# ml-rust/blazr

Measured on AMD Instinct MI355X. Metric: decode tokens/sec, Llama-3-8B AWQ-INT4 seq=1 on MI355X (and HBM-roofline fraction), higher is better.
Workload: dtype i4; 1 GPU; llama3-8b-awq greedy decode, batch 1, seq=1, prompt 16 (seed 26), whole step as one hipGraph; N>1 = independent replicas; resident_weight_bytes=5754585088, context_at_end=242

## Files before the change

blazr_amd/csrc/bz_host.hip:

```cpp
#include "bz_internal.h"
#include "bz_ggml.h"
#include <stdarg.h>
#include <stdio.h>
#include <string.h>
#include <math.h>
#include <algorithm>
#include <chrono>
#include <numeric>
#include <unordered_map>

static thread_local char g_err[1024] = "";
static bool bz_trace_on() { static int t = -1; if (t < 0) t = getenv("BZ_TRACE") ? 1 : 0; return t == 1; }
#define BZ_TRACE(...) do { if (bz_trace_on()) { fprintf(stderr, "[bz] " __VA_ARGS__); fputc('\n', stderr); fflush(stderr); } } while (0)
void bz_set_error(const char* fmt, ...) {
  va_list ap;
  va_start(ap, fmt);
  vsnprintf(g_err, sizeof(g_err), fmt, ap);
  va_end(ap);
}
extern "C" const char* bz_last_error(void) { return g_err; }
extern "C" int bz_abi_version(void) { return BZ_ABI_VERSION; }

size_t bz_dtype_size(int dt) {
  switch (dt) {
// ... 179 lines not shown
extern "C" int bz_tensor_to_host_pipelined(const bz_tensor* t, uint64_t ev, void* host, size_t bytes) {
  BZ_API_BEGIN
  if (!t || !host) BZ_FAIL(BZ_E_INVALID, "bad argument");
  if (bytes > t->nbytes) BZ_FAIL(BZ_E_INVALID, "to_host_pipelined: size");
  bz_device* d = t->dev;
  std::lock_guard<std::mutex> dlock__(d->mu);
  if (ev >= d->events.size()) BZ_FAIL(BZ_E_INVALID, "bad event");
  BZ_HIP(hipStreamWaitEvent(d->copy_stream, d->events[ev], 0));
  BZ_HIP(hipMemcpyAsync(host, t->ptr, bytes, hipMemcpyDeviceToHost, d->copy_stream));
  BZ_HIP(hipStreamSynchronize(d->copy_stream));
  return BZ_OK;
  BZ_API_END
}

struct RawTensor {
  int kind = 0;
  int dtype = BZ_F32;
  std::vector<int64_t> shape;
  int64_t N = 0, K = 0; int gs = 0; int ggml_type = 0;
  void* d0 = nullptr; void* d1 = nullptr; void* d2 = nullptr;
  float* d_bias = nullptr;
  std::vector<int32_t> g_idx;
  size_t bytes = 0;
  bool consumed = false;
};

struct FusedLinear {
  std::vector<LinearDev> parts;
  std::vector<int> n_off;
  int N = 0, K = 0;
  bool fix_out = true;
};

struct LayerDev {
  float* attn_norm = nullptr; float* ffn_norm = nullptr;
  FusedLinear qkv, o, gateup, down;
  void* down_slabs = nullptr;
};

struct MambaLayerDev {
  float* norm = nullptr; float* conv_w = nullptr; float* conv_b = nullptr; float* dt_bias = nullptr; float* A_log = nullptr; float* D = nullptr;
  float* gnorm = nullptr;
  FusedLinear in_proj, out_proj;
};

struct DsLayerDev {
  float* attn_norm = nullptr; float* ffn_norm = nullptr; float* kv_norm = nullptr;
  FusedLinear qkva, o;
  float* q_norm = nullptr; FusedLinear q_b;
  void* kv_b = nullptr; int kv_b_dt = BZ_BF16;
  bool is_moe = false;
  FusedLinear gateup, down;
  void* router = nullptr; int router_dt = BZ_BF16;
  void* e_gu = nullptr; void* e_dn = nullptr; int e_dt = BZ_BF16;
};

struct bz_model {
  std::recursive_mutex mu;
  std::vector<DsLayerDev> dlayers;
  float* mla_ws = nullptr; int mla_nsplit = 1;
  float* mla_scw = nullptr; float* mla_mxw = nullptr;
  double* mla_wsd = nullptr;
  long long* moe_gu_acc = nullptr;
  float* moe_xn = nullptr; float* moe_gu = nullptr; float* moe_out = nullptr; long long* moe_acc = nullptr; int* moe_sel = nullptr; float* moe_w = nullptr; float* moe_lg = nullptr; unsigned* moe_cnt = nullptr;
  int dpf_rows = 0; float* dpf_att = nullptr; void* dpf_xg16 = nullptr; float* dpf_gu = nullptr; void* dpf_a16 = nullptr; float* dpf_ye = nullptr; float* dpf_ysh = nullptr;
  int* dpf_sel = nullptr; float* dpf_w = nullptr; int* dpf_cnt = nullptr; int* dpf_off = nullptr; int* dpf_rowof = nullptr; int* dpf_tokof = nullptr;
  std::vector<MambaLayerDev> mlayers;
  float* ybuf = nullptr; float* vss = nullptr;
  int mpf_rows = 0; float* mpf_h = nullptr; float* mpf_t = nullptr; float* mpf_zx = nullptr; float* mpf_xbc = nullptr; float* mpf_y = nullptr; float* mpf_vss = nullptr;
  void* mpf_x16 = nullptr;
  bz_device* dev = nullptr;
  bz_model_config cfg;
  bool finalized = false;
  std::unordered_map<std::string, RawTensor> raw;
  std::vector<LayerDev> layers;
  void* embed = nullptr; int embed_dt = BZ_F16;
  int embed_ggml = 0;
  float* final_norm = nullptr;
  FusedLinear lm_head;
  std::unordered_map<std::string, LinearDev> named;
  std::vector<void*> owned;
  float* cos_t = nullptr; float* sin_t = nullptr;
  float* rope_cur = nullptr;
  float* att_ws = nullptr;
  float* hbuf[2] = {nullptr, nullptr};
  int pf_rows = 0; float* pf_h = nullptr; float* pf_t = nullptr; float* pf_qkv = nullptr; float* pf_gu = nullptr; void* pf_x16 = nullptr;
  int* row_pos = nullptr; int row_pos_n = 0;
  long long* pf_acc = nullptr;
  struct GqPf { float* wscale = nullptr; void* w3 = nullptr; };
  std::unordered_map<const FusedLinear*, GqPf> gq_pf;
  size_t gq_cache_bytes = 0;
  unsigned* gq_amax = nullptr; void* gq_w3_scratch = nullptr; size_t gq_w3_scratch_bytes = 0;
  void* pf_x3 = nullptr; float* pf_rscale = nullptr;
  void* pf_xq = nullptr; size_t pf_xq_bytes = 0;
  float* pf_ws = nullptr; size_t pf_ws_bytes = 0;
  long long* ring[3] = {nullptr, nullptr, nullptr};
  float* dring[3] = {nullptr, nullptr, nullptr};
  int ring_n = 0;
  float* attn_out = nullptr;
  float* logits = nullptr;
  float* pval = nullptr; int* pidx = nullptr; int nparts = 0;
  float* scratch = nullptr;
  long long* tok_tmp = nullptr;
  int* pos_tmp = nullptr;
  size_t resident = 0, per_token = 0;
};

static int dev_alloc(bz_model* m, void** p, size_t bytes) {
  hipError_t e = hipMalloc(p, std::max<size_t>(bytes, 16));
  if (e != hipSuccess) BZ_FAIL(BZ_E_OOM, "hipMalloc(%zu) failed: %s", bytes, hipGetErrorString(e));
  m->owned.push_back(*p);
  return BZ_OK;
}
static int upload(bz_device* d, void** out, const void* host, size_t bytes) {
  hipError_t e = hipMalloc(out, std::max<size_t>(bytes, 16));
  if (e != hipSuccess) BZ_FAIL(BZ_E_OOM, "hipMalloc(%zu) failed: %s", bytes, hipGetErrorString(e));
  if (bytes) BZ_HIP(hipMemcpy(*out, host, bytes, hipMemcpyHostToDevice));
  (void)d;
  return BZ_OK;
}

extern "C" int bz_model_create(bz_device* dev, const bz_model_config* cfg, bz_model** out) {
  BZ_API_BEGIN
  if (!dev || !cfg || !out) BZ_FAIL(BZ_E_INVALID, "bz_model_create: null argument");
  if (cfg->abi_version != BZ_ABI_VERSION) BZ_FAIL(BZ_E_INVALID, "config abi_version %d != %d", cfg->abi_version, BZ_ABI_VERSION);
  if (cfg->arch != BZ_ARCH_LLAMA && cfg->arch != BZ_ARCH_MAMBA2 && cfg->arch != BZ_ARCH_DEEPSEEK2) BZ_FAIL(BZ_E_UNSUPPORTED, "arch %d is not implemented", cfg->arch);
  if (cfg->arch == BZ_ARCH_DEEPSEEK2) {
    if (cfg->hidden <= 0 || cfg->n_layers <= 0 || cfg->n_heads <= 0 || cfg->vocab <= 0 || cfg->max_seq_len <= 0 || cfg->mla_kv_lora_rank <= 0 ||
        cfg->mla_nope_dim <= 0 || cfg->mla_rope_dim <= 0 || cfg->mla_v_dim <= 0 || cfg->moe_n_experts < 0 || cfg->moe_first_dense < 0)
      BZ_FAIL(BZ_E_INVALID, "config: non-positive deepseek2 dimension");
    if (cfg->mla_q_lora_rank < 0 || cfg->mla_q_lora_rank % 8) BZ_FAIL(BZ_E_INVALID, "config: q_lora_rank %d must be a non-negative multiple of 8", cfg->mla_q_lora_rank);
    if (cfg->hidden % 8 || cfg->mla_kv_lora_rank % 8 || cfg->mla_kv_lora_rank > 1024 || cfg->mla_rope_dim > 64 || (cfg->mla_rope_dim & 1) || cfg->mla_nope_dim % 4 ||
        cfg->mla_v_dim % 4)
      BZ_FAIL(BZ_E_UNSUPPORTED, "config: MLA dims unsupported (rank %% 8, rank <= 1024, rope <= 64 even, nope/v %% 4)");
    if (cfg->moe_n_experts > 0 && (cfg->moe_top_k <= 0 || cfg->moe_top_k > cfg->moe_n_experts || cfg->moe_top_k > 16 || cfg->moe_n_shared < 0 || cfg->moe_n_shared > 8 ||
                                   cfg->moe_inter <= 0 || cfg->moe_inter % 8 || cfg->moe_n_experts > 1024))
      BZ_FAIL(BZ_E_INVALID, "config: bad MoE configuration");
    if ((cfg->moe_first_dense > 0 || cfg->moe_n_experts == 0) && (cfg->inter <= 0 || cfg->inter % 8)) BZ_FAIL(BZ_E_INVALID, "config: dense layers need inter %% 8 == 0");
    if ((size_t)(cfg->mla_kv_lora_rank * 6 + cfg->mla_rope_dim * 2 + cfg->mla_nope_dim + 8 + cfg->max_seq_len) * 4 + 64 > 160 * 1024)
      BZ_FAIL(BZ_E_UNSUPPORTED, "config: max_seq_len %d too long for the single-pass MLA attention kernel", cfg->max_seq_len);
  } else if (cfg->arch == BZ_ARCH_MAMBA2) {
    if (cfg->hidden <= 0 || cfg->n_layers <= 0 || cfg->vocab <= 0 || cfg->ssm_d_inner <= 0 || cfg->ssm_n_heads <= 0 || cfg->ssm_head_dim <= 0 ||
        cfg->ssm_d_state <= 0 || cfg->ssm_n_groups <= 0 || cfg->ssm_conv_kernel < 2)
      BZ_FAIL(BZ_E_INVALID, "config: non-positive mamba2 dimension");
    if (cfg->ssm_n_heads * cfg->ssm_head_dim != cfg->ssm_d_inner || cfg->ssm_n_heads % cfg->ssm_n_groups || cfg->hidden % 8 || cfg->ssm_d_inner % 8)
      BZ_FAIL(BZ_E_INVALID, "config: inconsistent mamba2 dimensions");
  } else {
  if (cfg->hidden <= 0 || cfg->n_layers <= 0 || cfg->n_heads <= 0 || cfg->n_kv_heads <= 0 || cfg->head_dim <= 0 || cfg->inter <= 0 ||
      cfg->vocab <= 0 || cfg->max_seq_len <= 0)
    BZ_FAIL(BZ_E_INVALID, "config: non-positive dimension");
  if (cfg->n_heads % cfg->n_kv_heads) BZ_FAIL(BZ_E_INVALID, "config: n_heads %% n_kv_heads != 0");
  if (cfg->hidden % 8 || cfg->head_dim % 8 || cfg->inter % 8) BZ_FAIL(BZ_E_UNSUPPORTED, "config: hidden/head_dim/inter must be multiples of 8");
  }
  if (cfg->act_dtype != BZ_F32 && cfg->act_dtype != BZ_F16 && cfg->act_dtype != BZ_BF16) BZ_FAIL(BZ_E_INVALID, "config: bad act_dtype");
  bz_model* m = new bz_model();
  m->dev = dev; m->cfg = *cfg;
  if (cfg->arch == BZ_ARCH_DEEPSEEK2) { m->cfg.n_kv_heads = 1; m->cfg.head_dim = cfg->mla_kv_lora_rank + cfg->mla_rope_dim; }
  bz_dev_retain(dev);
  *out = m;
  return BZ_OK;
  BZ_API_END
}

static void raw_free(RawTensor& r) {
  if (r.d0) hipFree(r.d0);
  if (r.d1) hipFree(r.d1);
// ... 423 lines not shown
  const int H = c.hidden, nq = c.n_heads, nkv = c.n_kv_heads, hd = c.head_dim, I = c.inter, V = c.vocab;
  char nm[256];
  m->layers.resize(c.n_layers);
  for (int l = 0; l < c.n_layers; l++) {
    LayerDev& Ld = m->layers[l];
    snprintf(nm, sizeof nm, "model.layers.%d.", l);
    std::string p = nm;
    BZ_TRY(take_vector_f32(m, p + "input_layernorm.weight", H, &Ld.attn_norm));
    BZ_TRY(take_vector_f32(m, p + "post_attention_layernorm.weight", H, &Ld.ffn_norm));
    BZ_TRY(build_fused(m, {p + "self_attn.q_proj", p + "self_attn.k_proj", p + "self_attn.v_proj"}, &Ld.qkv));
    BZ_TRY(build_fused(m, {p + "self_attn.o_proj"}, &Ld.o));
    BZ_TRY(build_fused(m, {p + "mlp.gate_proj", p + "mlp.up_proj"}, &Ld.gateup));
    BZ_TRY(build_fused(m, {p + "mlp.down_proj"}, &Ld.down));
    if (Ld.qkv.N != (nq + 2 * nkv) * hd || Ld.qkv.K != H) BZ_FAIL(BZ_E_INVALID, "layer %d: q/k/v shapes do not match the config", l);
    if (Ld.o.N != H || Ld.o.K != nq * hd) BZ_FAIL(BZ_E_INVALID, "layer %d: o_proj shape does not match the config", l);
    if (Ld.gateup.N != 2 * I || Ld.gateup.K != H) BZ_FAIL(BZ_E_INVALID, "layer %d: gate/up shapes do not match the config", l);
    if (Ld.down.N != H || Ld.down.K != I) BZ_FAIL(BZ_E_INVALID, "layer %d: down_proj shape does not match the config", l);
    if (Ld.gateup.parts.size() == 1 && Ld.down.parts.size() == 1 && Ld.down.parts[0].kind == LK_ROWS) {
      char dummy = 0;
      if (bzk_mlp_dense_fusable(Ld.gateup.parts[0], Ld.down.parts[0], &dummy, H, I, c.act_dtype)) {
        BZ_TRY(dev_alloc(m, &Ld.down_slabs, (size_t)H * I * 2));
        BZ_TRY(bzk_repack_down_slabs(m->dev->stream, Ld.down.parts[0].w, H, I, Ld.down_slabs));
        m->resident += (size_t)H * I * 2;
      }
    }
  }
  BZ_HIP(hipStreamSynchronize(m->dev->stream));
  BZ_TRY(take_vector_f32(m, "model.norm.weight", H, &m->final_norm));
  {
    auto it = m->raw.find("model.embed_tokens.weight");
    if (it == m->raw.end()) BZ_FAIL(BZ_E_NOTFOUND, "finalize: 'model.embed_tokens.weight' was not added");
    RawTensor& r = it->second;
    const bool qemb = r.kind == 3 && (r.ggml_type == BZ_GGML_Q8_0 || r.ggml_type == BZ_GGML_Q4_K || r.ggml_type == BZ_GGML_Q5_K || r.ggml_type == BZ_GGML_Q6_K ||
                                      ggml_is_legacy(r.ggml_type));
    if ((r.kind != 0 && !qemb) || r.N != V || r.K != H)
      BZ_FAIL(BZ_E_INVALID, "finalize: embed_tokens must be dense or GGUF Q4_0/Q4_1/Q5_0/Q5_1/Q8_0/Q4_K/Q5_K/Q6_K [vocab, hidden]");
    const bool tied = c.tie_embeddings || !m->raw.count("lm_head.weight");
    if (qemb && tied) {
      if (V % 64) BZ_FAIL(BZ_E_UNSUPPORTED, "finalize: tied lm_head over a quantised embedding needs a vocabulary that is a multiple of 64 (vocab %d)", V);
      LinearDev L;
      BZ_TRY(build_gq(m, {&r}, &L));
      m->lm_head.parts.push_back(L); m->lm_head.n_off.push_back(0); m->lm_head.N = V; m->lm_head.K = H; m->lm_head.fix_out = true;
      LinearDev Vw = L; Vw.owned = false;
      m->named["lm_head.weight"] = Vw;
    }
    m->embed = r.d0; m->embed_dt = qemb ? BZ_U8 : r.dtype; m->embed_ggml = qemb ? r.ggml_type : 0;
    r.d0 = nullptr; m->owned.push_back(m->embed); r.consumed = true;
    m->resident += r.bytes;
    if (tied && !qemb) {
      LinearDev L; L.kind = LK_ROWS; L.N = V; L.K = H; L.wdt = m->embed_dt; L.w = m->embed; L.owned = false;
      L.bytes = 0; L.algo_bytes = r.bytes;
      m->lm_head.parts.push_back(L); m->lm_head.n_off.push_back(0); m->lm_head.N = V; m->lm_head.K = H; m->lm_head.fix_out = false;
      m->named["lm_head.weight"] = L;
    } else if (!tied) {
      BZ_TRY(build_fused(m, {"lm_head"}, &m->lm_head));
      force_direct(&m->lm_head);
      if (m->lm_head.N != V || m->lm_head.K != H) BZ_FAIL(BZ_E_INVALID, "finalize: lm_head shape does not match the config");
    }
  }
  if (m->lm_head.parts.size() != 1) BZ_FAIL(BZ_E_UNSUPPORTED, "finalize: lm_head must be a single tensor");
  for (auto& kv : m->raw) if (!kv.second.consumed) BZ_FAIL(BZ_E_INVALID, "finalize: tensor '%s' is not used by this architecture", kv.first.c_str());
  m->raw.clear();

  std::vector<float> cs, sn;
  rope_tables_host(c, cs, sn);
  void* p;
  BZ_TRY(dev_alloc(m, &p, cs.size() * 4)); m->cos_t = (float*)p; BZ_HIP(hipMemcpy(p, cs.data(), cs.size() * 4, hipMemcpyHostToDevice));
  BZ_TRY(dev_alloc(m, &p, sn.size() * 4)); m->sin_t = (float*)p; BZ_HIP(hipMemcpy(p, sn.data(), sn.size() * 4, hipMemcpyHostToDevice));
  BZ_TRY(dev_alloc(m, &p, 256 * 4)); m->rope_cur = (float*)p; BZ_HIP(hipMemset(p, 0, 256 * 4));
  BZ_TRY(dev_alloc(m, &p, bzk_attn_split_ws_bytes(c.n_heads))); m->att_ws = (float*)p;

  m->ring_n = std::max(std::max((nq + 2 * nkv) * hd, 2 * I), std::max(H, nq * hd));
  if (m->lm_head.fix_out) m->ring_n = std::max(m->ring_n, V);
  for (int i = 0; i < 3; i++) {
    BZ_TRY(dev_alloc(m, &p, (size_t)m->ring_n * 8)); m->ring[i] = (long long*)p; BZ_HIP(hipMemset(p, 0, (size_t)m->ring_n * 8));
    BZ_TRY(dev_alloc(m, &p, (size_t)m->ring_n * 4)); m->dring[i] = (float*)p; BZ_HIP(hipMemset(p, 0, (size_t)m->ring_n * 4));
  }
  for (int i = 0; i < 2; i++) { BZ_TRY(dev_alloc(m, &p, (size_t)H * 4)); m->hbuf[i] = (float*)p; }
  BZ_TRY(dev_alloc(m, &p, (size_t)nq * hd * 4)); m->attn_out = (float*)p;
  BZ_TRY(dev_alloc(m, &p, (size_t)V * 4)); m->logits = (float*)p;
  m->nparts = m->lm_head.fix_out ? 64 : bzk_gemv_rows_blocks(m->lm_head.parts[0]);
  BZ_TRY(dev_alloc(m, &p, (size_t)m->nparts * 4)); m->pval = (float*)p;
  BZ_TRY(dev_alloc(m, &p, (size_t)m->nparts * 4)); m->pidx = (int*)p;
  BZ_TRY(dev_alloc(m, &p, 4096)); m->scratch = (float*)p;
  BZ_TRY(dev_alloc(m, &p, 64)); m->tok_tmp = (long long*)p;
  BZ_TRY(dev_alloc(m, &p, 64)); m->pos_tmp = (int*)p;

  size_t act_b = bz_dtype_size(c.act_dtype);
  m->per_token = (size_t)(2 * c.n_layers + 1) * H * act_b + (m->embed_ggml ? ggml_blk_row_bytes(m->embed_ggml, H) : (size_t)H * bz_dtype_size(m->embed_dt));
  for (auto& Ld : m->layers)
    for (FusedLinear* F : {&Ld.qkv, &Ld.o, &Ld.gateup, &Ld.down})
      for (auto& L : F->parts) { m->resident += L.bytes; m->per_token += L.algo_bytes; }
  for (auto& L : m->lm_head.parts) { m->resident += L.bytes; m->per_token += L.algo_bytes; }
  BZ_HIP(hipDeviceSynchronize());
  m->finalized = true;
  return BZ_OK;
  BZ_API_END
}

extern "C" int bz_model_get_config(const bz_model* m, bz_model_config* out) {
  BZ_API_BEGIN
  if (!m || !out) BZ_FAIL(BZ_E_INVALID, "null argument");
  *out = m->cfg;
  return BZ_OK;
  BZ_API_END
}
extern "C" int bz_model_weight_bytes(const bz_model* m, size_t* resident, size_t* per_token) {
  BZ_API_BEGIN
  if (!m || !m->finalized) BZ_FAIL(BZ_E_INVALID, "model not finalized");
  if (resident) *resident = m->resident;
  if (per_token) *per_token = m->per_token;
  return BZ_OK;
  BZ_API_END
}
extern "C" int bz_rope_caches(bz_model* m, float* c, float* s) {
  BZ_API_BEGIN
  if (!m || !m->finalized) BZ_FAIL(BZ_E_INVALID, "model not finalized");
  size_t n = (size_t)m->cfg.max_seq_len * (m->cfg.head_dim / 2) * 4;
  if (c) BZ_HIP(hipMemcpy(c, m->cos_t, n, hipMemcpyDeviceToHost));
  if (s) BZ_HIP(hipMemcpy(s, m->sin_t, n, hipMemcpyDeviceToHost));
  return BZ_OK;
  BZ_API_END
}

static int take_dense(bz_model* m, const std::string& name, int64_t N, int64_t K, void** out, int* dt, size_t* bytes) {
  auto it = m->raw.find(name);
  if (it == m->raw.end()) BZ_FAIL(BZ_E_NOTFOUND, "finalize: tensor '%s' was not added", name.c_str());
  RawTensor& r = it->second;
  if (r.kind != 0 || r.N != N || r.K != K) BZ_FAIL(BZ_E_INVALID, "finalize: '%s' must be dense [%lld, %lld]", name.c_str(), (long long)N, (long long)K);
  *out = r.d0; *dt = r.dtype; if (bytes) *bytes = r.bytes;
  r.d0 = nullptr; m->owned.push_back(*out); r.consumed = true;
  m->resident += r.bytes;
  return BZ_OK;
}
static int stack_dense(bz_model* m, const std::string& name, int64_t N, int64_t K, int dt, void* dst, int64_t col0, int64_t ncols) {
  auto it = m->raw.find(name);
  if (it == m->raw.end()) BZ_FAIL(BZ_E_NOTFOUND, "finalize: tensor '%s' was not added", name.c_str());
  RawTensor& r = it->second;
  if (r.kind != 0 || r.N != N || r.K != K || r.dtype != dt) BZ_FAIL(BZ_E_INVALID, "finalize: '%s' must be dense [%lld, %lld] of the experts' dtype", name.c_str(), (long long)N, (long long)K);
  const size_t es = bz_dtype_size(dt);
  BZ_HIP(hipMemcpy2D(dst, (size_t)ncols * es, (const char*)r.d0 + (size_t)col0 * es, (size_t)K * es, (size_t)ncols * es, (size_t)N, hipMemcpyDeviceToDevice));
  return BZ_OK;
}

static int finalize_dsv2(bz_model* m) {
  const bz_model_config& c = m->cfg;
  const int H = c.hidden, NH = c.n_heads, R = c.mla_kv_lora_rank, DN = c.mla_nope_dim, DR = c.mla_rope_dim, DV = c.mla_v_dim, V = c.vocab;
  const int E = c.moe_n_experts, TK = c.moe_top_k, NS = c.moe_n_shared, MI = c.moe_inter;
  const size_t act_b = bz_dtype_size(c.act_dtype);
  char nm[256];
  m->dlayers.resize(c.n_layers);
  size_t per_token = 0;
  int ring_n = std::max(H, NH * DV);
  for (int l = 0; l < c.n_layers; l++) {
    DsLayerDev& L = m->dlayers[l];
    snprintf(nm, sizeof nm, "model.layers.%d.", l);
    std::string p = nm;
    BZ_TRY(take_vector_f32(m, p + "input_layernorm.weight", H, &L.attn_norm));
    BZ_TRY(take_vector_f32(m, p + "post_attention_layernorm.weight", H, &L.ffn_norm));
    BZ_TRY(take_vector_f32(m, p + "self_attn.kv_a_layernorm.weight", R, &L.kv_norm));
    const int QL = c.mla_q_lora_rank;
    if (QL > 0) {
      BZ_TRY(build_fused(m, {p + "self_attn.q_a_proj", p + "self_attn.kv_a_proj_with_mqa"}, &L.qkva));
      BZ_TRY(take_vector_f32(m, p + "self_attn.q_a_layernorm.weight", QL, &L.q_norm));
      BZ_TRY(build_fused(m, {p + "self_attn.q_b_proj"}, &L.q_b));
      if (L.q_b.parts.size() != 1 || L.q_b.parts[0].kind != LK_ROWS || L.q_b.N != NH * (DN + DR) || L.q_b.K != QL) BZ_FAIL(BZ_E_INVALID, "layer %d: q_b_proj must be dense [n_heads (nope + rope), q_lora_rank]", l);
// ... 29 lines not shown
      const size_t gu_sz = (size_t)2 * MI * H * es, dn_sz = (size_t)H * MI * es;
      BZ_TRY(dev_alloc(m, &L.e_gu, (size_t)(E + NS) * gu_sz));
      BZ_TRY(dev_alloc(m, &L.e_dn, (size_t)(E + NS) * dn_sz));
      for (int e = 0; e < E; e++) {
        snprintf(nm, sizeof nm, "%smlp.experts.%d.", p.c_str(), e);
        std::string q = nm;
        BZ_TRY(stack_dense(m, q + "gate_proj.weight", MI, H, L.e_dt, (char*)L.e_gu + (size_t)e * gu_sz, 0, H));
        BZ_TRY(stack_dense(m, q + "up_proj.weight", MI, H, L.e_dt, (char*)L.e_gu + (size_t)e * gu_sz + gu_sz / 2, 0, H));
        BZ_TRY(stack_dense(m, q + "down_proj.weight", H, MI, L.e_dt, (char*)L.e_dn + (size_t)e * dn_sz, 0, MI));
        for (const char* t : {"gate_proj.weight", "up_proj.weight", "down_proj.weight"}) { RawTensor& r = m->raw[q + t]; raw_free(r); r.consumed = true; }
      }
      if (NS > 0) {
        std::string q = p + "mlp.shared_experts.";
        auto itg = m->raw.find(q + "gate_proj.weight"), itu = m->raw.find(q + "up_proj.weight");
        if (itg == m->raw.end() || itu == m->raw.end()) BZ_FAIL(BZ_E_NOTFOUND, "finalize: layer %d shared experts missing", l);
        if (itg->second.kind != 0 || itg->second.N != (int64_t)NS * MI || itg->second.K != H || itg->second.dtype != L.e_dt || itu->second.kind != 0 ||
            itu->second.N != (int64_t)NS * MI || itu->second.K != H || itu->second.dtype != L.e_dt)
          BZ_FAIL(BZ_E_INVALID, "finalize: layer %d shared expert shapes do not match the config", l);
        for (int j = 0; j < NS; j++) {
          const size_t half_rows = (size_t)MI * H * es;
          BZ_HIP(hipMemcpy((char*)L.e_gu + (size_t)(E + j) * gu_sz, (const char*)itg->second.d0 + (size_t)j * half_rows, half_rows, hipMemcpyDeviceToDevice));
          BZ_HIP(hipMemcpy((char*)L.e_gu + (size_t)(E + j) * gu_sz + gu_sz / 2, (const char*)itu->second.d0 + (size_t)j * half_rows, half_rows, hipMemcpyDeviceToDevice));
          BZ_TRY(stack_dense(m, q + "down_proj.weight", H, (int64_t)NS * MI, L.e_dt, (char*)L.e_dn + (size_t)(E + j) * dn_sz, (int64_t)j * MI, MI));
        }
        for (const char* t : {"gate_proj.weight", "up_proj.weight", "down_proj.weight"}) { RawTensor& r = m->raw[q + t]; raw_free(r); r.consumed = true; }
      }
      m->resident += (size_t)(E + NS) * (gu_sz + dn_sz);
      per_token += rb + (size_t)(TK + NS) * (gu_sz + dn_sz);
    }
  }
  BZ_TRY(take_vector_f32(m, "model.norm.weight", H, &m->final_norm));
  {
    auto it = m->raw.find("model.embed_tokens.weight");
    if (it == m->raw.end()) BZ_FAIL(BZ_E_NOTFOUND, "finalize: 'model.embed_tokens.weight' was not added");
    RawTensor& r = it->second;
    if (r.kind != 0 || r.N != V || r.K != H) BZ_FAIL(BZ_E_INVALID, "finalize: embed_tokens must be dense [vocab, hidden]");
    m->embed = r.d0; m->embed_dt = r.dtype; r.d0 = nullptr; m->owned.push_back(m->embed); r.consumed = true;
    m->resident += r.bytes;
    if (c.tie_embeddings || !m->raw.count("lm_head.weight")) {
      LinearDev L; L.kind = LK_ROWS; L.N = V; L.K = H; L.wdt = m->embed_dt; L.w = m->embed; L.owned = false; L.bytes = 0; L.algo_bytes = r.bytes;
      m->lm_head.parts.push_back(L); m->lm_head.n_off.push_back(0); m->lm_head.N = V; m->lm_head.K = H; m->lm_head.fix_out = false;
      m->named["lm_head.weight"] = L;
    } else {
      BZ_TRY(build_fused(m, {"lm_head"}, &m->lm_head));
      force_direct(&m->lm_head);
      if (m->lm_head.N != V || m->lm_head.K != H || m->lm_head.fix_out) BZ_FAIL(BZ_E_INVALID, "finalize: lm_head must be dense [vocab, hidden]");
    }
  }
  for (auto& kv : m->raw) if (!kv.second.consumed) BZ_FAIL(BZ_E_INVALID, "finalize: tensor '%s' is not used by this architecture", kv.first.c_str());
  m->raw.clear();
  bz_model_config rc = c; rc.head_dim = DR;
  std::vector<float> cs, sn;
  rope_tables_host(rc, cs, sn);
  void* p;
  BZ_TRY(dev_alloc(m, &p, cs.size() * 4)); m->cos_t = (float*)p; BZ_HIP(hipMemcpy(p, cs.data(), cs.size() * 4, hipMemcpyHostToDevice));
  BZ_TRY(dev_alloc(m, &p, sn.size() * 4)); m->sin_t = (float*)p; BZ_HIP(hipMemcpy(p, sn.data(), sn.size() * 4, hipMemcpyHostToDevice));
  m->ring_n = std::max(ring_n, NH * (DN + DR) + R + DR + c.mla_q_lora_rank);
  for (int i = 0; i < 3; i++) {
    BZ_TRY(dev_alloc(m, &p, (size_t)m->ring_n * 8)); m->ring[i] = (long long*)p; BZ_HIP(hipMemset(p, 0, (size_t)m->ring_n * 8));
    BZ_TRY(dev_alloc(m, &p, (size_t)m->ring_n * 4)); m->dring[i] = (float*)p; BZ_HIP(hipMemset(p, 0, (size_t)m->ring_n * 4));
  }
  for (int i = 0; i < 2; i++) { BZ_TRY(dev_alloc(m, &p, (size_t)H * 4)); m->hbuf[i] = (float*)p; }
  BZ_TRY(dev_alloc(m, &p, (size_t)NH * DV * 4)); m->attn_out = (float*)p;
  m->mla_nsplit = bzk_mla_nsplit(NH);
  BZ_TRY(dev_alloc(m, &p, (size_t)NH * m->mla_nsplit * (R + 2) * 4)); m->mla_ws = (float*)p;
  BZ_TRY(dev_alloc(m, &p, (size_t)NH * m->mla_nsplit * (R + 1) * 8)); m->mla_wsd = (double*)p;
  BZ_TRY(dev_alloc(m, &p, (size_t)NH * m->mla_nsplit * ((c.max_seq_len + m->mla_nsplit - 1) / m->mla_nsplit + 1) * 4)); m->mla_scw = (float*)p;
  BZ_TRY(dev_alloc(m, &p, (size_t)NH * m->mla_nsplit * 4)); m->mla_mxw = (float*)p;
  BZ_TRY(dev_alloc(m, &p, (size_t)V * 4)); m->logits = (float*)p;
  if (E > 0) {
    BZ_TRY(dev_alloc(m, &p, (size_t)H * 4)); m->moe_xn = (float*)p;
    BZ_TRY(dev_alloc(m, &p, (size_t)(TK + NS) * 2 * MI * 4)); m->moe_gu = (float*)p;
    BZ_TRY(dev_alloc(m, &p, (size_t)(TK + NS) * 2 * MI * 8)); m->moe_gu_acc = (long long*)p; BZ_HIP(hipMemset(p, 0, (size_t)(TK + NS) * 2 * MI * 8));
    BZ_TRY(dev_alloc(m, &p, (size_t)H * 4)); m->moe_out = (float*)p;
    BZ_TRY(dev_alloc(m, &p, (size_t)(TK + 1) * H * 8)); m->moe_acc = (long long*)p; BZ_HIP(hipMemset(p, 0, (size_t)(TK + 1) * H * 8));
    BZ_TRY(dev_alloc(m, &p, (size_t)(TK + NS + 4) * 4)); m->moe_sel = (int*)p; BZ_HIP(hipMemset(p, 0, (size_t)(TK + NS + 4) * 4));
    BZ_TRY(dev_alloc(m, &p, (size_t)(TK + NS + 4) * 4)); m->moe_w = (float*)p; BZ_HIP(hipMemset(p, 0, (size_t)(TK + NS + 4) * 4));
    BZ_TRY(dev_alloc(m, &p, (size_t)(E + 4) * 4)); m->moe_lg = (float*)p;
    BZ_TRY(dev_alloc(m, &p, 64)); m->moe_cnt = (unsigned*)p; BZ_HIP(hipMemset(p, 0, 64));
  }
  m->nparts = bzk_gemv_rows_blocks(m->lm_head.parts[0]);
  BZ_TRY(dev_alloc(m, &p, (size_t)m->nparts * 4)); m->pval = (float*)p;
  BZ_TRY(dev_alloc(m, &p, (size_t)m->nparts * 4)); m->pidx = (int*)p;
  BZ_TRY(dev_alloc(m, &p, 4096)); m->scratch = (float*)p;
  BZ_TRY(dev_alloc(m, &p, 64)); m->tok_tmp = (long long*)p;
  BZ_TRY(dev_alloc(m, &p, 64)); m->pos_tmp = (int*)p;
  for (auto& L : m->lm_head.parts) { m->resident += L.bytes; per_token += L.algo_bytes; }
  m->per_token = per_token + (size_t)H * bz_dtype_size(m->embed_dt) + (size_t)H * act_b;
  BZ_HIP(hipDeviceSynchronize());
  m->finalized = true;
  return BZ_OK;
}

static int finalize_mamba2(bz_model* m) {
  const bz_model_config& c = m->cfg;
  const int D = c.hidden, DI = c.ssm_d_inner, NH = c.ssm_n_heads, NS = c.ssm_d_state, G = c.ssm_n_groups, KC = c.ssm_conv_kernel, V = c.vocab;
  const int conv_dim = DI + 2 * G * NS, d_in = 2 * DI + 2 * G * NS + NH;
  char nm[256];
  m->mlayers.resize(c.n_layers);
  for (int l = 0; l < c.n_layers; l++) {
    MambaLayerDev& L = m->mlayers[l];
    snprintf(nm, sizeof nm, "backbone.layers.%d.", l);
    std::string p = nm;
    BZ_TRY(take_vector_f32(m, p + "norm.weight", D, &L.norm));
    BZ_TRY(take_vector_f32(m, p + "mixer.conv1d.weight", conv_dim * KC, &L.conv_w));
    BZ_TRY(take_vector_f32(m, p + "mixer.conv1d.bias", conv_dim, &L.conv_b));
    BZ_TRY(take_vector_f32(m, p + "mixer.dt_bias", NH, &L.dt_bias, false));
    if (m->raw.count(p + "mixer.A_log")) BZ_TRY(take_vector_f32(m, p + "mixer.A_log", NH, &L.A_log, false));
    else {
      BZ_TRY(take_vector_f32(m, p + "mixer.A", NH, &L.A_log, false));
      std::vector<float> a(NH);
      BZ_HIP(hipMemcpy(a.data(), L.A_log, (size_t)NH * 4, hipMemcpyDeviceToHost));
      for (int i = 0; i < NH; i++) {
        if (!(a[i] < 0.f)) BZ_FAIL(BZ_E_INVALID, "layer %d: mixer.A[%d] = %g is not negative (A = -exp(A_log))", l, i, (double)a[i]);
        a[i] = logf(-a[i]);
      }
      BZ_HIP(hipMemcpy(L.A_log, a.data(), (size_t)NH * 4, hipMemcpyHostToDevice));
    }
    BZ_TRY(take_vector_f32(m, p + "mixer.D", NH, &L.D, false));
    BZ_TRY(take_vector_f32(m, p + "mixer.norm.weight", DI, &L.gnorm));
    BZ_TRY(build_fused(m, {p + "mixer.in_proj"}, &L.in_proj));
    BZ_TRY(build_fused(m, {p + "mixer.out_proj"}, &L.out_proj));
    if (L.in_proj.N != d_in || L.in_proj.K != D || L.out_proj.N != D || L.out_proj.K != DI) BZ_FAIL(BZ_E_INVALID, "layer %d: in_proj/out_proj shapes do not match the config", l);
    if (L.in_proj.parts[0].kind != LK_ROWS || L.out_proj.parts[0].kind != LK_ROWS)
      BZ_FAIL(BZ_E_UNSUPPORTED, "mamba2: quantised projections are not implemented (dense f16/bf16/f32)");
  }
  BZ_TRY(take_vector_f32(m, "backbone.norm_f.weight", D, &m->final_norm));
  {
    auto it = m->raw.find("backbone.embeddings.weight");
    if (it == m->raw.end()) BZ_FAIL(BZ_E_NOTFOUND, "finalize: 'backbone.embeddings.weight' was not added");
    RawTensor& r = it->second;
    if (r.kind != 0 || r.N != V || r.K != D) BZ_FAIL(BZ_E_INVALID, "finalize: embeddings must be dense [vocab, hidden]");
    m->embed = r.d0; m->embed_dt = r.dtype; r.d0 = nullptr; m->owned.push_back(m->embed); r.consumed = true;
    m->resident += r.bytes;
    if (c.tie_embeddings || !m->raw.count("lm_head.weight")) {
      LinearDev L; L.kind = LK_ROWS; L.N = V; L.K = D; L.wdt = m->embed_dt; L.w = m->embed; L.owned = false; L.bytes = 0; L.algo_bytes = r.bytes;
      m->lm_head.parts.push_back(L); m->lm_head.n_off.push_back(0); m->lm_head.N = V; m->lm_head.K = D; m->lm_head.fix_out = false;
      m->named["lm_head.weight"] = L;
    } else {
      BZ_TRY(build_fused(m, {"lm_head"}, &m->lm_head));
      force_direct(&m->lm_head);
      if (m->lm_head.fix_out) BZ_FAIL(BZ_E_UNSUPPORTED, "mamba2: quantised lm_head is not implemented");
    }
  }
  for (auto& kv : m->raw) if (!kv.second.consumed) BZ_FAIL(BZ_E_INVALID, "finalize: tensor '%s' is not used by this architecture", kv.first.c_str());
  m->raw.clear();
  void* p;
  m->ring_n = std::max(std::max(d_in, DI), D);
  for (int i = 0; i < 3; i++) {
    BZ_TRY(dev_alloc(m, &p, (size_t)m->ring_n * 8)); m->ring[i] = (long long*)p; BZ_HIP(hipMemset(p, 0, (size_t)m->ring_n * 8));
    BZ_TRY(dev_alloc(m, &p, (size_t)m->ring_n * 4)); m->dring[i] = (float*)p; BZ_HIP(hipMemset(p, 0, (size_t)m->ring_n * 4));
  }
  for (int i = 0; i < 2; i++) { BZ_TRY(dev_alloc(m, &p, (size_t)D * 4)); m->hbuf[i] = (float*)p; }
  BZ_TRY(dev_alloc(m, &p, (size_t)DI * 4)); m->ybuf = (float*)p;
  BZ_TRY(dev_alloc(m, &p, (size_t)NH * 8)); m->vss = (float*)p;
  BZ_TRY(dev_alloc(m, &p, (size_t)V * 4)); m->logits = (float*)p;
  m->nparts = bzk_gemv_rows_blocks(m->lm_head.parts[0]);
  BZ_TRY(dev_alloc(m, &p, (size_t)m->nparts * 4)); m->pval = (float*)p;
  BZ_TRY(dev_alloc(m, &p, (size_t)m->nparts * 4)); m->pidx = (int*)p;
  BZ_TRY(dev_alloc(m, &p, 64)); m->tok_tmp = (long long*)p;
  BZ_TRY(dev_alloc(m, &p, 64)); m->pos_tmp = (int*)p;
  const size_t act_b = bz_dtype_size(c.act_dtype);
  m->per_token = (size_t)D * bz_dtype_size(m->embed_dt) + (size_t)D * act_b;
  for (auto& L : m->mlayers) {
    for (FusedLinear* F : {&L.in_proj, &L.out_proj}) for (auto& P : F->parts) { m->resident += P.bytes; m->per_token += P.algo_bytes; }
    m->per_token += (size_t)(conv_dim * (KC + 1) + 3 * NH + DI + D) * act_b;
  }
  for (auto& L : m->lm_head.parts) { m->resident += L.bytes; m->per_token += L.algo_bytes; }
  BZ_HIP(hipDeviceSynchronize());
  m->finalized = true;
  return BZ_OK;
}

extern "C" int bz_ssm_state_create(bz_model* m, int batch, int dtype, bz_ssm_state** out) {
  BZ_API_BEGIN
  if (!m || !m->finalized || m->cfg.arch != BZ_ARCH_MAMBA2 || !out) BZ_FAIL(BZ_E_INVALID, "ssm_state_create: needs a finalized mamba2 model");
  if (batch != 1) BZ_FAIL(BZ_E_UNSUPPORTED, "ssm state: batch %d (single-stream decode only)", batch);
  if (dtype != BZ_F32 && dtype != BZ_F16 && dtype != BZ_BF16) BZ_FAIL(BZ_E_INVALID, "ssm state: dtype %d", dtype);
  if (dtype != m->cfg.act_dtype) BZ_FAIL(BZ_E_UNSUPPORTED, "ssm state dtype must equal the model's activation dtype");
  BZ_HIP(hipSetDevice(m->dev->id));
  const bz_model_config& c = m->cfg;
  bz_ssm_state* s = new bz_ssm_state();
  s->dev = m->dev; s->layers = c.n_layers; s->n_heads = c.ssm_n_heads; s->head_dim = c.ssm_head_dim; s->d_state = c.ssm_d_state;
  s->conv_dim = c.ssm_d_inner + 2 * c.ssm_n_groups * c.ssm_d_state; s->kc = c.ssm_conv_kernel; s->dtype = dtype;
  const size_t sb = (size_t)s->layers * s->n_heads * s->head_dim * s->d_state * bz_dtype_size(dtype);
  const size_t cb = (size_t)s->layers * s->conv_dim * (s->kc - 1) * 4;
  if (hipMalloc(&s->ssm, sb) != hipSuccess || hipMalloc((void**)&s->conv, cb) != hipSuccess) { delete s; BZ_FAIL(BZ_E_OOM, "ssm state: hipMalloc failed"); }
  BZ_HIP(hipMemsetAsync(s->ssm, 0, sb, m->dev->stream));
  BZ_HIP(hipMemsetAsync(s->conv, 0, cb, m->dev->stream));
  bz_dev_retain(m->dev);
  *out = s;
  return BZ_OK;
  BZ_API_END
}
extern "C" int bz_ssm_state_free(bz_ssm_state* s) {
  BZ_API_BEGIN
  if (!s) return BZ_OK;
  hipStreamSynchronize(s->dev->stream);
  hipFree(s->ssm); hipFree(s->conv);
  bz_dev_release(s->dev);
  delete s;
  return BZ_OK;
  BZ_API_END
}
extern "C" int bz_ssm_state_reset(bz_ssm_state* s) {
  BZ_API_BEGIN
  if (!s) BZ_FAIL(BZ_E_INVALID, "null state");
  const size_t sb = (size_t)s->layers * s->n_heads * s->head_dim * s->d_state * bz_dtype_size(s->dtype);
  const size_t cb = (size_t)s->layers * s->conv_dim * (s->kc - 1) * 4;
  BZ_HIP(hipMemsetAsync(s->ssm, 0, sb, s->dev->stream));
  BZ_HIP(hipMemsetAsync(s->conv, 0, cb, s->dev->stream));
  return BZ_OK;
  BZ_API_END
}

extern "C" int bz_kv_create(bz_device* dev, int layers, int batch, int n_kv, int init_cap, int max_len, int hd, int dtype, bz_kv** out) {
  BZ_API_BEGIN
  if (!dev || !out) BZ_FAIL(BZ_E_INVALID, "null argument");
  if (batch != 1) BZ_FAIL(BZ_E_UNSUPPORTED, "kv cache: batch %d (single-stream decode only)", batch);
  if (layers <= 0 || n_kv <= 0 || init_cap <= 0 || max_len < init_cap || hd <= 0) BZ_FAIL(BZ_E_INVALID, "kv cache: bad dimensions");
  if (dtype != BZ_F16 && dtype != BZ_BF16 && dtype != BZ_F32) BZ_FAIL(BZ_E_INVALID, "kv cache: dtype %d", dtype);
  BZ_HIP(hipSetDevice(dev->id));
  bz_kv* kv = new bz_kv();
  kv->dev = dev; kv->layers = layers; kv->n_kv = n_kv; kv->cap = init_cap; kv->max_len = max_len; kv->hd = hd; kv->dtype = dtype;
  size_t bytes = (size_t)layers * n_kv * init_cap * hd * bz_dtype_size(dtype);
  if (hipMalloc(&kv->k, bytes) != hipSuccess || hipMalloc(&kv->v, bytes) != hipSuccess) { delete kv; BZ_FAIL(BZ_E_OOM, "kv cache: hipMalloc(%zu) failed", bytes); }
  BZ_HIP(hipMemsetAsync(kv->k, 0, bytes, dev->stream));
  BZ_HIP(hipMemsetAsync(kv->v, 0, bytes, dev->stream));
  bz_dev_retain(dev);
  *out = kv;
  return BZ_OK;
  BZ_API_END
}
extern "C" int bz_kv_free(bz_kv* kv) {
  BZ_API_BEGIN
  if (!kv) return BZ_OK;
  hipStreamSynchronize(kv->dev->stream);
  hipFree(kv->k); hipFree(kv->v);
  bz_dev_release(kv->dev);
  delete kv;
  return BZ_OK;
  BZ_API_END
// ... 16 lines not shown
  const size_t oldp = (size_t)kv->cap * kv->hd * es, newp = (size_t)ncap * kv->hd * es;
  BZ_HIP(hipMemcpy2DAsync(nk, newp, kv->k, oldp, oldp, rows, hipMemcpyDeviceToDevice, st));
  BZ_HIP(hipMemcpy2DAsync(nv, newp, kv->v, oldp, oldp, rows, hipMemcpyDeviceToDevice, st));
  BZ_HIP(hipStreamSynchronize(st));
  hipFree(kv->k); hipFree(kv->v);
  kv->k = nk; kv->v = nv; kv->cap = ncap;
  return BZ_OK;
}

static KvView view_of(const bz_kv* kv) {
  KvView v{};
  v.k = kv->k; v.v = kv->v; v.dtype = kv->dtype; v.hd = kv->hd; v.n_kv = kv->n_kv; v.paged = 0;
  v.layer_stride = (long long)kv->n_kv * kv->cap * kv->hd; v.cap = kv->cap; v.bs = 1; v.block_table = nullptr; v.slot = nullptr;
  return v;
}
static KvView view_of(const bz_paged_kv* kv, const int* block_table, const int* slot) {
  KvView v{};
  v.k = kv->k; v.v = kv->v; v.dtype = kv->dtype; v.hd = kv->hd; v.n_kv = kv->n_kv; v.paged = 1;
  v.layer_stride = (long long)kv->num_blocks * kv->n_kv * kv->block_size * kv->hd; v.cap = 0; v.bs = kv->block_size;
  v.block_table = block_table; v.slot = slot;
  return v;
}

extern "C" int bz_kv_read(const bz_kv* kv, int layer, int kvh, int which, int len, float* host) {
  BZ_API_BEGIN
  if (!kv || !host || layer < 0 || layer >= kv->layers || kvh < 0 || kvh >= kv->n_kv || len < 0 || len > kv->cap) BZ_FAIL(BZ_E_INVALID, "kv_read: bad argument");
  float* d;
  BZ_HIP(hipMalloc(&d, std::max<size_t>((size_t)len * kv->hd * 4, 16)));
  int rc = bzk_kv_read(kv->dev->stream, view_of(kv), layer, kvh, which, len, d);
  if (rc == BZ_OK) { hipMemcpyAsync(host, d, (size_t)len * kv->hd * 4, hipMemcpyDeviceToHost, kv->dev->stream); hipStreamSynchronize(kv->dev->stream); }
  hipFree(d);
  return rc;
  BZ_API_END
}

extern "C" int bz_paged_kv_create(bz_device* dev, int layers, int num_blocks, int block_size, int n_kv, int hd, int dtype, bz_paged_kv** out) {
  BZ_API_BEGIN
  if (!dev || !out) BZ_FAIL(BZ_E_INVALID, "null argument");
  if (layers <= 0 || num_blocks <= 0 || block_size <= 0 || n_kv <= 0 || hd <= 0) BZ_FAIL(BZ_E_INVALID, "paged kv: bad dimensions");
  if (dtype != BZ_F16 && dtype != BZ_BF16 && dtype != BZ_F32) BZ_FAIL(BZ_E_INVALID, "paged kv: dtype %d", dtype);
  BZ_HIP(hipSetDevice(dev->id));
  bz_paged_kv* kv = new bz_paged_kv();
  kv->dev = dev; kv->layers = layers; kv->num_blocks = num_blocks; kv->block_size = block_size; kv->n_kv = n_kv; kv->hd = hd; kv->dtype = dtype;
  size_t bytes = (size_t)layers * num_blocks * n_kv * block_size * hd * bz_dtype_size(dtype);
  if (hipMalloc(&kv->k, bytes) != hipSuccess || hipMalloc(&kv->v, bytes) != hipSuccess) { delete kv; BZ_FAIL(BZ_E_OOM, "paged kv: hipMalloc(%zu) failed", bytes); }
  BZ_HIP(hipMemsetAsync(kv->k, 0, bytes, dev->stream));
  BZ_HIP(hipMemsetAsync(kv->v, 0, bytes, dev->stream));
  bz_dev_retain(dev);
  *out = kv;
  return BZ_OK;
  BZ_API_END
}
extern "C" int bz_paged_kv_free(bz_paged_kv* kv) {
  BZ_API_BEGIN
  if (!kv) return BZ_OK;
  hipStreamSynchronize(kv->dev->stream);
  hipFree(kv->k); hipFree(kv->v);
  bz_dev_release(kv->dev);
  delete kv;
  return BZ_OK;
  BZ_API_END
}
extern "C" int bz_paged_kv_set_seq_len(bz_paged_kv* kv, int n) { if (!kv || n < 0) BZ_FAIL(BZ_E_INVALID, "bad argument"); kv->seq_len = n; return BZ_OK; }
extern "C" int bz_paged_kv_seq_len(const bz_paged_kv* kv) { return kv ? kv->seq_len : -1; }

__global__ void k_set_int(int* p, int v) { p[0] = v; }

static thread_local hipStream_t tl_capture_stream = nullptr;
static hipStream_t step_stream(const bz_model* m) { return tl_capture_stream ? tl_capture_stream : m->dev->stream; }

static int att_split_min() { const char* e = getenv("BZ_SPLIT_MIN"); return e ? atoi(e) : 512; }
static int att_positions_for(int len) { return len > att_split_min() ? len : 0; }

struct StepIO {
  KvView kv;
  const long long* d_tok;
  const int* d_pos;
  const float* hidden_in = nullptr; const float* prev_in = nullptr;
  int layer_start = 0, layer_end = -1;
  bool do_embed = true, do_head = true;
  float* hidden_out = nullptr; float* prev_out = nullptr;
  FinalArgs* final_args = nullptr;
  bz_ssm_state* ssm = nullptr;
  int att_positions = 0;
};

struct RingState { int ri = 0; int dirty[3] = {0, 0, 0}; };

static int run_fused(bz_model* m, const FusedLinear& F, Pro pro, RingState& rs, VSrc* out, const ConvShift* shift = nullptr) {
  hipStream_t st = step_stream(m);
  const int act = m->cfg.act_dtype;
  const int ri = rs.ri, rz = (rs.ri + 1) % 3;
  long long* acc = m->ring[ri];
  float* direct = m->dring[ri];
  static const bool no_mix = getenv("BZ_NO_GQ_MIX") != nullptr;
  if (!no_mix && F.parts.size() == 2 && F.fix_out && F.n_off[1] == F.parts[0].N && bzk_gq_mix_ok(F.parts[0], F.parts[1], pro)) {
    GemvOut o{};
    o.acc = acc; o.zero_buf = rs.dirty[rz] > 0 ? m->ring[rz] : nullptr; o.zero_n = rs.dirty[rz];
    BZ_TRY(bzk_gemv_gq_mix(st, F.parts[0], F.parts[1], pro, o));
    rs.dirty[rz] = 0; rs.dirty[ri] = F.N; rs.ri = rz;
    out->fix = 1; out->p = (const void*)acc;
    return BZ_OK;
  }
  for (size_t i = 0; i < F.parts.size(); i++) {
    const LinearDev& L = F.parts[i];
    Pro p = pro; p.perm = L.perm;
    GemvOut o{};
    o.acc = acc + F.n_off[i]; o.direct = direct + F.n_off[i];
    o.zero_buf = (i == 0 && rs.dirty[rz] > 0) ? m->ring[rz] : nullptr; o.zero_n = rs.dirty[rz];
    if (i == 0 && shift) o.shift = *shift;
    BZ_TRY(bzk_gemv(st, L, p, o, act));
  }
  rs.dirty[rz] = 0;
  rs.dirty[ri] = F.fix_out ? F.N : 0;
  rs.ri = rz;
  out->fix = F.fix_out ? 1 : 0;
  out->p = F.fix_out ? (const void*)acc : (const void*)direct;
  return BZ_OK;
}

static int llama_step(bz_model* m, const StepIO& io) {
  const bz_model_config& c = m->cfg;
  hipStream_t st = step_stream(m);
  const int H = c.hidden, I = c.inter, act = c.act_dtype;
  const int lend = io.layer_end < 0 ? c.n_layers : io.layer_end;
  int cur = 0;
  RingState rs;
  VSrc prev{nullptr, 0};
  if (io.do_embed) {
    BZ_TRY(bzk_embed(st, m->embed, m->embed_dt, m->embed_ggml, io.d_tok, H, act, m->hbuf[cur], io.d_pos, m->cos_t, m->sin_t, c.head_dim / 2, m->rope_cur));
  } else {
    if (io.d_pos && lend > io.layer_start) BZ_TRY(bzk_rope_row(st, io.d_pos, m->cos_t, m->sin_t, c.head_dim / 2, m->rope_cur));
    BZ_HIP(hipMemcpyAsync(m->hbuf[cur], io.hidden_in, (size_t)H * 4, hipMemcpyDeviceToDevice, st));
    if (io.prev_in) { prev.p = io.prev_in; prev.fix = 0; }
  }
  for (int l = io.layer_start; l < lend; l++) {
    const LayerDev& Ld = m->layers[l];
    Pro pn{}; pn.mode = PRO_NORM; pn.src = prev; pn.h_in = m->hbuf[cur]; pn.h_out = m->hbuf[cur ^ 1]; pn.norm_w = Ld.attn_norm;
    pn.eps = c.rms_eps; pn.H = H; pn.act = act;
    VSrc qkv;
    BZ_TRY(run_fused(m, Ld.qkv, pn, rs, &qkv));
    cur ^= 1;

    AttnArgs aa{};
    aa.qkv = qkv; aa.cos_t = m->cos_t; aa.sin_t = m->sin_t; aa.interleaved = c.rope_interleaved; aa.pos = io.d_pos; aa.rope_cur = m->rope_cur;
    aa.nq = c.n_heads; aa.nkv = c.n_kv_heads; aa.hd = c.head_dim; aa.act = act; aa.kv = io.kv; aa.layer = l; aa.out = m->attn_out;
    aa.zero_buf = nullptr; aa.zero_n = 0; aa.q_only = 0;
    VSrc ov;
    static const bool no_fuse = getenv("BZ_NO_ATTN_FUSION") != nullptr;
    const bool fuse_cap = !no_fuse && Ld.o.parts.size() == 1 && Ld.o.fix_out && bzk_attn_oproj_slices(aa, Ld.o.parts[0]) > 0;
    static const bool no_split = getenv("BZ_NO_ATTN_SPLIT") != nullptr;
    const bool split_wanted = !no_split && io.att_positions > 0 && m->att_ws && bzk_attn_split_ok(aa);
    const bool merge_fused = fuse_cap && Ld.o.parts[0].kind == LK_Q4G && bzk_attn_merge_oproj_ok(aa, Ld.o.parts[0]);
    const bool fuse_o = fuse_cap && (io.att_positions == 0 || (split_wanted && merge_fused));
    const bool split = split_wanted && (!fuse_o || merge_fused);
    int nsplit = 0;
    if (split) {
      nsplit = bzk_attn_split_slices(io.att_positions);
      BZ_TRY(bzk_attn_split(st, aa, nsplit, m->att_ws));
    }
    if (fuse_o) {
      const int rz = (rs.ri + 1) % 3;
      aa.zero_buf = rs.dirty[rz] > 0 ? m->ring[rz] : nullptr; aa.zero_n = rs.dirty[rz];
      if (split) BZ_TRY(bzk_attn_merge_oproj(st, aa, m->att_ws, nsplit, Ld.o.parts[0], m->ring[rs.ri]));
      else BZ_TRY(bzk_attn_oproj(st, aa, Ld.o.parts[0], m->ring[rs.ri]));
      ov = VSrc{m->ring[rs.ri], 1};
      rs.dirty[rz] = 0; rs.dirty[rs.ri] = Ld.o.N; rs.ri = rz;
    } else {
      if (split) BZ_TRY(bzk_attn_merge(st, aa, m->att_ws, nsplit));
      else BZ_TRY(bzk_attn_decode(st, aa));
      Pro pp{}; pp.mode = PRO_PLAIN; pp.src = VSrc{m->attn_out, 0}; pp.act = act; pp.H = 0;
      BZ_TRY(run_fused(m, Ld.o, pp, rs, &ov));
    }

    Pro pf{}; pf.mode = PRO_NORM; pf.src = ov; pf.h_in = m->hbuf[cur]; pf.h_out = m->hbuf[cur ^ 1]; pf.norm_w = Ld.ffn_norm;
    pf.eps = c.rms_eps; pf.H = H; pf.act = act;
    VSrc dn;
    static const bool no_mlp_fuse = getenv("BZ_NO_MLP_FUSION") != nullptr;
    if (!no_mlp_fuse && act == BZ_F16 && Ld.gateup.parts.size() == 1 && Ld.down.parts.size() == 1 && bzk_mlp_fusable(Ld.gateup.parts[0], Ld.down.parts[0], H, I)) {
      const int rz = (rs.ri + 1) % 3;
      BZ_TRY(bzk_mlp_q4g(st, Ld.gateup.parts[0], Ld.down.parts[0], H, I, pf, m->ring[rs.ri], rs.dirty[rz] > 0 ? m->ring[rz] : nullptr, rs.dirty[rz]));
      dn = VSrc{m->ring[rs.ri], 1};
      rs.dirty[rz] = 0; rs.dirty[rs.ri] = H; rs.ri = rz;
      cur ^= 1;
    } else if (!no_mlp_fuse && Ld.gateup.parts.size() == 1 && Ld.down.parts.size() == 1 && bzk_mlp_dense_fusable(Ld.gateup.parts[0], Ld.down.parts[0], Ld.down_slabs, H, I, act)) {
      const int rz = (rs.ri + 1) % 3;
      BZ_TRY(bzk_mlp_dense(st, Ld.gateup.parts[0], Ld.down.parts[0], Ld.down_slabs, H, I, pf, m->ring[rs.ri], rs.dirty[rz] > 0 ? m->ring[rz] : nullptr, rs.dirty[rz]));
      dn = VSrc{m->ring[rs.ri], 1};
      rs.dirty[rz] = 0; rs.dirty[rs.ri] = H; rs.ri = rz;
      cur ^= 1;
    } else if (!no_mlp_fuse && Ld.gateup.parts.size() == 1 && Ld.down.parts.size() == 1 && bzk_mlp_gq_fusable(Ld.gateup.parts[0], Ld.down.parts[0], H, I, act)) {
      const int rz = (rs.ri + 1) % 3;
      BZ_TRY(bzk_mlp_gq(st, Ld.gateup.parts[0], Ld.down.parts[0], H, I, pf, m->ring[rs.ri], rs.dirty[rz] > 0 ? m->ring[rz] : nullptr, rs.dirty[rz]));
      dn = VSrc{m->ring[rs.ri], 1};
      rs.dirty[rz] = 0; rs.dirty[rs.ri] = H; rs.ri = rz;
      cur ^= 1;
    } else {
      VSrc gu;
      BZ_TRY(run_fused(m, Ld.gateup, pf, rs, &gu));
      cur ^= 1;
      Pro ps{}; ps.mode = PRO_SILU; ps.src = gu; ps.H = I; ps.act = act;
      BZ_TRY(run_fused(m, Ld.down, ps, rs, &dn));
    }
    prev = dn;
  }
  if (io.hidden_out) {
    BZ_HIP(hipMemcpyAsync(io.hidden_out, m->hbuf[cur], (size_t)H * 4, hipMemcpyDeviceToDevice, st));
    if (io.prev_out && prev.p) {
      if (prev.fix) BZ_TRY(bzk_fix_to_f32(st, (const long long*)prev.p, H, act, io.prev_out));
      else BZ_HIP(hipMemcpyAsync(io.prev_out, prev.p, (size_t)H * 4, hipMemcpyDeviceToDevice, st));
    }
  }
  const int ra = (rs.ri + 2) % 3, rb = (rs.ri + 1) % 3;
  if (io.do_head) {
    Pro ph{}; ph.mode = PRO_NORM; ph.src = prev; ph.h_in = m->hbuf[cur]; ph.h_out = nullptr; ph.norm_w = m->final_norm;
    ph.eps = c.rms_eps; ph.H = H; ph.act = act;
    int rfin = ra;
    if (m->lm_head.fix_out) {
      VSrc lv;
      BZ_TRY(run_fused(m, m->lm_head, ph, rs, &lv));
      BZ_TRY(bzk_fix_to_f32(st, (const long long*)lv.p, c.vocab, act, m->logits));
      BZ_TRY(bzk_argmax_partials(st, m->logits, c.vocab, m->pval, m->pidx, m->nparts));
      rfin = -1;
    } else {
      GemvOut o{};
      o.direct = m->logits; o.amax_val = m->pval; o.amax_idx = m->pidx;
      o.zero_buf = rs.dirty[rb] > 0 ? m->ring[rb] : nullptr; o.zero_n = rs.dirty[rb];
      BZ_TRY(bzk_gemv(st, m->lm_head.parts[0], ph, o, act));
      rs.dirty[rb] = 0;
    }
    if (io.final_args) {
      FinalArgs fa = *io.final_args;
      fa.pval = m->pval; fa.pidx = m->pidx; fa.nparts = m->nparts;
      if (rfin >= 0) { fa.zero_buf = rs.dirty[rfin] > 0 ? m->ring[rfin] : nullptr; fa.zero_n = rs.dirty[rfin]; }
      BZ_TRY(bzk_argmax_final(st, fa));
      if (rfin >= 0) rs.dirty[rfin] = 0;
    }
  }
  for (int i = 0; i < 3; i++) if (rs.dirty[i] > 0) BZ_TRY(bzk_zero64(st, m->ring[i], rs.dirty[i]));
  return BZ_OK;
}


static int mamba_step(bz_model* m, const StepIO& io) {
  const bz_model_config& c = m->cfg;
  hipStream_t st = step_stream(m);
  const int D = c.hidden, DI = c.ssm_d_inner, NH = c.ssm_n_heads, NS = c.ssm_d_state, G = c.ssm_n_groups, KC = c.ssm_conv_kernel, act = c.act_dtype;
  const int conv_dim = DI + 2 * G * NS;
  bz_ssm_state* S = io.ssm;
  int cur = 0;
  RingState rs;
  VSrc prev{nullptr, 0};
  BZ_TRY(bzk_embed(st, m->embed, m->embed_dt, m->embed_ggml, io.d_tok, D, act, m->hbuf[cur]));
  for (int l = 0; l < c.n_layers; l++) {
    const MambaLayerDev& L = m->mlayers[l];
    Pro pn{}; pn.mode = PRO_NORM; pn.src = prev; pn.h_in = m->hbuf[cur]; pn.h_out = m->hbuf[cur ^ 1]; pn.norm_w = L.norm; pn.eps = c.rms_eps; pn.H = D; pn.act = act;
    VSrc zx;
    BZ_TRY(run_fused(m, L.in_proj, pn, rs, &zx));
    cur ^= 1;
    SsmArgs sa{};
    sa.zx = zx; sa.z_off = 0; sa.x_off = DI; sa.dt_off = DI + conv_dim; sa.dt_bias = L.dt_bias; sa.A_log = L.A_log; sa.D = L.D;
    sa.conv_w = L.conv_w; sa.conv_b = L.conv_b; sa.conv_state = S->conv + (size_t)l * conv_dim * (KC - 1); sa.conv_kernel = KC;
    sa.state = (char*)S->ssm + (size_t)l * NH * c.ssm_head_dim * NS * bz_dtype_size(S->dtype); sa.sdt = S->dtype;
    sa.n_heads = NH; sa.head_dim = c.ssm_head_dim; sa.d_state = NS; sa.n_groups = G; sa.d_inner = DI; sa.act = act; sa.y = m->ybuf; sa.gate = 1; sa.vss = m->vss;
    BZ_TRY(bzk_ssm_step(st, sa));
    Pro pg{}; pg.mode = PRO_GATED2; pg.src = VSrc{m->ybuf, 0}; pg.h_in = m->vss; pg.aux2 = NH; pg.norm_w = L.gnorm; pg.eps = c.rms_eps; pg.H = DI; pg.act = act; pg.aux = G;
    VSrc ov;
    ConvShift shf{sa.conv_state, zx, DI, DI, 2 * G * NS, KC};
    BZ_TRY(run_fused(m, L.out_proj, pg, rs, &ov, &shf));
    prev = ov;
  }
  const int ra = (rs.ri + 2) % 3, rb = (rs.ri + 1) % 3;
  if (io.do_head) {
    Pro ph{}; ph.mode = PRO_NORM; ph.src = prev; ph.h_in = m->hbuf[cur]; ph.h_out = nullptr; ph.norm_w = m->final_norm; ph.eps = c.rms_eps; ph.H = D; ph.act = act;
    GemvOut o{};
    o.direct = m->logits; o.amax_val = m->pval; o.amax_idx = m->pidx;
    o.zero_buf = rs.dirty[rb] > 0 ? m->ring[rb] : nullptr; o.zero_n = rs.dirty[rb];
    BZ_TRY(bzk_gemv(st, m->lm_head.parts[0], ph, o, act));
    rs.dirty[rb] = 0;
    if (io.final_args) {
      FinalArgs fa = *io.final_args;
      fa.pval = m->pval; fa.pidx = m->pidx; fa.nparts = m->nparts;
      fa.zero_buf = rs.dirty[ra] > 0 ? m->ring[ra] : nullptr; fa.zero_n = rs.dirty[ra];
      BZ_TRY(bzk_argmax_final(st, fa));
      rs.dirty[ra] = 0;
    }
  }
  for (int i = 0; i < 3; i++) if (rs.dirty[i] > 0) BZ_TRY(bzk_zero64(st, m->ring[i], rs.dirty[i]));
  return BZ_OK;
}

static int dsv2_step(bz_model* m, const StepIO& io) {
  const bz_model_config& c = m->cfg;
  hipStream_t st = step_stream(m);
  const int H = c.hidden, NH = c.n_heads, R = c.mla_kv_lora_rank, DN = c.mla_nope_dim, DR = c.mla_rope_dim, DV = c.mla_v_dim, act = c.act_dtype;
  const int E = c.moe_n_experts, TK = c.moe_top_k, NS = c.moe_n_shared, MI = c.moe_inter;
  int cur = 0;
  RingState rs;
  VSrc prev{nullptr, 0};
  BZ_TRY(bzk_embed(st, m->embed, m->embed_dt, m->embed_ggml, io.d_tok, H, act, m->hbuf[cur]));
  for (int l = 0; l < c.n_layers; l++) {
    const DsLayerDev& L = m->dlayers[l];
    Pro pn{}; pn.mode = PRO_NORM; pn.src = prev; pn.h_in = m->hbuf[cur]; pn.h_out = m->hbuf[cur ^ 1]; pn.norm_w = L.attn_norm; pn.eps = c.rms_eps; pn.H = H; pn.act = act; pn.f32_sums = 0;
    VSrc qkva;
    BZ_TRY(run_fused(m, L.qkva, pn, rs, &qkva));
    cur ^= 1;
    MlaArgs ma{};
    if (c.mla_q_lora_rank > 0) {
      Pro pq{}; pq.mode = PRO_NORM; pq.src = VSrc{nullptr, 0}; pq.h_in = (const float*)qkva.p; pq.h_out = nullptr; pq.norm_w = L.q_norm; pq.eps = c.rms_eps; pq.H = c.mla_q_lora_rank; pq.act = act; pq.f32_sums = 0;
      VSrc qv;
      BZ_TRY(run_fused(m, L.q_b, pq, rs, &qv));
      ma.kva = (const float*)qkva.p + c.mla_q_lora_rank;
      qkva = qv;
    }
    ma.qkv = qkva; ma.kv_norm = L.kv_norm; ma.eps = c.rms_eps; ma.wkvb = L.kv_b; ma.wdt = L.kv_b_dt; ma.cos_t = m->cos_t; ma.sin_t = m->sin_t; ma.pos = io.d_pos;
    ma.n_heads = NH; ma.rank = R; ma.nope = DN; ma.rope = DR; ma.vdim = DV; ma.act = act; ma.kv = io.kv; ma.layer = l; ma.out = m->attn_out;
    ma.scale = mla_softmax_scale(c);
    ma.ws = m->mla_ws; ma.nsplit = m->mla_nsplit;
    static const bool f32_mla = getenv("BZ_DSV2_F32_SUMS") != nullptr;
    if (!f32_mla && (act == BZ_F16 || act == BZ_BF16) && bzk_mla_x_ok(ma, c.max_seq_len)) BZ_TRY(bzk_mla_attn_x(st, ma, c.max_seq_len, m->mla_wsd, m->mla_scw, m->mla_mxw));
    else BZ_TRY(bzk_mla_attn(st, ma, c.max_seq_len));
    Pro pp{}; pp.mode = PRO_PLAIN; pp.src = VSrc{m->attn_out, 0}; pp.act = act; pp.H = 0; pp.f32_sums = 0;
    VSrc ov;
    BZ_TRY(run_fused(m, L.o, pp, rs, &ov));
    Pro pf{}; pf.mode = PRO_NORM; pf.src = ov; pf.h_in = m->hbuf[cur]; pf.h_out = m->hbuf[cur ^ 1]; pf.norm_w = L.ffn_norm; pf.eps = c.rms_eps; pf.H = H; pf.act = act; pf.f32_sums = 0;
    if (!L.is_moe) {
      VSrc gu, dn;
      BZ_TRY(run_fused(m, L.gateup, pf, rs, &gu));
      cur ^= 1;
      Pro ps{}; ps.mode = PRO_SILU; ps.src = gu; ps.H = c.inter; ps.act = act; ps.f32_sums = 0;
      BZ_TRY(run_fused(m, L.down, ps, rs, &dn));
      prev = dn;
    } else {
      const int slots = TK + NS;
      const size_t es = bz_dtype_size(L.e_dt);
      static const bool no_fr = getenv("BZ_NO_MOE_ROUTE_FUSION") != nullptr;
      if (!no_fr && bzk_moe_rows2_ok(L.e_dt, H) && bzk_moe_rows2_ok(L.e_dt, MI) && bzk_moe_rows2_ok(L.router_dt, H) && E <= 1024 && slots <= 128) {
        LinearDev RL; RL.kind = LK_ROWS; RL.N = E; RL.K = H; RL.wdt = L.router_dt; RL.w = L.router; RL.sk = 2; RL.owned = false; RL.algo_bytes = (size_t)E * H * bz_dtype_size(L.router_dt);
        FusedLinear RF; RF.parts.push_back(RL); RF.n_off.push_back(0); RF.N = E; RF.K = H; RF.fix_out = true;
        VSrc lg;
        Pro pr = pf; pr.f32_sums = 0;
        BZ_TRY(run_fused(m, RF, pr, rs, &lg));
        cur ^= 1;
        Pro pg = pf; pg.h_out = nullptr;
        MoeGemvArgs g1{};
        g1.w = L.e_gu; g1.expert_stride = (long long)2 * MI * H; g1.sel = nullptr; g1.N = 2 * MI; g1.K = H; g1.src_stride = 0;
        g1.acc = m->moe_gu_acc; g1.acc_stride = 2 * MI; g1.acc_slots = slots;
        g1.route = RouteArgs{(const long long*)lg.p, E, TK, NS, c.moe_routed_scale, c.moe_norm_topk, m->moe_sel, m->moe_w};
        BZ_TRY(bzk_moe_gemv(st, g1, L.e_dt, slots, pg, act, true, (double)slots * 2 * MI * H * es));
        MoeGemvArgs g2{};
        g2.w = L.e_dn; g2.expert_stride = (long long)H * MI; g2.sel = m->moe_sel; g2.N = H; g2.K = MI; g2.src_stride = 2 * MI;
        g2.acc = m->moe_acc; g2.acc_stride = H; g2.acc_slots = TK + 1;
        Pro p2{}; p2.mode = PRO_SILU; p2.src = VSrc{m->moe_gu_acc, 1}; p2.H = MI; p2.act = act;
        BZ_TRY(bzk_moe_gemv(st, g2, L.e_dt, slots, p2, act, true, (double)slots * H * MI * es));
        BZ_TRY(bzk_moe_combine(st, m->moe_acc, m->moe_w, TK, NS > 0, H, act, m->moe_out, m->moe_gu_acc, slots * 2 * MI));
        prev = VSrc{m->moe_out, 0};
        continue;
      }
      BZ_TRY(bzk_moe_router(st, pf, L.router, L.router_dt, E, TK, NS, c.moe_routed_scale, c.moe_norm_topk, m->moe_xn, m->moe_sel, m->moe_w, m->moe_lg, m->moe_cnt));
      cur ^= 1;
      const bool r2 = bzk_moe_rows2_ok(L.e_dt, H) && bzk_moe_rows2_ok(L.e_dt, MI);
      MoeGemvArgs g1{};
      g1.w = L.e_gu; g1.expert_stride = (long long)2 * MI * H; g1.sel = m->moe_sel; g1.N = 2 * MI; g1.K = H; g1.src_stride = 0;
      g1.out = m->moe_gu; g1.out_stride = 2 * MI;
      if (r2) { g1.acc = m->moe_gu_acc; g1.acc_stride = 2 * MI; g1.acc_slots = slots; }
      Pro p1{}; p1.mode = PRO_PLAIN; p1.src = VSrc{m->moe_xn, 0}; p1.act = act;
      BZ_TRY(bzk_moe_gemv(st, g1, L.e_dt, slots, p1, act, r2, (double)slots * 2 * MI * H * es));
      MoeGemvArgs g2{};
      g2.w = L.e_dn; g2.expert_stride = (long long)H * MI; g2.sel = m->moe_sel; g2.N = H; g2.K = MI; g2.src_stride = 2 * MI;
      g2.acc = m->moe_acc; g2.acc_stride = H; g2.acc_slots = TK + 1;
      Pro p2{}; p2.mode = PRO_SILU; p2.src = r2 ? VSrc{m->moe_gu_acc, 1} : VSrc{m->moe_gu, 0}; p2.H = MI; p2.act = act;
      BZ_TRY(bzk_moe_gemv(st, g2, L.e_dt, slots, p2, act, true, (double)slots * H * MI * es));
      BZ_TRY(bzk_moe_combine(st, m->moe_acc, m->moe_w, TK, NS > 0, H, act, m->moe_out, r2 ? m->moe_gu_acc : nullptr, slots * 2 * MI));
      prev = VSrc{m->moe_out, 0};
    }
  }
  const int ra = (rs.ri + 2) % 3, rb = (rs.ri + 1) % 3;
  if (io.do_head) {
    Pro ph{}; ph.mode = PRO_NORM; ph.src = prev; ph.h_in = m->hbuf[cur]; ph.h_out = nullptr; ph.norm_w = m->final_norm; ph.eps = c.rms_eps; ph.H = H; ph.act = act;
    GemvOut o{};
    o.direct = m->logits; o.amax_val = m->pval; o.amax_idx = m->pidx;
    o.zero_buf = rs.dirty[rb] > 0 ? m->ring[rb] : nullptr; o.zero_n = rs.dirty[rb];
    BZ_TRY(bzk_gemv(st, m->lm_head.parts[0], ph, o, act));
    rs.dirty[rb] = 0;
    if (io.final_args) {
      FinalArgs fa = *io.final_args;
      fa.pval = m->pval; fa.pidx = m->pidx; fa.nparts = m->nparts;
      fa.zero_buf = rs.dirty[ra] > 0 ? m->ring[ra] : nullptr; fa.zero_n = rs.dirty[ra];
      BZ_TRY(bzk_argmax_final(st, fa));
      rs.dirty[ra] = 0;
    }
  }
  for (int i = 0; i < 3; i++) if (rs.dirty[i] > 0) BZ_TRY(bzk_zero64(st, m->ring[i], rs.dirty[i]));
  return BZ_OK;
}

static int model_step(bz_model* m, const StepIO& io) {
  if (m->cfg.arch == BZ_ARCH_MAMBA2) return mamba_step(m, io);
  if (m->cfg.arch == BZ_ARCH_DEEPSEEK2) return dsv2_step(m, io);
  return llama_step(m, io);
}

static int check_fwd(bz_model* m, const bz_tensor* tokens, int S) {
  if (!m || !m->finalized) BZ_FAIL(BZ_E_INVALID, "forward: model not finalized");
  if (!tokens || tokens->dtype != BZ_I64 || tokens->nbytes < (size_t)S * 8 || S <= 0) BZ_FAIL(BZ_E_INVALID, "forward: tokens must be an I64 tensor with >= S elements");
  BZ_HIP(hipSetDevice(m->dev->id));
  return BZ_OK;
}

static int emit_logits(bz_model* m, bz_tensor* logits_out, int row) {
  const size_t vb = (size_t)m->cfg.vocab * 4;
  if (!logits_out || logits_out->dtype != BZ_F32 || logits_out->nbytes < (size_t)(row + 1) * vb) BZ_FAIL(BZ_E_INVALID, "forward: logits_out too small");
  BZ_HIP(hipMemcpyAsync((char*)logits_out->ptr + (size_t)row * vb, m->logits, vb, hipMemcpyDeviceToDevice, m->dev->stream));
  return BZ_OK;
}


static int find_linear(bz_model* m, const char* name, LinearDev* out);
static int prefill_min_rows() {
  static const int v = getenv("BZ_NO_MFMA_PREFILL") ? (1 << 30) : (getenv("BZ_PREFILL_MIN") ? atoi(getenv("BZ_PREFILL_MIN")) : 8);
  return v;
}
static int prefill_exact(const bz_model* m, int n, bool decode_batch);
static bool prefill_eligible(const bz_model* m, int S, int total_len, bool decode_batch = false) {
  const bz_model_config& c = m->cfg;
  static const bool no_gq = getenv("BZ_NO_GGUF_PREFILL") != nullptr;
  if (c.arch != BZ_ARCH_LLAMA || S < prefill_min_rows() || (c.act_dtype != BZ_F16 && c.act_dtype != BZ_BF16 && (c.act_dtype != BZ_F32 || no_gq))) return false;
  if (c.hidden % 64 || (c.n_heads * c.head_dim) % 64 || c.inter % 64 || c.head_dim % 8 || 256 % (c.head_dim / 8)) return false;
  const int rep = c.n_heads / c.n_kv_heads;
  if (rep != 1 && rep != 2 && rep != 4 && rep != 8) return false;
  const bool attn_exact = !decode_batch && (prefill_exact(m, S, false) != 0 || c.act_dtype == BZ_F32);
  const bool attn_mfma = !decode_batch && c.act_dtype != BZ_F32 && !attn_exact && bzk_pf_attn_mfma_ok(c.head_dim, rep);
  if (!attn_mfma && (!decode_batch || !bzk_pf_attn_mfma_ok(c.head_dim, rep)) &&
      bzk_pf_attn_smem(c.n_heads, c.n_kv_heads, c.head_dim, total_len, attn_exact) > 160 * 1024) return false;
  if (c.act_dtype == BZ_F32) {
    for (const LayerDev& L : m->layers)
      for (const FusedLinear* F : {&L.qkv, &L.o, &L.gateup, &L.down}) {
        if (F->parts.empty()) return false;
        unsigned long long ntot = 0;
        for (const LinearDev& P : F->parts) { if (!bzk_gq_split_ok(P) || P.bias || P.K != F->parts[0].K) return false; ntot += (unsigned long long)P.N; }
        if (ntot * 3ull * (unsigned long long)F->parts[0].K >= (1ull << 32) || (unsigned long long)std::min(S, 2048) * 3ull * (unsigned long long)F->parts[0].K >= (1ull << 32)) return false;
      }
    return true;
  }
  bool any_dense = false;
  for (const LayerDev& L : m->layers)
    for (const FusedLinear* F : {&L.qkv, &L.o, &L.gateup, &L.down}) {
      if (F->parts.size() != 1) return false;
      const LinearDev& P = F->parts[0];
      const bool dense_ok = P.kind == LK_ROWS && P.wdt == c.act_dtype, q4_ok = bzk_gemm_q4g_rows_ok(P);
      if (!dense_ok && !q4_ok) return false;
      any_dense = any_dense || dense_ok;
    }
  if (any_dense && !decode_batch) {
    static const int env = getenv("BZ_EXACT_PREFILL") ? atoi(getenv("BZ_EXACT_PREFILL")) : -1;
    static const int max_rows = getenv("BZ_EXACT_PREFILL_MAX") ? atoi(getenv("BZ_EXACT_PREFILL_MAX")) : 16;
    if (env != 0 && (env > 0 || S <= max_rows)) return false;
  }
  return m->lm_head.parts.size() == 1 && m->lm_head.parts[0].kind == LK_ROWS && !m->lm_head.fix_out;
}
static int ensure_pf_ws(bz_model* m) {
  if (m->pf_ws) return BZ_OK;
  void* p;
  m->pf_ws_bytes = (size_t)48 << 20;
  BZ_TRY(dev_alloc(m, &p, m->pf_ws_bytes));
  m->pf_ws = (float*)p;
  return BZ_OK;
}
static int prefill_ws(bz_model* m, int rows) {
  if (m->pf_rows >= rows) return BZ_OK;
  const bz_model_config& c = m->cfg;
  const size_t qn = (size_t)(c.n_heads + 2 * c.n_kv_heads) * c.head_dim, xw = std::max<size_t>(std::max<size_t>(c.hidden, c.inter), (size_t)c.n_heads * c.head_dim);
  BZ_HIP(hipStreamSynchronize(m->dev->stream));
  void* p;
// ... 809 lines not shown
  const int wave = (blockIdx.x * 512 + threadIdx.x) >> 6, lane = threadIdx.x & 63;
  const bz_u32x4_t* p = src + (size_t)wave * per_wave_vec + lane;
  bz_u32x4_t acc = {0, 0, 0, 0};
  for (size_t i = 0; i < per_wave_vec; i += 64 * 8) {
    bz_u32x4_t v[8];
#pragma unroll
    for (int d = 0; d < 8; d++) v[d] = __builtin_nontemporal_load(p + i + 64 * d);
#pragma unroll
    for (int d = 0; d < 8; d++) acc ^= v[d];
  }
  if ((acc.x ^ acc.y ^ acc.z ^ acc.w) == 0x12345678u) sink[0] = 1;
}
extern "C" int bz_probe_hbm_read(bz_device* dev, size_t bytes, int iters, double* gbs) {
  BZ_API_BEGIN
  if (!dev || !gbs || iters <= 0 || bytes < (64u << 20)) BZ_FAIL(BZ_E_INVALID, "probe_hbm_read: bad argument (>= 64 MiB)");
  BZ_HIP(hipSetDevice(dev->id));
  hipStream_t st = dev->stream;
  const int NBUF = 4, waves = 256 * 8;
  const size_t per_wave_vec = bytes / 16 / waves / 512 * 512;
  const size_t used = per_wave_vec * 16 * waves;
  void* bufs[NBUF] = {nullptr, nullptr, nullptr, nullptr}; unsigned* sink = nullptr;
  int rc = BZ_OK;
  for (int b = 0; b < NBUF; b++) if (hipMalloc(&bufs[b], used) != hipSuccess) { rc = BZ_E_OOM; bufs[b] = nullptr; break; } else hipMemsetAsync(bufs[b], b + 1, used, st);
  if (rc == BZ_OK && hipMalloc((void**)&sink, 64) != hipSuccess) rc = BZ_E_OOM;
  double best = 0.0;
  if (rc == BZ_OK) {
    hipEvent_t e0, e1; hipEventCreate(&e0); hipEventCreate(&e1);
    for (int i = 0; i < iters + 2; i++) {
      hipEventRecord(e0, st);
      hipLaunchKernelGGL(k_probe_read, dim3(256), dim3(512), 0, st, (const bz_u32x4_t*)bufs[i % NBUF], per_wave_vec, sink);
      hipEventRecord(e1, st);
      hipEventSynchronize(e1);
      float ms = 0.f; hipEventElapsedTime(&ms, e0, e1);
      if (i >= 2 && ms > 0.f) best = std::max(best, (double)used / 1e9 / (ms * 1e-3));
    }
    hipEventDestroy(e0); hipEventDestroy(e1);
  }
  for (int b = 0; b < NBUF; b++) if (bufs[b]) hipFree(bufs[b]);
  if (sink) hipFree(sink);
  if (rc != BZ_OK) BZ_FAIL(rc, "probe_hbm_read: out of device memory");
  *gbs = best;
  return BZ_OK;
  BZ_API_END
}

extern "C" int bz_logits_to_token(bz_device* dev, const bz_tensor* logits, int64_t rows, int64_t vocab, const bz_tensor* ids, const bz_tensor* cnts,
                                  int n, float rp, float fp, float pp, float temperature, int top_k, float top_p, float min_p, uint64_t seed,
                                  bz_tensor* token_out) {
  BZ_API_BEGIN
  if (!dev || !logits || !token_out || rows <= 0 || vocab <= 0) BZ_FAIL(BZ_E_INVALID, "logits_to_token: bad argument");
  if (logits->dtype != BZ_F32 || logits->nbytes < (size_t)rows * vocab * 4) BZ_FAIL(BZ_E_INVALID, "logits_to_token: logits must be F32 [rows,vocab]");
  if (token_out->dtype != BZ_I64 || token_out->nbytes < 8) BZ_FAIL(BZ_E_INVALID, "logits_to_token: token_out must be I64[1]");
  if (n > 0 && (!ids || !cnts || ids->dtype != BZ_I64 || cnts->dtype != BZ_I32 || ids->nbytes < (size_t)n * 8 || cnts->nbytes < (size_t)n * 4))
    BZ_FAIL(BZ_E_INVALID, "logits_to_token: ids I64[n] / cnts I32[n] required");
  std::lock_guard<std::mutex> dlock__(dev->mu);
  BZ_HIP(hipSetDevice(dev->id));
  float* scratch = dev->scratch;
  if (temperature < 0.0f) BZ_FAIL(BZ_E_INVALID, "logits_to_token: negative temperature");
  if (temperature != 0.0f)
    return bzk_sample(dev->stream, &dev->samp_ws, (const float*)logits->ptr + (size_t)(rows - 1) * vocab, vocab, n ? (const long long*)ids->ptr : nullptr,
                      n ? (const int*)cnts->ptr : nullptr, n, rp, fp, pp, temperature, top_k, top_p, min_p, seed, (long long*)token_out->ptr);
  int rc = bzk_logits_to_token(dev->stream, (const float*)logits->ptr + (size_t)(rows - 1) * vocab, vocab, n ? (const long long*)ids->ptr : nullptr,
                               n ? (const int*)cnts->ptr : nullptr, n, rp, fp, pp, temperature, top_k, top_p, min_p, seed, scratch,
                               (long long*)token_out->ptr);
  return rc;
  BZ_API_END
}
extern "C" int bz_argmax_to_buf(bz_device* dev, const bz_tensor* logits, int64_t rows, int64_t vocab, bz_tensor* token_out) {
  BZ_API_BEGIN
  return bz_logits_to_token(dev, logits, rows, vocab, nullptr, nullptr, 0, 1.0f, 0.f, 0.f, 0.f, 0, 1.f, 0.f, 0, token_out);
  BZ_API_END
}

struct bz_decode_graph {
  bz_model* m = nullptr;
  bz_device* dev = nullptr;
  hipGraph_t graph = nullptr; hipGraphExec_t exec = nullptr;
  hipGraph_t graph_long = nullptr; hipGraphExec_t exec_long = nullptr;
  KvView view{}; int capacity = 0;
  int seed_pos = 0;
  long long* tok_buf = nullptr;
  int* pos = nullptr;
  int* step = nullptr;
  long long* tok_log = nullptr;
  int* block_table = nullptr; int max_blocks = 0;
  bz_kv* kv = nullptr; bz_paged_kv* pkv = nullptr; bz_ssm_state* ssm = nullptr;
  std::vector<hipEvent_t> evs;
  long long replays = 0;
  static const int LOGCAP = 4096;
};

static int graph_capture_variant(bz_decode_graph* g, int att_positions, hipGraph_t* graph_out, hipGraphExec_t* exec_out) {
  bz_model* m = g->m;
  FinalArgs fa{};
  fa.tok_out = g->tok_buf; fa.tok_log = g->tok_log; fa.step = g->step; fa.logcap = bz_decode_graph::LOGCAP; fa.pos = g->pos;
  StepIO io{};
  io.kv = g->view; io.d_tok = g->tok_buf; io.d_pos = g->pos; io.final_args = &fa; io.ssm = g->ssm; io.att_positions = att_positions;
  BZ_TRACE("graph: begin capture");
  hipStream_t cap = nullptr;
  BZ_HIP(hipStreamCreateWithFlags(&cap, hipStreamNonBlocking));
  hipError_t eb = hipStreamBeginCapture(cap, hipStreamCaptureModeThreadLocal);
  if (eb != hipSuccess) { hipStreamDestroy(cap); BZ_FAIL(BZ_E_HIP, "hipStreamBeginCapture failed: %s", hipGetErrorString(eb)); }
  tl_capture_stream = cap;
  int rc = model_step(m, io);
  tl_capture_stream = nullptr;
  hipGraph_t graph = nullptr;
  hipError_t e = hipStreamEndCapture(cap, &graph);
  hipStreamDestroy(cap);
  BZ_TRACE("graph: end capture rc=%d hip=%d", rc, (int)e);
  if (rc != BZ_OK) { if (graph) hipGraphDestroy(graph); return rc; }
  if (e != hipSuccess) BZ_FAIL(BZ_E_HIP, "hipStreamEndCapture failed: %s", hipGetErrorString(e));
  *graph_out = graph;
  BZ_HIP(hipGraphInstantiate(exec_out, graph, nullptr, nullptr, 0));
  BZ_TRACE("graph: instantiated");
  return BZ_OK;
}

static int graph_capture_common(bz_decode_graph* g, const KvView& view) {
  bz_model* m = g->m;
  hipStream_t st = m->dev->stream;
  BZ_HIP(hipMalloc(&g->tok_buf, 64));
  BZ_HIP(hipMalloc(&g->pos, 64));
  BZ_HIP(hipMalloc(&g->step, 64));
  BZ_HIP(hipMemset(g->tok_buf, 0, 64)); BZ_HIP(hipMemset(g->pos, 0, 64)); BZ_HIP(hipMemset(g->step, 0, 64));
  BZ_HIP(hipHostMalloc(&g->tok_log, sizeof(long long) * bz_decode_graph::LOGCAP, hipHostMallocDefault));
  memset(g->tok_log, 0xff, sizeof(long long) * bz_decode_graph::LOGCAP);
  BZ_HIP(hipDeviceSynchronize());
  g->view = view;
  BZ_TRY(graph_capture_variant(g, 0, &g->graph, &g->exec));
  for (int i = 0; i < 8; i++) { hipEvent_t ev; BZ_HIP(hipEventCreateWithFlags(&ev, hipEventDisableTiming)); g->evs.push_back(ev); }
  return BZ_OK;
}

extern "C" int bz_decode_graph_capture(bz_model* m, bz_kv* kv, bz_decode_graph** out) {
  BZ_API_BEGIN
  if (!m || !m->finalized || !kv || !out) BZ_FAIL(BZ_E_INVALID, "graph capture: bad argument");
  std::lock_guard<std::recursive_mutex> lock__(m->mu);
  if (m->cfg.arch == BZ_ARCH_MAMBA2) BZ_FAIL(BZ_E_INVALID, "graph capture: model has no KV cache (use bz_decode_graph_capture_ssm)");
  if (kv->layers != m->cfg.n_layers || kv->n_kv != m->cfg.n_kv_heads || kv->hd != m->cfg.head_dim) BZ_FAIL(BZ_E_INVALID, "graph capture: cache does not match the model");
  BZ_HIP(hipSetDevice(m->dev->id));
  BZ_TRY(kv_grow(kv, kv->max_len));
  bz_decode_graph* g = new bz_decode_graph();
  bz_dev_retain(m->dev); g->dev = m->dev;
  g->m = m; g->kv = kv; g->capacity = kv->max_len;
  int rc = graph_capture_common(g, view_of(kv));
  if (rc != BZ_OK) { bz_decode_graph_free(g); return rc; }
  *out = g;
  return BZ_OK;
  BZ_API_END
}
extern "C" int bz_decode_graph_capture_paged(bz_model* m, bz_paged_kv* kv, int max_blocks, bz_decode_graph** out) {
  BZ_API_BEGIN
  if (!m || !m->finalized || !kv || !out || max_blocks <= 0) BZ_FAIL(BZ_E_INVALID, "graph capture: bad argument");
  std::lock_guard<std::recursive_mutex> lock__(m->mu);
  if (m->cfg.arch == BZ_ARCH_MAMBA2) BZ_FAIL(BZ_E_INVALID, "graph capture: model has no KV cache (use bz_decode_graph_capture_ssm)");
  if (kv->layers != m->cfg.n_layers || kv->n_kv != m->cfg.n_kv_heads || kv->hd != m->cfg.head_dim) BZ_FAIL(BZ_E_INVALID, "graph capture: cache does not match the model");
  BZ_HIP(hipSetDevice(m->dev->id));
  bz_decode_graph* g = new bz_decode_graph();
  bz_dev_retain(m->dev); g->dev = m->dev;
  g->m = m; g->pkv = kv; g->max_blocks = max_blocks; g->capacity = std::min(max_blocks * kv->block_size, m->cfg.max_seq_len);
  BZ_HIP(hipMalloc(&g->block_table, (size_t)max_blocks * 4));
  BZ_HIP(hipMemset(g->block_table, 0, (size_t)max_blocks * 4));
  int rc = graph_capture_common(g, view_of(kv, g->block_table, nullptr));
  if (rc != BZ_OK) { bz_decode_graph_free(g); return rc; }
  *out = g;
  return BZ_OK;
  BZ_API_END
}
extern "C" int bz_decode_graph_capture_ssm(bz_model* m, bz_ssm_state* st, bz_decode_graph** out) {
  BZ_API_BEGIN
  if (!m || !m->finalized || !out) BZ_FAIL(BZ_E_INVALID, "graph capture: bad argument");
  std::lock_guard<std::recursive_mutex> lock__(m->mu);
  BZ_TRY(check_ssm(m, st));
  BZ_HIP(hipSetDevice(m->dev->id));
  bz_decode_graph* g = new bz_decode_graph();
  bz_dev_retain(m->dev); g->dev = m->dev;
  g->m = m; g->ssm = st;
  int rc = graph_capture_common(g, KvView{});
  if (rc != BZ_OK) { bz_decode_graph_free(g); return rc; }
  *out = g;
  return BZ_OK;
  BZ_API_END
}
struct bz_batch_graph {
  bz_model* m = nullptr; bz_device* dev = nullptr; bz_paged_kv* kv = nullptr;
  hipGraph_t graph = nullptr; hipGraphExec_t exec = nullptr;
  int N = 0, max_blocks = 0, capacity = 0;
  long long* tok = nullptr; long long* next = nullptr; int* pos = nullptr; int* slot = nullptr; int* table = nullptr; int* step = nullptr;
  bz_tensor* logits = nullptr;
  long long* log = nullptr;
  std::vector<int> host_pos;
  long long replays = 0;
  static const int LOGCAP = 1024;
};
extern "C" int bz_decode_batch_graph_free(bz_batch_graph* g) {
  BZ_API_BEGIN
  if (!g) return BZ_OK;
  if (g->dev) hipSetDevice(g->dev->id);
  hipDeviceSynchronize();
  if (g->exec) hipGraphExecDestroy(g->exec);
  if (g->graph) hipGraphDestroy(g->graph);
  for (void* p : {(void*)g->tok, (void*)g->next, (void*)g->pos, (void*)g->slot, (void*)g->table, (void*)g->step}) if (p) hipFree(p);
  if (g->log) hipHostFree(g->log);
  if (g->logits) bz_tensor_free(g->logits);
  if (g->dev) bz_dev_release(g->dev);
  delete g;
  return BZ_OK;
  BZ_API_END
}
extern "C" int bz_decode_batch_graph_capture(bz_model* m, bz_paged_kv* kv, int N, int max_blocks, bz_batch_graph** out) {
  BZ_API_BEGIN
  if (!m || !m->finalized || !kv || !out || N < 2 || N > 512 || max_blocks <= 0) BZ_FAIL(BZ_E_INVALID, "batch graph capture: bad argument (2 <= N <= 512)");
// ... 46 lines not shown
  BZ_API_END
}
extern "C" int bz_decode_batch_graph_seed(bz_batch_graph* g, const int64_t* tokens, const int32_t* seq_lens, const int32_t* block_table) {
  BZ_API_BEGIN
  if (!g || !tokens || !seq_lens || !block_table) BZ_FAIL(BZ_E_INVALID, "batch graph seed: null argument");
  std::lock_guard<std::recursive_mutex> lock__(g->m->mu);
  std::vector<int> p0(g->N);
  for (int i = 0; i < g->N; i++) {
    if (seq_lens[i] <= 0 || seq_lens[i] > g->capacity) BZ_FAIL(BZ_E_INVALID, "batch graph seed: sequence %d has length %d (capacity %d)", i, seq_lens[i], g->capacity);
    p0[i] = seq_lens[i] - 2;
    g->host_pos[i] = seq_lens[i] - 2;
  }
  hipStream_t st = g->m->dev->stream;
  int z = 0;
  BZ_HIP(hipMemcpyAsync(g->next, tokens, (size_t)g->N * 8, hipMemcpyHostToDevice, st));
  BZ_HIP(hipMemcpyAsync(g->pos, p0.data(), (size_t)g->N * 4, hipMemcpyHostToDevice, st));
  BZ_HIP(hipMemcpyAsync(g->table, block_table, (size_t)g->N * g->max_blocks * 4, hipMemcpyHostToDevice, st));
  BZ_HIP(hipMemcpyAsync(g->step, &z, 4, hipMemcpyHostToDevice, st));
  BZ_HIP(hipStreamSynchronize(st));
  g->replays = 0;
  return BZ_OK;
  BZ_API_END
}
extern "C" int bz_decode_batch_graph_set_block_table(bz_batch_graph* g, const int32_t* block_table) {
  BZ_API_BEGIN
  if (!g || !block_table) BZ_FAIL(BZ_E_INVALID, "batch graph set_block_table: null argument");
  hipStream_t st = g->m->dev->stream;
  BZ_HIP(hipMemcpyAsync(g->table, block_table, (size_t)g->N * g->max_blocks * 4, hipMemcpyHostToDevice, st));
  BZ_HIP(hipStreamSynchronize(st));
  return BZ_OK;
  BZ_API_END
}
extern "C" int bz_decode_batch_graph_replay(bz_batch_graph* g) {
  BZ_API_BEGIN
  if (!g || !g->exec) BZ_FAIL(BZ_E_INVALID, "null batch graph");
  std::lock_guard<std::recursive_mutex> lock__(g->m->mu);
  int maxlen = 0;
  for (int i = 0; i < g->N; i++) {
    if (g->host_pos[i] + 1 >= g->capacity) BZ_FAIL(BZ_E_INVALID, "batch graph replay: sequence %d would reach position %d, beyond the capacity %d the step was captured over", i, g->host_pos[i] + 1, g->capacity);
    maxlen = std::max(maxlen, g->host_pos[i] + 2);
  }
  BZ_HIP(hipGraphLaunch(g->exec, g->m->dev->stream));
  for (int i = 0; i < g->N; i++) g->host_pos[i]++;
  if (g->kv->seq_len < maxlen) g->kv->seq_len = maxlen;
  g->replays++;
  return BZ_OK;
  BZ_API_END
}
extern "C" int bz_decode_batch_graph_read_tokens(bz_batch_graph* g, int64_t step, int64_t* tokens_out) {
  BZ_API_BEGIN
  if (!g || !tokens_out || step < 0 || step >= g->replays || step < g->replays - bz_batch_graph::LOGCAP) BZ_FAIL(BZ_E_INVALID, "batch graph read_tokens: step out of range");
  BZ_HIP(hipStreamSynchronize(g->m->dev->stream));
  const long long* row = g->log + (size_t)(step % bz_batch_graph::LOGCAP) * g->N;
  for (int i = 0; i < g->N; i++) tokens_out[i] = row[i];
  return BZ_OK;
  BZ_API_END
}
extern "C" int bz_decode_batch_graph_logits(bz_batch_graph* g, bz_tensor** logits_out) {
  BZ_API_BEGIN
  if (!g || !logits_out) BZ_FAIL(BZ_E_INVALID, "batch graph logits: null argument");
  *logits_out = g->logits;
  return BZ_OK;
  BZ_API_END
}

extern "C" int bz_decode_graph_set_block_table(bz_decode_graph* g, const int32_t* bt, int n) {
  BZ_API_BEGIN
  if (!g || !g->block_table || !bt || n < 0 || n > g->max_blocks) BZ_FAIL(BZ_E_INVALID, "set_block_table: bad argument");
  BZ_HIP(hipMemcpyAsync(g->block_table, bt, (size_t)n * 4, hipMemcpyHostToDevice, g->m->dev->stream));
  BZ_HIP(hipStreamSynchronize(g->m->dev->stream));
  return BZ_OK;
  BZ_API_END
}
extern "C" int bz_decode_graph_seed(bz_decode_graph* g, int64_t token, int position) {
  BZ_API_BEGIN
  if (!g) BZ_FAIL(BZ_E_INVALID, "null graph");
  const int limit = g->ssm ? INT32_MAX : std::min(g->capacity, g->m->cfg.max_seq_len);
  if (position < 0 || position >= limit) BZ_FAIL(BZ_E_INVALID, "graph seed: position %d out of range (cache capacity %d, max_seq_len %d)", position, g->capacity, g->m->cfg.max_seq_len);
  hipStream_t st = g->m->dev->stream;
  long long t = token; int p = position, z = 0;
  BZ_HIP(hipMemcpyAsync(g->tok_buf, &t, 8, hipMemcpyHostToDevice, st));
  BZ_HIP(hipMemcpyAsync(g->pos, &p, 4, hipMemcpyHostToDevice, st));
  BZ_HIP(hipMemcpyAsync(g->step, &z, 4, hipMemcpyHostToDevice, st));
  BZ_HIP(hipStreamSynchronize(st));
  g->replays = 0; g->seed_pos = position;
  return BZ_OK;
  BZ_API_END
}
extern "C" int bz_decode_graph_replay(bz_decode_graph* g) {
  BZ_API_BEGIN
  if (!g || !g->exec) BZ_FAIL(BZ_E_INVALID, "null graph");
  std::lock_guard<std::recursive_mutex> lock__(g->m->mu);
  hipStream_t st = g->m->dev->stream;
  hipGraphExec_t exec = g->exec;
  if (!g->ssm && g->seed_pos + g->replays >= (long long)std::min(g->capacity, g->m->cfg.max_seq_len))
    BZ_FAIL(BZ_E_INVALID, "graph replay: position %lld is beyond the cache capacity %d / max_seq_len %d the step was captured over", g->seed_pos + g->replays, g->capacity,
            g->m->cfg.max_seq_len);
  if (!g->ssm && g->capacity > 0 && att_positions_for((int)(g->seed_pos + g->replays + 1)) > 0) {
    if (!g->exec_long) {
      BZ_HIP(hipSetDevice(g->m->dev->id));
      BZ_TRY(graph_capture_variant(g, g->capacity, &g->graph_long, &g->exec_long));
    }
    exec = g->exec_long;
  }
  BZ_HIP(hipGraphLaunch(exec, st));
  BZ_HIP(hipEventRecord(g->evs[g->replays % g->evs.size()], st));
  g->replays++;
  if (g->kv) g->kv->seq_len++;
  if (g->pkv) g->pkv->seq_len++;
  return BZ_OK;
  BZ_API_END
}
extern "C" int bz_decode_graph_read_token(bz_decode_graph* g, int64_t step, int64_t* out) {
  BZ_API_BEGIN
  if (!g || !out || step < 0 || step >= g->replays) BZ_FAIL(BZ_E_INVALID, "read_token: step %lld of %lld", (long long)step, g ? g->replays : 0);
  if (g->replays - step > (long long)g->evs.size()) BZ_HIP(hipStreamSynchronize(g->m->dev->stream));
  else BZ_HIP(hipEventSynchronize(g->evs[step % g->evs.size()]));
  if (g->replays - step > bz_decode_graph::LOGCAP) BZ_FAIL(BZ_E_INVALID, "read_token: step %lld fell out of the token log", (long long)step);
  *out = ((volatile long long*)g->tok_log)[step % bz_decode_graph::LOGCAP];
  return BZ_OK;
  BZ_API_END
}
extern "C" int bz_decode_graph_read_logits(bz_decode_graph* g, float* host, size_t n) {
  BZ_API_BEGIN
  if (!g || !host || n > (size_t)g->m->cfg.vocab) BZ_FAIL(BZ_E_INVALID, "read_logits: bad argument");
  BZ_HIP(hipMemcpyAsync(host, g->m->logits, n * 4, hipMemcpyDeviceToHost, g->m->dev->stream));
  BZ_HIP(hipStreamSynchronize(g->m->dev->stream));
  return BZ_OK;
  BZ_API_END
}
extern "C" int bz_decode_graph_free(bz_decode_graph* g) {
  BZ_API_BEGIN
  if (!g) return BZ_OK;
  hipStreamSynchronize(g->dev->stream);
  for (auto ev : g->evs) hipEventDestroy(ev);
  if (g->exec) hipGraphExecDestroy(g->exec);
  if (g->graph) hipGraphDestroy(g->graph);
  if (g->exec_long) hipGraphExecDestroy(g->exec_long);
  if (g->graph_long) hipGraphDestroy(g->graph_long);
  if (g->tok_buf) hipFree(g->tok_buf);
  if (g->pos) hipFree(g->pos);
  if (g->step) hipFree(g->step);
  if (g->block_table) hipFree(g->block_table);
  if (g->tok_log) hipHostFree(g->tok_log);
  bz_dev_release(g->dev);
  delete g;
  return BZ_OK;
  BZ_API_END
}

static int penalty_window(const std::vector<uint32_t>& hist, int last_n, std::vector<int64_t>& ids, std::vector<int32_t>& cnts) {
  size_t b = 0;
  if (last_n > 0 && (size_t)last_n < hist.size()) b = hist.size() - last_n;
  ids.clear(); cnts.clear();
  for (size_t i = b; i < hist.size(); i++) {
    size_t j = 0;
    for (; j < ids.size(); j++) if (ids[j] == (int64_t)hist[i]) { cnts[j]++; break; }
    if (j == ids.size()) { ids.push_back(hist[i]); cnts.push_back(1); }
  }
  return (int)ids.size();
}

extern "C" int bz_generate(bz_model* m, const int64_t* prompt, int n_prompt, const bz_gen_config* gc, int64_t* out_tokens, bz_gen_stats* stats) { return bz_generate_grammar(m, prompt, n_prompt, gc, nullptr, nullptr, nullptr, 0, out_tokens, stats); }

extern "C" int bz_generate_grammar(bz_model* m, const int64_t* prompt, int n_prompt, const bz_gen_config* gc, bz_grammar* g, const uint8_t* vocab_bytes,
                                   const int64_t* offsets, int64_t V, int64_t* out_tokens, bz_gen_stats* stats) {
  BZ_API_BEGIN
  if (!m || !m->finalized || !prompt || !gc || !out_tokens) BZ_FAIL(BZ_E_INVALID, "generate: bad argument");
  if (g && (!offsets || V != m->cfg.vocab)) BZ_FAIL(BZ_E_INVALID, "generate: a grammar needs the bytes of all %d tokens of the model's vocabulary (got V = %lld)", m->cfg.vocab, (long long)V);
  if (n_prompt <= 0) { if (stats) memset(stats, 0, sizeof(*stats)); return BZ_OK; }
  const bz_model_config& c = m->cfg;
  bz_device* dev = m->dev;
  BZ_HIP(hipSetDevice(dev->id));
  for (int i = 0; i < n_prompt; i++) if (prompt[i] < 0 || prompt[i] >= c.vocab) BZ_FAIL(BZ_E_INVALID, "generate: prompt token %lld out of vocab", (long long)prompt[i]);
  int max_tokens = std::min(gc->max_tokens, std::max(0, c.max_seq_len - n_prompt));
  const bool greedy = gc->temperature == 0.0f;
  if (gc->use_graph && !greedy) BZ_FAIL(BZ_E_INVALID, "generate: graph mode is greedy-only (cli/run.rs:144-157)");
  if (gc->use_graph && (gc->dry_multiplier > 0.f || gc->typical_p > 0.f || gc->n_logit_bias > 0 || gc->mirostat_mode >= 2))
    BZ_FAIL(BZ_E_INVALID, "generate: graph mode has no host-side sampler options");
  if (gc->n_logit_bias < 0 || (gc->n_logit_bias > 0 && (!gc->logit_bias_ids || !gc->logit_bias_vals))) BZ_FAIL(BZ_E_INVALID, "generate: bad logit_bias arrays");
  const int kv_dt = c.act_dtype;
  int rc = BZ_OK;
  bz_tensor *t_prompt = nullptr, *t_logits = nullptr, *t_tok = nullptr, *t_ids = nullptr, *t_cnts = nullptr, *t_slot = nullptr, *t_bt = nullptr;
  bz_kv* kv = nullptr; bz_paged_kv* pkv = nullptr; bz_decode_graph* graph = nullptr; bz_ssm_state* ssm = nullptr; bz_mirostat* mstate = nullptr;
  bz_device_grammar* dg = nullptr;
  const bool use_graph = gc->use_graph && !g;
  const bool mamba = c.arch == BZ_ARCH_MAMBA2;
  auto mamba_arch = [](const bz_model_config& cc) { return cc.arch == BZ_ARCH_MAMBA2; };
  std::vector<uint32_t> history(prompt, prompt + n_prompt);
  std::vector<int32_t> bt;
  int n_out = 0, finish = 0;
  auto T0 = std::chrono::steady_clock::now();
  auto T1 = T0;
  std::vector<std::chrono::steady_clock::time_point> tok_t;
  tok_t.reserve((size_t)std::max(max_tokens, 0));
  const char* backend = mamba_arch(c) ? "mamba2" : (gc->paged ? "paged" : "contiguous");
  BZ_TRACE("phase=\"prefill_start\" backend=\"%s\" prompt_tokens=%d", backend, n_prompt);
  int64_t sh1[1] = {1}, shp[1] = {n_prompt}, shv[2] = {1, c.vocab}, sh64[1] = {4096};
#define GEN_TRY(x) do { rc = (x); if (rc != BZ_OK) goto done; } while (0)
  GEN_TRY(bz_tensor_from_host(dev, BZ_I64, shp, 1, prompt, &t_prompt));
  GEN_TRY(bz_tensor_zeros(dev, BZ_F32, shv, 2, &t_logits));
  GEN_TRY(bz_tensor_zeros(dev, BZ_I64, sh1, 1, &t_tok));
  GEN_TRY(bz_tensor_zeros(dev, BZ_I64, sh64, 1, &t_ids));
  GEN_TRY(bz_tensor_zeros(dev, BZ_I32, sh64, 1, &t_cnts));
  if (g) GEN_TRY(bz_grammar_to_device(dev, g, vocab_bytes, offsets, V, &dg));
  if (mamba) {
    GEN_TRY(bz_ssm_state_create(m, 1, c.act_dtype, &ssm));
    GEN_TRY(bz_forward_ssm(m, t_prompt, n_prompt, ssm, t_logits, 0));
  } else if (gc->paged) {
    const int bs = gc->block_size > 0 ? gc->block_size : 16;
    const int total = n_prompt + max_tokens;
    const int nblocks = (total + bs - 1) / bs + 4;
    GEN_TRY(bz_paged_kv_create(dev, c.n_layers, nblocks, bs, c.n_kv_heads, c.head_dim, kv_dt, &pkv));
    bt.resize(nblocks);
    for (int i = 0; i < nblocks; i++) bt[i] = i;
    int64_t shb[1] = {nblocks}, shs[1] = {n_prompt};
    GEN_TRY(bz_tensor_from_host(dev, BZ_I32, shb, 1, bt.data(), &t_bt));
    std::vector<int32_t> slots(n_prompt);
    for (int i = 0; i < n_prompt; i++) slots[i] = bt[i / bs] * bs + i % bs;
    GEN_TRY(bz_tensor_from_host(dev, BZ_I32, shs, 1, slots.data(), &t_slot));
    GEN_TRY(bz_forward_paged(m, t_prompt, n_prompt, pkv, t_slot, t_bt, nblocks, n_prompt, 0, t_logits, 0));
  } else {
    const int cap = std::min(n_prompt + max_tokens, c.max_seq_len);
    GEN_TRY(bz_kv_create(dev, c.n_layers, 1, c.n_kv_heads, std::max(cap, 1), c.max_seq_len, c.head_dim, kv_dt, &kv));
    GEN_TRY(bz_forward_kv(m, t_prompt, n_prompt, kv, 0, t_logits, 0));
// ... 431 lines not shown
```

blazr_amd/csrc/bz_internal.h:

```cpp
#pragma once
#include <hip/hip_runtime.h>
#include <hip/hip_ext.h>
#include <hip/hip_fp16.h>
#include <stdint.h>
#include <string>
#include <vector>
#include <unordered_map>
#include <memory>
#include <mutex>
#include <new>
#include <stdexcept>
#include "../../include/blazr_hip.h"

void bz_set_error(const char* fmt, ...);
#define BZ_FAIL(code, ...) do { bz_set_error(__VA_ARGS__); return (code); } while (0)
#define BZ_HIP(expr) do { hipError_t e__ = (expr); if (e__ != hipSuccess) { \
  bz_set_error("%s failed: %s (%s:%d)", #expr, hipGetErrorString(e__), __FILE__, __LINE__); return BZ_E_HIP; } } while (0)
#define BZ_TRY(expr) do { int rc__ = (expr); if (rc__ != BZ_OK) return rc__; } while (0)
#define BZ_API_BEGIN try {
#define BZ_API_END } catch (const std::bad_alloc&) { bz_set_error("out of host memory (std::bad_alloc)"); return BZ_E_OOM; } \
  catch (const std::length_error& e__) { bz_set_error("size out of range (%s)", e__.what()); return BZ_E_OOM; }             \
  catch (const std::exception& e__) { bz_set_error("internal error: %s", e__.what()); return BZ_E_INVALID; }               \
  catch (...) { bz_set_error("internal error: unknown C++ exception"); return BZ_E_INVALID; }

// ... 50 lines not shown
  int refs = 1;
};
void bz_dev_retain(bz_device* d);
void bz_dev_release(bz_device* d);

struct bz_tensor {
  bz_device* dev = nullptr;
  void* ptr = nullptr;
  int dtype = BZ_F32;
  std::vector<int64_t> shape;
  size_t nbytes = 0;
  bool owned = true;
};

struct bz_kv {
  bz_device* dev = nullptr;
  int layers = 0, batch = 1, n_kv = 0, cap = 0, max_len = 0, hd = 0, dtype = BZ_F16;
  int seq_len = 0;
  void* k = nullptr; void* v = nullptr;
};

struct bz_ssm_state {
  bz_device* dev = nullptr;
  int layers = 0, n_heads = 0, head_dim = 0, d_state = 0, conv_dim = 0, kc = 0, dtype = BZ_BF16;
  void* ssm = nullptr;
  float* conv = nullptr;
};

struct bz_paged_kv {
  bz_device* dev = nullptr;
  int layers = 0, num_blocks = 0, block_size = 16, n_kv = 0, hd = 0, dtype = BZ_F16;
  int seq_len = 0;
  void* k = nullptr; void* v = nullptr;
};

struct KvView {
  void* k; void* v;
  int dtype, hd, n_kv;
  int paged;
  long long layer_stride;
  int cap;
  int bs;
  const int* block_table;
  const int* slot;
};

size_t bz_dtype_size(int dtype);

struct BzTimingRec { const char* label; double bytes; hipEvent_t e0, e1; };
struct BzTimingSink { std::vector<BzTimingRec> recs; };
void bzk_set_timing_sink(BzTimingSink* s);
BzTimingSink* bzk_timing_sink();
#define BZ_LAUNCH(label, bytes, kernel, grid, block, smem, stream, ...)                                              \
  do {                                                                                                               \
    BzTimingSink* sink__ = bzk_timing_sink();                                                                        \
    if (sink__) {                                                                                                    \
      hipEvent_t e0__, e1__;                                                                                         \
      BZ_HIP(hipEventCreate(&e0__));                                                                                 \
      BZ_HIP(hipEventCreate(&e1__));                                                                                 \
      hipExtLaunchKernelGGL(kernel, grid, block, smem, stream, e0__, e1__, 0, __VA_ARGS__);                          \
      sink__->recs.push_back(BzTimingRec{label, (double)(bytes), e0__, e1__});                                       \
    } else {                                                                                                         \
      hipLaunchKernelGGL(kernel, grid, block, smem, stream, __VA_ARGS__);                                            \
    }                                                                                                                \
  } while (0)

struct ConvShift { float* cs; VSrc src; int x_off, ch0, n, kc; };

struct MoeSlots { const int* sel; long long expert_stride; int n; long long src_stride; long long acc_stride; int acc_slots; };

struct RouteArgs { const long long* lg; int E, top_k, n_shared; float routed_scale; int norm_topk; int* sel_out; float* w_out; };

struct GqMix { const uint4* Wq6; const uint2* Wh6; const uint4* Hd6; const __half* Dd6; int nt4; };
bool bzk_gq_mix_ok(const LinearDev& A, const LinearDev& B, const Pro& pro);
int bzk_gemv_gq_mix(hipStream_t s, const LinearDev& A, const LinearDev& B, const Pro& pro, const struct GemvOut& out);

struct GemvOut {
  long long* acc;
  float* direct;
  long long* zero_buf;
  int zero_n;
  float* amax_val; int* amax_idx;
  ConvShift shift;
};

int bzk_gemv(hipStream_t s, const LinearDev& L, const Pro& pro, const GemvOut& out, int act);
int bzk_gemv_rows_blocks(const LinearDev& L);
bool bzk_gemm_q4g_rows_ok(const LinearDev& L);
bool bzk_gemm_q4g_mfma_ok(const LinearDev& L, int xdt, int rows);
int bzk_gemm_q4g_mfma(hipStream_t s, const LinearDev& L, const void* x16, int S, int act, float* y, float* ws = nullptr, size_t ws_bytes = 0);
int bzk_gemm_q4g_rows(hipStream_t s, const LinearDev& L, int xdt, const void* x16, int rows, int act, long long* acc, float* y);
int bzk_rows_choose_sk(int N, int K);
bool bzk_mlp_gq_fusable(const LinearDev& gu, const LinearDev& dn, int H, int I, int act);
int bzk_mlp_gq(hipStream_t s, const LinearDev& gu, const LinearDev& dn, int H, int I, const Pro& pro, long long* acc, long long* zero_buf, int zero_n);
int bzk_repack_down_slabs(hipStream_t s, const void* w, int H, int I, void* out);
bool bzk_mlp_dense_fusable(const LinearDev& gu, const LinearDev& dn, const void* down_slabs, int H, int I, int act);
int bzk_mlp_dense(hipStream_t s, const LinearDev& gu, const LinearDev& dn, const void* down_slabs, int H, int I, const Pro& pro, long long* acc, long long* zero_buf, int zero_n);
bool bzk_mlp_fusable(const LinearDev& gu, const LinearDev& dn, int H, int I);
int bzk_mlp_q4g(hipStream_t s, const LinearDev& gu, const LinearDev& dn, int H, int I, const Pro& pro, long long* acc, long long* zero_buf, int zero_n);
int bzk_repack_awq(hipStream_t s, const uint32_t* d_qweight, const float* d_scales, const float* d_zeros, int N, int K, int gs,
                   void* w_out, void* s_out, void* z_out);
int bzk_repack_gptq(hipStream_t s, const uint32_t* d_qweight, const float* d_scales, const uint32_t* d_qzeros, const int* d_perm,
                    const int* d_gidx, int N, int K, int gs, void* w_out, void* s_out, void* z_out);
int bzk_dequant_q4g(hipStream_t s, const LinearDev& L, float* out );
int bzk_dequant_rows(hipStream_t s, const LinearDev& L, float* out);
int bzk_repack_gq(hipStream_t s, int kind, const void* raw, int N, int K, void* wq, void* wh, void* hd, void* dd);
int bzk_dequant_gq(hipStream_t s, const LinearDev& L, float* out);
bool bzk_gq_split_ok(const LinearDev& L);
int bzk_gq_absmax(hipStream_t s, const LinearDev& L, unsigned* amax);
int bzk_gq_wscale(hipStream_t s, const unsigned* amax, float* wscale);
int bzk_gq_split3(hipStream_t s, const LinearDev& L, const float* wscale, void* out, int row0);
bool bzk_gemm_q4g_i8_ok(const LinearDev& L, int xdt);
size_t bzk_pf_quant_i8_bytes(int S, int K, size_t* par_off);
int bzk_pf_quant_i8(hipStream_t s, const void* x16, int S, int K, void* xq);
int bzk_gemm_q4g_i8(hipStream_t s, const LinearDev& L, const void* xq, int S, int act, float* y);
int bzk_pf_split3(hipStream_t s, const float* x, int S, int K, void* xs, float* rscale, const float* wscale);
int bzk_argmax_partials(hipStream_t s, const float* v, long long n, float* pval, int* pidx, int nb);
int bzk_embed(hipStream_t s, const void* table, int tdt, int gg, const long long* tok, int H, int act, float* h_out, const int* pos = nullptr,
              const float* cos_t = nullptr, const float* sin_t = nullptr, int half = 0, float* rope_cur = nullptr);
int bzk_rope_row(hipStream_t s, const int* pos, const float* cos_t, const float* sin_t, int half, float* rope_cur);
int bzk_fix_to_f32(hipStream_t s, const long long* acc, int n, int act, float* out);
int bzk_zero64(hipStream_t s, long long* p, int n);

struct AttnArgs {
  VSrc qkv;
  const float* cos_t; const float* sin_t;
  const float* rope_cur;
  int interleaved;
  const int* pos;
  int nq, nkv, hd, act;
  KvView kv; int layer;
  float* out;
  long long* zero_buf; int zero_n;
  int q_only;
};
int bzk_attn_decode(hipStream_t s, const AttnArgs& a);
int bzk_attn_oproj_slices(const AttnArgs& a, const LinearDev& L);
int bzk_attn_oproj(hipStream_t s, const AttnArgs& a, const LinearDev& L, long long* acc);
int bzk_attn_split_slices(int positions);
int bzk_attn_split_ok(const AttnArgs& a);
size_t bzk_attn_split_ws_bytes(int nq);
int bzk_attn_split(hipStream_t s, const AttnArgs& a, int nsplit, float* ws);
int bzk_attn_merge(hipStream_t s, const AttnArgs& a, const float* ws, int nsplit);
int bzk_attn_merge_oproj_ok(const AttnArgs& a, const LinearDev& L);
int bzk_attn_merge_oproj(hipStream_t s, const AttnArgs& a, const float* ws, int nsplit, const LinearDev& L, long long* acc);
int bzk_kv_insert(hipStream_t s, const KvView& kv, int layer, const float* k, const float* v, const int* pos, int nkv, int hd);
int bzk_kv_read(hipStream_t s, const KvView& kv, int layer, int kvh, int which, int len, float* out);


struct FinalArgs {
  const float* pval; const int* pidx; int nparts;
  long long* tok_out;
  long long* tok_log; int* step;
  int logcap;
  int* pos;
  long long* zero_buf; int zero_n;
};
int bzk_argmax_final(hipStream_t s, const FinalArgs& a);
int bzk_logits_to_token(hipStream_t s, const float* logits, long long V, const long long* ids, const int* cnts, int n, float rp,
                        float fp, float pp, float temperature, int top_k, float top_p, float min_p, unsigned long long seed,
                        float* scratch , long long* tok_out);
int bzk_rms_norm(hipStream_t s, const float* x, const float* prev, const float* w, int rows, int n, float eps, int act, float* y,
                 float* h_out);
int bzk_rope(hipStream_t s, float* x, int S, int nh, int hd, int position, const float* cos_t, const float* sin_t, int interleaved,
             int act);
int bzk_silu_mul(hipStream_t s, const float* g, const float* u, long long n, int act, float* y);

struct MlaArgs {
  VSrc qkv;
  const float* kv_norm; float eps;
  const void* wkvb; int wdt;
  const float* cos_t; const float* sin_t; const int* pos;
  int n_heads, rank, nope, rope, vdim, act;
  KvView kv; int layer;
  float* out;
  float scale;
  int batch; int pos0; long long q_stride; long long out_stride;
  const float* kva;
  float* ws; int nsplit;
};
int bzk_mla_nsplit(int n_heads);
bool bzk_mla_x_ok(const MlaArgs& a, int max_len);
int bzk_mla_attn_x(hipStream_t s, const MlaArgs& a, int max_len, double* wsd, float* scw, float* mxw);
int bzk_mla_append_rows(hipStream_t s, const float* kva, long long stride, int S, const float* kv_norm, float eps, int rank, int rope, const float* cos_t, const float* sin_t,
                        int pos0, int act, const KvView& kv, int layer);
int bzk_moe_route_rows(hipStream_t s, int dt, const void* x16, int S, int H, const void* wr, int wdt, int E, int top_k, float routed_scale, int norm_topk, int* sel, float* wsel);
int bzk_moe_plan_rows(hipStream_t s, const int* sel, int S, int top_k, int E, int* counts, int* offsets, int* row_of, int* tok_of);
int bzk_moe_gather_rows(hipStream_t s, const void* x16, const int* tok_of, int rows, int H, void* xg16);
int bzk_moe_combine_rows(hipStream_t s, const float* ye, const int* row_of, const float* wsel, const float* ysh, int S, int top_k, int H, int act, float* out);
struct MoeGemvArgs {
  const void* w; long long expert_stride;
  const int* sel;
  int N, K;
  long long src_stride;
  float* out; long long out_stride;
  long long* acc; long long acc_stride; int acc_slots;
  RouteArgs route;
};
int bzk_moe_gemv(hipStream_t s, const MoeGemvArgs& g, int wdt, int n_slots, const Pro& pro, int act, bool split, double bytes);
int bzk_mla_attn(hipStream_t s, const MlaArgs& a, int max_len);
int bzk_moe_router(hipStream_t s, const Pro& pro, const void* wr, int wdt, int E, int top_k, int n_shared, float routed_scale, int norm_topk,
                   float* xn_out, int* sel, float* wsel, float* lg_glob, unsigned* counter);
int bzk_moe_combine(hipStream_t s, long long* acc, const float* wsel, int top_k, int has_shared, int H, int act, float* out, long long* zero_buf = nullptr, int zero_n = 0);
bool bzk_moe_rows2_ok(int wdt, int K);

int bzk_gemm_nt(hipStream_t s, int dt, const void* x16, const void* w, const float* bias, int S, int N, int K, int act, float* y, float* ws = nullptr, size_t ws_bytes = 0,
                const float* rscale = nullptr);
int bzk_gemm_nt_grouped(hipStream_t s, int dt, const void* x16, const void* w, long long w_stride, int G, const int* g_off, const int* g_cnt, int max_rows, long long total_rows,
                        int N, int K, int act, float* y);
int bzk_pf_cvt16(hipStream_t s, int dt, const float* x, size_t n, void* y);
int bzk_pf_embed(hipStream_t s, const void* table, int tdt, int gg, const long long* tok, int S, int H, int act, float* out);
int bzk_pf_norm(hipStream_t s, int dt, float* hbuf, const float* prev, const float* w, int S, int H, float eps, int act, void* x16);
int bzk_pf_rope_kv(hipStream_t s, float* qkv, int S, int nq, int nkv, int hd, const float* cos_t, const float* sin_t, int interleaved, int pos0, int act,
                   const KvView& kv, int layer, const int* slots, const int* row_pos = nullptr);
int bzk_pf_attn(hipStream_t s, int dt, const float* qkv, int S, int nq, int nkv, int hd, int pos0, int act, const KvView& kv, int layer, void* out16,
                const int* row_pos = nullptr, int table_stride = 0, int max_len = 0, bool exact = false);
struct BzSsmScan {
  const float* xbc; int conv_dim; const float* zx; int ld; int dt_off; const float* dt_bias; const float* A_log; const float* D; void* state;
  int n_heads, head_dim, d_state, n_groups, d_inner, act, S; float* y; float* vss;
};
bool bzk_ssm_scan_ok(int head_dim, int d_state, int n_groups, int kc);
int bzk_ssm_scan_pieces(int head_dim);
int bzk_pf_conv(hipStream_t s, const float* zx, int ld, int x_off, int conv_dim, int kc, const float* w, const float* b, float* conv_state, int S, int act, float* out);
int bzk_ssm_scan(hipStream_t s, const BzSsmScan& b, int state_dtype);
int bzk_pf_gnorm(hipStream_t s, int dt, const float* v, const float* vss, const float* w, int S, int DI, int G, int NH, float eps, int act, void* x16);
int bzk_pf_silu(hipStream_t s, int dt, const float* gu, int S, int I, int act, void* a16);
size_t bzk_pf_attn_smem(int nq, int nkv, int hd, int len, bool exact = false);
bool bzk_pf_attn_mfma_ok(int hd, int rep);

int bzk_sample(hipStream_t s, void** ws, const float* logits, long long V, const long long* ids, const int* cnts, int n, float rp, float fp, float pp,
               float temperature, int top_k, float top_p, float min_p, unsigned long long seed, long long* tok_out);
int bzk_sample_free(void* ws);

struct SsmArgs {
  VSrc zx;
  int z_off, x_off, dt_off;
  const float* conv_w; const float* conv_b; float* conv_state; int conv_kernel;
  const float* dt_bias; const float* A_log; const float* D;
  void* state; int sdt;
  int n_heads, head_dim, d_state, n_groups, d_inner, act;
  float* y;
// ... 122 lines not shown
```

blazr_amd/csrc/bz_kernels.hip:

```cpp
#include "bz_internal.h"
#include "bz_dev.h"
#include "bz_ggml.h"
#include <math.h>

#include <hip/hip_ext.h>

static thread_local BzTimingSink* g_sink = nullptr;
void bzk_set_timing_sink(BzTimingSink* s) { g_sink = s; }
BzTimingSink* bzk_timing_sink() { return g_sink; }

__device__ __forceinline__ float block_sum256(float v, float* red) {
  v = wave_sum(v);
  if ((threadIdx.x & 63) == 0) red[threadIdx.x >> 6] = v;
  __syncthreads();
  float t = (red[0] + red[1]) + (red[2] + red[3]);
  __syncthreads();
  return t;
}

template <int NTH>
__device__ __forceinline__ void zero_duty(long long* zb, int zn) {
  if (zb)
    for (int i = blockIdx.x * NTH + threadIdx.x; i < zn; i += gridDim.x * NTH) zb[i] = 0;
}
// ... 1500 lines not shown
      if (WDT == BZ_F16) {
        w[2 * i] = __half2float(__ushort_as_half((unsigned short)(u[i] & 0xffffu)));
        w[2 * i + 1] = __half2float(__ushort_as_half((unsigned short)(u[i] >> 16)));
      } else {
        w[2 * i] = __uint_as_float(u[i] << 16);
        w[2 * i + 1] = __uint_as_float(u[i] & 0xffff0000u);
      }
    }
  }
}

template <int WDT> struct RowPiece { uint4 a; };
template <> struct RowPiece<BZ_F32> { uint4 a, b; };
template <int WDT>
__device__ __forceinline__ RowPiece<WDT> piece_load(const void* W, size_t elem_off) {
  RowPiece<WDT> p;
  if constexpr (WDT == BZ_F32) { p.a = ldnt((const uint4*)((const float*)W + elem_off)); p.b = ldnt((const uint4*)((const float*)W + elem_off + 4)); }
  else p.a = ldnt((const uint4*)((const unsigned short*)W + elem_off));
  return p;
}
template <int WDT>
__device__ __forceinline__ float piece_dot(const RowPiece<WDT>& p, const float4& xa, const float4& xb) {
  float w[8];
  if constexpr (WDT == BZ_F32) {
    w[0] = __uint_as_float(p.a.x); w[1] = __uint_as_float(p.a.y); w[2] = __uint_as_float(p.a.z); w[3] = __uint_as_float(p.a.w);
    w[4] = __uint_as_float(p.b.x); w[5] = __uint_as_float(p.b.y); w[6] = __uint_as_float(p.b.z); w[7] = __uint_as_float(p.b.w);
  } else {
    const unsigned u[4] = {p.a.x, p.a.y, p.a.z, p.a.w};
#pragma unroll
    for (int i = 0; i < 4; i++) {
      if constexpr (WDT == BZ_F16) {
        w[2 * i] = __half2float(__ushort_as_half((unsigned short)(u[i] & 0xffffu)));
        w[2 * i + 1] = __half2float(__ushort_as_half((unsigned short)(u[i] >> 16)));
      } else {
        w[2 * i] = __uint_as_float(u[i] << 16);
        w[2 * i + 1] = __uint_as_float(u[i] & 0xffff0000u);
      }
    }
  }
  return w[0] * xa.x + w[1] * xa.y + w[2] * xa.z + w[3] * xa.w + w[4] * xb.x + w[5] * xb.y + w[6] * xb.z + w[7] * xb.w;
}
template <int WDT>
__device__ __forceinline__ double piece_dot_d(const RowPiece<WDT>& p, const double (&x)[8], double acc) {
  float w[8];
  if constexpr (WDT == BZ_F32) {
    w[0] = __uint_as_float(p.a.x); w[1] = __uint_as_float(p.a.y); w[2] = __uint_as_float(p.a.z); w[3] = __uint_as_float(p.a.w);
    w[4] = __uint_as_float(p.b.x); w[5] = __uint_as_float(p.b.y); w[6] = __uint_as_float(p.b.z); w[7] = __uint_as_float(p.b.w);
  } else {
    const unsigned u[4] = {p.a.x, p.a.y, p.a.z, p.a.w};
#pragma unroll
    for (int i = 0; i < 4; i++) {
      if constexpr (WDT == BZ_F16) {
        w[2 * i] = __half2float(__ushort_as_half((unsigned short)(u[i] & 0xffffu)));
        w[2 * i + 1] = __half2float(__ushort_as_half((unsigned short)(u[i] >> 16)));
      } else {
        w[2 * i] = __uint_as_float(u[i] << 16);
        w[2 * i + 1] = __uint_as_float(u[i] & 0xffff0000u);
      }
    }
  }
#pragma unroll
  for (int e = 0; e < 8; e++) acc = fma((double)w[e], x[e], acc);
  return acc;
}
template <int WDT>
__device__ __forceinline__ double piece_dot_x(const RowPiece<WDT>& p, const float4& xa, const float4& xb, double acc) {
  static_assert(WDT == BZ_F16 || WDT == BZ_BF16, "exact f32 products need 16-bit operands");
  const unsigned u[4] = {p.a.x, p.a.y, p.a.z, p.a.w};
  const float x[8] = {xa.x, xa.y, xa.z, xa.w, xb.x, xb.y, xb.z, xb.w};
#pragma unroll
  for (int i = 0; i < 4; i++) {
    float w0, w1;
    if constexpr (WDT == BZ_F16) { w0 = __half2float(__ushort_as_half((unsigned short)(u[i] & 0xffffu))); w1 = __half2float(__ushort_as_half((unsigned short)(u[i] >> 16))); }
    else { w0 = __uint_as_float(u[i] << 16); w1 = __uint_as_float(u[i] & 0xffff0000u); }
    acc += (double)__fmul_rn(w0, x[2 * i]);
    acc += (double)__fmul_rn(w1, x[2 * i + 1]);
  }
  return acc;
}
__device__ __forceinline__ void x8_to_d(const float4& xa, const float4& xb, double (&x)[8]) {
  x[0] = (double)xa.x; x[1] = (double)xa.y; x[2] = (double)xa.z; x[3] = (double)xa.w; x[4] = (double)xb.x; x[5] = (double)xb.y; x[6] = (double)xb.z; x[7] = (double)xb.w;
}

template <int WDT, bool SPLIT>
__device__ __forceinline__ void rows_body(const void* __restrict__ W, const float* __restrict__ bias, int N, int K, int rows_per_wg, const Pro& pro,
                                          float* out, int act, float* pval, int* pidx, long long* zero_buf, int zero_n, int SK, long long* accbuf,
                                          const int bid) {
  extern __shared__ __attribute__((aligned(16))) char smem[];
  const int KP = (K + 511) & ~511;
  float* xs = (float*)smem;
  float* red = xs + KP;
  const int wave = __builtin_amdgcn_readfirstlane(threadIdx.x >> 6), lane = threadIdx.x & 63;
  const int rpw = rows_per_wg >> 2;
  const int rb = SPLIT ? bid / SK : bid, ks = SPLIT ? bid % SK : 0;
  const int rbeg = rb * rows_per_wg + wave * rpw;
  const int rend = min(rbeg + rpw, N);
  const int KCall = KP >> 9, KCs = SPLIT ? (KCall + SK - 1) / SK : KCall;
  const int kc0 = ks * KCs;
  const int KC = max(min(KCs, KCall - kc0), 1);
  const int kb = kc0 * 512;
  const int ngroups = rend > rbeg ? (rend - rbeg + 3) >> 2 : 0;
  const int nsteps = ngroups * KC;
  struct Stage { RowPiece<WDT> p[4]; };
  int ir = min(rbeg, N - 1), ikc = 0, ist = 0;
  auto issue = [&](Stage& S) {
    const int k = kb + ikc * 512 + lane * 8;
    const int ko = k < K ? k : 0;
#pragma unroll
    for (int rr = 0; rr < 4; rr++) S.p[rr] = piece_load<WDT>(W, (size_t)min(ir + rr, N - 1) * K + ko);
    if (ist + 1 < nsteps) { ist++; if (++ikc == KC) { ikc = 0; ir += 4; } }
  };
  Stage s0, s1, s2;
  issue(s0);
  issue(s1);
  __builtin_amdgcn_sched_barrier(0);
  zero_duty<256>(zero_buf, zero_n);
  const float4* xs4;
  if (!SPLIT || pro.mode == PRO_GATED) {
    for (int i = K + threadIdx.x; i < KP; i += 256) xs[xs_pos<true>(i)] = 0.f;
    build_x_simple<true>(pro, 0, K, xs, red, bid == 0);
    xs4 = (const float4*)(xs + kb);
  } else {
    const int KR = max(min(K - kb, KC * 512), 0);
    for (int i = KR + threadIdx.x; i < KC * 512; i += 256) xs[xs_pos<true>(i)] = 0.f;
    build_x_simple<true>(pro, kb, KR, xs, red, bid == 0);
    xs4 = (const float4*)xs;
  }
  float bestv = -INFINITY; int besti = 0x7fffffff;
  double acc[4] = {0.0, 0.0, 0.0, 0.0};
  int cr = rbeg, ckc = 0, cst = 0;
  auto consume = [&](const Stage& S) {
    if (cst >= nsteps) return;
    cst++;
    const float4 xa = xs4[ckc * 128 + lane], xb = xs4[ckc * 128 + 64 + lane];
    if constexpr (WDT == BZ_F32) {
      double xd[8];
      x8_to_d(xa, xb, xd);
#pragma unroll
      for (int rr = 0; rr < 4; rr++) acc[rr] = piece_dot_d<WDT>(S.p[rr], xd, acc[rr]);
    } else {
#pragma unroll
      for (int rr = 0; rr < 4; rr++) acc[rr] = piece_dot_x<WDT>(S.p[rr], xa, xb, acc[rr]);
    }
    if (++ckc == KC) {
      ckc = 0;
#pragma unroll
      for (int rr = 0; rr < 4; rr++) {
        const double vd = wave_sum_d(acc[rr]);
        acc[rr] = 0.0;
        if (cr + rr < rend) {
          if (SPLIT) {
            if (lane == 0) atomicAdd((unsigned long long*)(accbuf + cr + rr), (unsigned long long)d2fix(vd + ((bias && ks == 0) ? (double)bias[cr + rr] : 0.0), pro.act));
          } else {
            float v = (float)vd;
            if (bias) v += bias[cr + rr];
            v = round_act(v, act);
            if (lane == 0) out[cr + rr] = v;
            if (v > bestv) { bestv = v; besti = cr + rr; }
          }
        }
      }
      cr += 4;
    }
  };
  for (int st = 0; st < nsteps; st += 3) {
    issue(s2); consume(s0);
    issue(s0); consume(s1);
    issue(s1); consume(s2);
  }
  if (!SPLIT && pval) {
    float* bv = red + 4; int* bi = (int*)(red + 8);
    if (lane == 0) { bv[wave] = bestv; bi[wave] = besti; }
    __syncthreads();
    if (threadIdx.x == 0) {
      float v = bv[0]; int ix = bi[0];
      for (int w2 = 1; w2 < 4; w2++) if (bv[w2] > v) { v = bv[w2]; ix = bi[w2]; }
      pval[bid] = v; pidx[bid] = ix;
    }
  }
}

template <int WDT, bool SPLIT>
__global__ __launch_bounds__(256) void k_gemv_rows(const void* __restrict__ W, const float* __restrict__ bias, int N, int K,
                                                   int rows_per_wg, Pro pro, float* out, int act, float* pval, int* pidx,
                                                   long long* zero_buf, int zero_n, int SK, long long* accbuf) {
  rows_body<WDT, SPLIT>(W, bias, N, K, rows_per_wg, pro, out, act, pval, pidx, zero_buf, zero_n, SK, accbuf, blockIdx.x);
}

__device__ __forceinline__ float wave_sum4(float v0, float v1, float v2, float v3) {
  bz_u2_t r = __builtin_amdgcn_permlane32_swap(__float_as_uint(v0), __float_as_uint(v1), false, false);
  const float s01 = __uint_as_float(r.x) + __uint_as_float(r.y);
  r = __builtin_amdgcn_permlane32_swap(__float_as_uint(v2), __float_as_uint(v3), false, false);
  const float s23 = __uint_as_float(r.x) + __uint_as_float(r.y);
  r = __builtin_amdgcn_permlane16_swap(__float_as_uint(s01), __float_as_uint(s23), false, false);
  return grp_reduce<16, OpAdd>(__uint_as_float(r.x) + __uint_as_float(r.y));
}
__device__ __forceinline__ void swap32_d(double a, double b, double& ra, double& rb) {
  const long long ba = __double_as_longlong(a), bb = __double_as_longlong(b);
  const bz_u2_t lo = __builtin_amdgcn_permlane32_swap((unsigned)ba, (unsigned)bb, false, false), hi = __builtin_amdgcn_permlane32_swap((unsigned)(ba >> 32), (unsigned)(bb >> 32), false, false);
  ra = __longlong_as_double(((long long)hi.x << 32) | lo.x); rb = __longlong_as_double(((long long)hi.y << 32) | lo.y);
}
__device__ __forceinline__ void swap16_d(double a, double b, double& ra, double& rb) {
  const long long ba = __double_as_longlong(a), bb = __double_as_longlong(b);
  const bz_u2_t lo = __builtin_amdgcn_permlane16_swap((unsigned)ba, (unsigned)bb, false, false), hi = __builtin_amdgcn_permlane16_swap((unsigned)(ba >> 32), (unsigned)(bb >> 32), false, false);
  ra = __longlong_as_double(((long long)hi.x << 32) | lo.x); rb = __longlong_as_double(((long long)hi.y << 32) | lo.y);
}
__device__ __forceinline__ double wave_sum4_d(double v0, double v1, double v2, double v3) {
  double a, b;
  swap32_d(v0, v1, a, b); const double s01 = a + b;
  swap32_d(v2, v3, a, b); const double s23 = a + b;
  swap16_d(s01, s23, a, b);
  return grp_sum_d<16>(a + b);
}

__device__ __forceinline__ void conv_shift_one(const ConvShift& c, int i, int act) {
  const int ch = c.ch0 + i;
  float* cs = c.cs + (size_t)ch * (c.kc - 1);
  const float xr = vsrc_get(c.src, c.x_off + ch, act);
  for (int j = 0; j + 1 < c.kc - 1; j++) cs[j] = cs[j + 1];
  cs[c.kc - 2] = xr;
}
__global__ void k_conv_shift(ConvShift c, int act) {
  const int i = blockIdx.x * blockDim.x + threadIdx.x;
  if (i < c.n) conv_shift_one(c, i, act);
}

__device__ void moe_softmax_topk(const float* lg, int E, int top_k, int n_shared, float routed_scale, int norm_topk, int* sel, float* wsel, int lane);
template <int WDT, int MODE, bool FIX, int ROUTE = 0, bool EX = false>
__global__ __launch_bounds__(ROUTE ? 832 : 768) void k_gemv_rows2(const void* __restrict__ W, const float* __restrict__ bias, int N, int K, Pro pro,
                                                    long long* __restrict__ acc, long long* zero_buf, int zero_n, ConvShift shift, MoeSlots slots, RouteArgs route) {
  constexpr int NR = ROUTE ? 2 : 1;
  __shared__ __attribute__((aligned(16))) float xs[NR * 1024];
  __shared__ double dred[4];
  __shared__ float grs[4][8];
  __shared__ unsigned cnt[4];
  __shared__ float lgs[ROUTE ? 1024 : 1];
  __shared__ int ssel[ROUTE ? 128 : 1];
  __shared__ float swgt[ROUTE ? 128 : 1];
  const int tid = threadIdx.x, lane = tid & 63;
  const int wave = __builtin_amdgcn_readfirstlane(tid >> 6);
  const int NRG = (N + 3) >> 2, KCall = (K + 511) >> 9;
  int u0[NR], u1[NR], ub[NR], kcA[NR], slA[NR], kcB[NR], slB[NR], sbase[NR];
  bool hasB[NR];
#pragma unroll
  for (int r = 0; r < NR; r++) {
    sbase[r] = ROUTE ? (r == 0 ? route.top_k : 0) : 0;
    const int nsl = ROUTE ? (r == 0 ? route.n_shared : route.top_k) : slots.n;
    const int nseg = KCall * nsl;
    const long long U = (long long)NRG * nseg;
    u0[r] = (int)(U * blockIdx.x / gridDim.x); u1[r] = (int)(U * (blockIdx.x + 1) / gridDim.x);
    const int segA = u0[r] / NRG, segB = min(segA + 1, max(nseg - 1, 0));
    hasB[r] = segA + 1 < nseg;
    const int nd = max(nsl, 1);
    kcA[r] = segA / nd; slA[r] = segA - kcA[r] * nd; kcB[r] = segB / nd; slB[r] = segB - kcB[r] * nd;
    ub[r] = (segA + 1) * NRG;
  }
  const int act = pro.act;
  if (tid == 0) { cnt[0] = 0; cnt[1] = 0; cnt[2] = 0; cnt[3] = 0; }
  if (ROUTE && wave == 12) {
    __builtin_amdgcn_s_setprio(3);
    for (int j = lane; j < route.E; j += 64) lgs[j] = fix2f(route.lg[j], pro.act);
    __syncthreads();
    __builtin_amdgcn_s_waitcnt(0xc07f);
    moe_softmax_topk(lgs, route.E, route.top_k, route.n_shared, route.routed_scale, route.norm_topk, ssel, swgt, lane);
    __builtin_amdgcn_s_waitcnt(0xc07f);
    if (lane == 0) atomicAdd(&cnt[2], 1u);
    if (blockIdx.x == 0)
      for (int j = lane; j < route.top_k + route.n_shared; j += 64) { route.sel_out[j] = ssel[j]; route.w_out[j] = swgt[j]; }
    return;
// ... 565 lines not shown
    const unsigned hb = (wh[(((size_t)nt * (K >> 8) + (k >> 8)) * 64 + lane) * 8 + (kc & 7)] >> (8 * (r & 3) + (r >> 2))) & 1u;
    const float d = __half2float(__ushort_as_half((unsigned short)(hw[0] & 0xffffu))), dmin = __half2float(__ushort_as_half((unsigned short)(hw[0] >> 16)));
    int sc, mn;
    q4k_scale_min(hw, (k & 255) >> 5, sc, mn);
    return __fsub_rn(__fmul_rn(__fmul_rn(d, (float)sc), (float)(lo | (hb << 4))), __fmul_rn(dmin, (float)mn));
  }
  const int F = r >> 2;
  const unsigned hword = wh[(((size_t)nt * (K >> 5) + kc) * 64 + lane) * 2 + (F >> 2)];
  const unsigned hi2 = (hword >> (8 * (r & 3) + 2 * (F & 3))) & 3u;
  const int q = (int)(lo | (hi2 << 4)) - 32;
  const int si = (k & 255) >> 4;
  const int sc = (int)(signed char)((hw[si >> 2] >> (8 * (si & 3))) & 255u);
  return __half2float(dd[((size_t)nt * (K >> 8) + (k >> 8)) * 64 + lane]) * (float)sc * (float)q;
}
__global__ void k_dequant_gq(int fmt, const uint32_t* wq, const uint32_t* wh, const uint32_t* hd, const __half* dd, int N, int K, float* out) {
  const size_t total = (size_t)N * K;
  for (size_t idx = (size_t)blockIdx.x * blockDim.x + threadIdx.x; idx < total; idx += (size_t)gridDim.x * blockDim.x)
    out[idx] = gq_elem(fmt, wq, wh, hd, dd, K, (int)(idx / (size_t)K), (int)(idx % (size_t)K));
}
static int gq_fmt(const LinearDev& L) { return gq_fmt_of(L.kind); }
int bzk_dequant_gq(hipStream_t s, const LinearDev& L, float* out) {
  hipLaunchKernelGGL(k_dequant_gq, dim3(2048), dim3(256), 0, s, gq_fmt(L), (const uint32_t*)L.w, (const uint32_t*)L.zeros, (const uint32_t*)L.hdr,
                     (const __half*)L.scales, L.N, L.K, out);
  BZ_HIP(hipGetLastError());
  return BZ_OK;
}

__global__ void k_gq_absmax(int fmt, const uint32_t* wq, const uint32_t* wh, const uint32_t* hd, const __half* dd, int N, int K, unsigned* amax) {
  const size_t total = (size_t)N * K;
  float am = 0.f;
  for (size_t idx = (size_t)blockIdx.x * blockDim.x + threadIdx.x; idx < total; idx += (size_t)gridDim.x * blockDim.x)
    am = fmaxf(am, fabsf(gq_elem(fmt, wq, wh, hd, dd, K, (int)(idx / (size_t)K), (int)(idx % (size_t)K))));
  am = wave_max(am);
  if ((threadIdx.x & 63) == 0) atomicMax(amax, __float_as_uint(am));
}
__global__ void k_gq_wscale(const unsigned* amax, float* wscale) {
  const unsigned eb = (*amax >> 23) & 255u;
  *wscale = (eb == 0u || eb == 255u || eb > 240u || eb < 20u) ? 1.0f : __uint_as_float((127u + 13u + 127u - eb) << 23);
}
__global__ __launch_bounds__(256) void k_gq_split3(int fmt, const uint32_t* wq, const uint32_t* wh, const uint32_t* hd, const __half* dd, int N, int K, const float* wscale,
                                                   unsigned short* out, int row0) {
  const size_t total = (size_t)N * (K >> 3);
  const float sc = *wscale;
  for (size_t idx = (size_t)blockIdx.x * blockDim.x + threadIdx.x; idx < total; idx += (size_t)gridDim.x * blockDim.x) {
    const int n = (int)(idx / (size_t)(K >> 3)), k0 = (int)(idx % (size_t)(K >> 3)) * 8;
    unsigned short a[8], b[8], c[8];
#pragma unroll
    for (int e = 0; e < 8; e++) {
      const float vs = gq_elem(fmt, wq, wh, hd, dd, K, n, k0 + e) * sc;
      const __half h = f16_cvt(vs);
      const float hf = __half2float(h), l = vs - hf;
      a[e] = __half_as_ushort(h); b[e] = __half_as_ushort(f16_cvt(hf * (1.0f / 2048.0f))); c[e] = __half_as_ushort(f16_cvt(l * 2048.0f));
    }
    unsigned short* o = out + (size_t)(row0 + n) * 3 * K + k0;
    *(uint4*)o = make_uint4(a[0] | ((unsigned)a[1] << 16), a[2] | ((unsigned)a[3] << 16), a[4] | ((unsigned)a[5] << 16), a[6] | ((unsigned)a[7] << 16));
    *(uint4*)(o + K) = make_uint4(b[0] | ((unsigned)b[1] << 16), b[2] | ((unsigned)b[3] << 16), b[4] | ((unsigned)b[5] << 16), b[6] | ((unsigned)b[7] << 16));
    *(uint4*)(o + 2 * K) = make_uint4(c[0] | ((unsigned)c[1] << 16), c[2] | ((unsigned)c[3] << 16), c[4] | ((unsigned)c[5] << 16), c[6] | ((unsigned)c[7] << 16));
  }
}
bool bzk_gq_split_ok(const LinearDev& L) {
  return (L.kind == LK_Q80 || L.kind == LK_Q4K || L.kind == LK_Q5K || L.kind == LK_Q6K || L.kind == LK_Q40 || L.kind == LK_Q41 || L.kind == LK_Q50 ||
          L.kind == LK_Q51) && L.K % 64 == 0 && L.N % 64 == 0;
}
int bzk_gq_absmax(hipStream_t s, const LinearDev& L, unsigned* amax) {
  hipLaunchKernelGGL(k_gq_absmax, dim3(2048), dim3(256), 0, s, gq_fmt(L), (const uint32_t*)L.w, (const uint32_t*)L.zeros, (const uint32_t*)L.hdr, (const __half*)L.scales, L.N, L.K, amax);
  BZ_HIP(hipGetLastError());
  return BZ_OK;
}
int bzk_gq_wscale(hipStream_t s, const unsigned* amax, float* wscale) {
  hipLaunchKernelGGL(k_gq_wscale, dim3(1), dim3(1), 0, s, amax, wscale);
  BZ_HIP(hipGetLastError());
  return BZ_OK;
}
int bzk_gq_split3(hipStream_t s, const LinearDev& L, const float* wscale, void* out, int row0) {
  hipLaunchKernelGGL(k_gq_split3, dim3(4096), dim3(256), 0, s, gq_fmt(L), (const uint32_t*)L.w, (const uint32_t*)L.zeros, (const uint32_t*)L.hdr, (const __half*)L.scales, L.N, L.K, wscale,
                     (unsigned short*)out, row0);
  BZ_HIP(hipGetLastError());
  return BZ_OK;
}

int bzk_argmax_partials(hipStream_t s, const float* v, long long n, float* pval, int* pidx, int nb);

int bzk_gemv(hipStream_t s, const LinearDev& L, const Pro& pro, const GemvOut& out, int act) {
  if (L.kind == LK_Q4G && act == BZ_F16 && bzk_gemv_slim_ok(L, pro)) {
    if (!out.acc) BZ_FAIL(BZ_E_INVALID, "int4 gemv needs a fixed-point accumulator");
    const int nks = L.K / 256, ntg = (L.N / 64 + 7) / 8;
#define LAUNCH_SLIM(FIX, NJ) BZ_LAUNCH("gemv_q4g<norm>", L.algo_bytes, (k_gemv_q4g_slim<FIX, NJ, BZ_F16>), dim3(nks * ntg), dim3(768), 0, s, (const uint4*)L.w, \
    (const __half*)L.scales, (const unsigned char*)L.zeros, L.bias, L.N, L.K, pro, out.acc, out.zero_buf, out.zero_n)
#define LAUNCH_SLIM_NJ(FIX) do { if (L.K == 2048) LAUNCH_SLIM(FIX, 1); else if (L.K == 4096) LAUNCH_SLIM(FIX, 2); else LAUNCH_SLIM(FIX, 4); } while (0)
    if (pro.src.fix) LAUNCH_SLIM_NJ(1); else LAUNCH_SLIM_NJ(0);
#undef LAUNCH_SLIM_NJ
#undef LAUNCH_SLIM
    BZ_HIP(hipGetLastError());
    return BZ_OK;
  }
  if (L.kind == LK_Q4G) {
    if (!out.acc) BZ_FAIL(BZ_E_INVALID, "q4g gemv needs a fixed-point accumulator");
    const int G = L.K / 128, GW = L.gw;
    const int nst = (L.N + 255) / 256;
    const int grid = nst * (G / GW);
    const size_t smem = q4g_smem(GW);
    const int maxj = pro.mode == PRO_NORM ? (pro.H + 1023) / 1024 : 1;
    if (GW > 16) BZ_FAIL(BZ_E_INVALID, "q4g gemv: %d groups per workgroup (max 16)", GW);
#define LAUNCH_Q4G(MODE, FIX, MJ, NPF) BZ_LAUNCH(MODE == PRO_NORM ? "gemv_q4g<norm>" : (MODE == PRO_SILU ? "gemv_q4g<silu>" : "gemv_q4g<plain>"), \
    L.algo_bytes, (k_gemv_q4g<MODE, FIX, MJ, NPF>), dim3(grid), dim3(256), smem, s, (const uint4*)L.w,                      \
    (const __half*)L.scales, (const unsigned char*)L.zeros, L.bias, L.N, L.K, GW, nst, pro, out.acc, out.zero_buf, out.zero_n)
#define LAUNCH_Q4G_N(MODE, FIX, MJ) do { if (GW == 1) LAUNCH_Q4G(MODE, FIX, MJ, 1); else if (L.npf >= 4 && GW >= 4) LAUNCH_Q4G(MODE, FIX, MJ, 4); \
                                          else LAUNCH_Q4G(MODE, FIX, MJ, 2); } while (0)
#define LAUNCH_Q4G_F(MODE, MJ) do { if (pro.src.fix) LAUNCH_Q4G_N(MODE, 1, MJ); else LAUNCH_Q4G_N(MODE, 0, MJ); } while (0)
    if (pro.mode == PRO_PLAIN) LAUNCH_Q4G_F(PRO_PLAIN, 1);
    else if (pro.mode == PRO_SILU) LAUNCH_Q4G_F(PRO_SILU, 1);
    else if (maxj <= 1) LAUNCH_Q4G_F(PRO_NORM, 1);
    else if (maxj <= 2) LAUNCH_Q4G_F(PRO_NORM, 2);
    else if (maxj <= 4) LAUNCH_Q4G_F(PRO_NORM, 4);
    else if (maxj <= 8) LAUNCH_Q4G_F(PRO_NORM, 8);
    else BZ_FAIL(BZ_E_UNSUPPORTED, "hidden size %d too large for the fused norm prologue", pro.H);
#undef LAUNCH_Q4G_N
#undef LAUNCH_Q4G_F
#undef LAUNCH_Q4G
    BZ_HIP(hipGetLastError());
    return BZ_OK;
  }
  if (L.kind == LK_ROWS && bzk_rows2_ok(L, pro, out)) {
    const long long U = (long long)((L.N + 3) / 4) * ((L.K + 511) / 512);
    const int KC = (L.K + 511) / 512;
    const int nb = (int)std::max<long long>(std::min<long long>(256, U), KC);
    const char* lbl = pro.mode == PRO_NORM ? "gemv_rows2<norm>" : pro.mode == PRO_GATED2 ? "gemv_rows2<gated>" : pro.mode == PRO_SILU ? "gemv_rows2<silu>" : "gemv_rows2";
#define LAUNCH_R2(DT, MODE, FIX) do { if (pro.f32_sums) LAUNCH_R2X(DT, MODE, FIX, false); else LAUNCH_R2X(DT, MODE, FIX, true); } while (0)
#define LAUNCH_R2X(DT, MODE, FIX, EX_) BZ_LAUNCH(lbl, L.algo_bytes, (k_gemv_rows2<DT, MODE, FIX, 0, EX_>), dim3(nb), dim3(768), 0, s, (const void*)L.w, L.bias, L.N, L.K, pro, \
    out.acc, out.zero_buf, out.zero_n, out.shift, MoeSlots{nullptr, 0, 1, 0, 0, 1}, RouteArgs{})
#define LAUNCH_R2_F(DT, MODE) do { if (pro.src.fix) LAUNCH_R2(DT, MODE, true); else LAUNCH_R2(DT, MODE, false); } while (0)
#define LAUNCH_R2_M(DT) do { if (pro.mode == PRO_NORM) LAUNCH_R2_F(DT, PRO_NORM); else if (pro.mode == PRO_SILU) LAUNCH_R2_F(DT, PRO_SILU); \
    else if (pro.mode == PRO_GATED2) LAUNCH_R2(DT, PRO_GATED2, false); else LAUNCH_R2_F(DT, PRO_PLAIN); } while (0)
    if (L.wdt == BZ_F16) LAUNCH_R2_M(BZ_F16); else LAUNCH_R2_M(BZ_BF16);
#undef LAUNCH_R2_M
#undef LAUNCH_R2_F
#undef LAUNCH_R2
#undef LAUNCH_R2X
    BZ_HIP(hipGetLastError());
    return BZ_OK;
  }
  if (L.kind == LK_ROWS) {
    const int SK = L.sk > 1 ? L.sk : 1;
    if (out.shift.cs) { hipLaunchKernelGGL(k_conv_shift, dim3((out.shift.n + 255) / 256), dim3(256), 0, s, out.shift, act); BZ_HIP(hipGetLastError()); }
    if (SK == 1 && !out.direct) BZ_FAIL(BZ_E_INVALID, "rows gemv needs a direct output");
    if (SK > 1 && (!out.acc || out.amax_val)) BZ_FAIL(BZ_E_INVALID, "split-K rows gemv needs a fixed-point accumulator");
    const int rpw = SK > 1 ? 16 : rows_per_wg_for(L.N);
    const int grid = ((L.N + rpw - 1) / rpw) * SK;
    const int KP = (L.K + 511) & ~511;
    const size_t smem = (size_t)KP * 4 + 64;
    if (smem > 160 * 1024) BZ_FAIL(BZ_E_UNSUPPORTED, "K=%d too large for the rows GEMV", L.K);
    const char* lbl = out.amax_val ? "gemv_rows<lm_head+argmax>" : pro.mode == PRO_NORM ? "gemv_rows<norm>" : (pro.mode == PRO_GATED || pro.mode == PRO_GATED2) ? "gemv_rows<gated>"
                      : pro.mode == PRO_SILU ? "gemv_rows<silu>" : "gemv_rows";
#define LAUNCH_ROWS1(DT, SP) BZ_LAUNCH(lbl, L.algo_bytes, (k_gemv_rows<DT, SP>), dim3(grid), \
    dim3(256), smem, s, (const void*)L.w, L.bias, L.N, L.K, rpw, pro, out.direct, act, out.amax_val, out.amax_idx, out.zero_buf, out.zero_n, SK, out.acc)
#define LAUNCH_ROWS(DT) do { if (SK > 1) LAUNCH_ROWS1(DT, true); else LAUNCH_ROWS1(DT, false); } while (0)
    if (L.wdt == BZ_F16) LAUNCH_ROWS(BZ_F16); else if (L.wdt == BZ_BF16) LAUNCH_ROWS(BZ_BF16); else LAUNCH_ROWS(BZ_F32);
#undef LAUNCH_ROWS
#undef LAUNCH_ROWS1
    BZ_HIP(hipGetLastError());
    return BZ_OK;
  }
  if (bzk_gq_slim_ok(L, pro)) {
    if (!out.acc) BZ_FAIL(BZ_E_INVALID, "block-quant gemv needs a fixed-point accumulator");
    const int nsb = L.K / 256, ntg = (L.N / 64 + 7) / 8;
    const char* label = L.kind == LK_Q4K ? "gemv_q4_K<slim>" : L.kind == LK_Q5K ? "gemv_q5_K<slim>" : L.kind == LK_Q6K ? "gemv_q6_K<slim>"
                      : L.kind == LK_Q40 ? "gemv_q4_0<slim>" : L.kind == LK_Q41 ? "gemv_q4_1<slim>" : L.kind == LK_Q50 ? "gemv_q5_0<slim>" : "gemv_q5_1<slim>";
#define LAUNCH_GQS(FMT, MODE, FIX, NJ) BZ_LAUNCH(label, L.algo_bytes, (k_gemv_gq_slim<FMT, MODE, FIX, NJ>), dim3(nsb * ntg), dim3(512), 0, s, (const uint4*)L.w, \
    (const uint2*)L.zeros, (const uint4*)L.hdr, (const __half*)L.scales, L.bias, L.N, L.K, pro, out.acc, out.zero_buf, out.zero_n, GqMix{})
#define LAUNCH_GQS_NJ(FMT, FIX) do { if (pro.mode == PRO_SILU) LAUNCH_GQS(FMT, PRO_SILU, FIX, 1); else if (L.K == 2048) LAUNCH_GQS(FMT, PRO_NORM, FIX, 1); \
    else if (L.K == 4096) LAUNCH_GQS(FMT, PRO_NORM, FIX, 2); else LAUNCH_GQS(FMT, PRO_NORM, FIX, 4); } while (0)
#define LAUNCH_GQS_F(FMT) do { if (pro.src.fix) LAUNCH_GQS_NJ(FMT, 1); else LAUNCH_GQS_NJ(FMT, 0); } while (0)
    if (L.kind == LK_Q4K) LAUNCH_GQS_F(GQ_Q4K); else if (L.kind == LK_Q5K) LAUNCH_GQS_F(GQ_Q5K); else if (L.kind == LK_Q6K) LAUNCH_GQS_F(GQ_Q6K);
    else if (L.kind == LK_Q40) LAUNCH_GQS_F(GQ_Q40); else if (L.kind == LK_Q41) LAUNCH_GQS_F(GQ_Q41); else if (L.kind == LK_Q50) LAUNCH_GQS_F(GQ_Q50);
    else LAUNCH_GQS_F(GQ_Q51);
#undef LAUNCH_GQS_F
#undef LAUNCH_GQS_NJ
#undef LAUNCH_GQS
    BZ_HIP(hipGetLastError());
    return BZ_OK;
  }
  if (L.kind == LK_Q80 || L.kind == LK_Q4K || L.kind == LK_Q5K || L.kind == LK_Q6K || L.kind == LK_Q40 || L.kind == LK_Q41 || L.kind == LK_Q50 || L.kind == LK_Q51) {
    if (!out.acc) BZ_FAIL(BZ_E_INVALID, "block-quant gemv needs a fixed-point accumulator");
    const int SB = L.K / 256, SBW = L.gw;
    if (SBW <= 0 || SB % SBW || SBW > 8) BZ_FAIL(BZ_E_INVALID, "block-quant gemv: bad k-slice %d of %d superblocks", SBW, SB);
    const int nst = (L.N + 255) / 256;
    const int grid = nst * (SB / SBW);
    const size_t smem = gq_smem(SBW);
    const int maxj = pro.mode == PRO_NORM ? (pro.H + 1023) / 1024 : 1;
    const char* label = L.kind == LK_Q80 ? "gemv_q8_0" : L.kind == LK_Q4K ? "gemv_q4_K" : L.kind == LK_Q5K ? "gemv_q5_K" : L.kind == LK_Q6K ? "gemv_q6_K"
                      : L.kind == LK_Q40 ? "gemv_q4_0" : L.kind == LK_Q41 ? "gemv_q4_1" : L.kind == LK_Q50 ? "gemv_q5_0" : "gemv_q5_1";
#define LAUNCH_GQ(FMT, MODE, FIX, MJ) BZ_LAUNCH(label, L.algo_bytes, (k_gemv_gq<FMT, MODE, FIX, MJ>), dim3(grid), dim3(256), smem, s, (const uint4*)L.w, \
    (const uint2*)L.zeros, (const uint4*)L.hdr, (const __half*)L.scales, L.bias, L.N, L.K, SBW, nst, pro, out.acc, out.zero_buf, out.zero_n)
#define LAUNCH_GQ_F(FMT, MODE, MJ) do { if (pro.src.fix) LAUNCH_GQ(FMT, MODE, 1, MJ); else LAUNCH_GQ(FMT, MODE, 0, MJ); } while (0)
#define LAUNCH_GQ_M(FMT) do { if (pro.mode == PRO_PLAIN) LAUNCH_GQ_F(FMT, PRO_PLAIN, 1); else if (pro.mode == PRO_SILU) LAUNCH_GQ_F(FMT, PRO_SILU, 1); \
    else if (maxj <= 1) LAUNCH_GQ_F(FMT, PRO_NORM, 1); else if (maxj <= 2) LAUNCH_GQ_F(FMT, PRO_NORM, 2); else if (maxj <= 4) LAUNCH_GQ_F(FMT, PRO_NORM, 4); \
    else if (maxj <= 8) LAUNCH_GQ_F(FMT, PRO_NORM, 8); else BZ_FAIL(BZ_E_UNSUPPORTED, "hidden size %d too large for the fused norm prologue", pro.H); } while (0)
    if (L.kind == LK_Q80) LAUNCH_GQ_M(GQ_Q80); else if (L.kind == LK_Q4K) LAUNCH_GQ_M(GQ_Q4K); else if (L.kind == LK_Q5K) LAUNCH_GQ_M(GQ_Q5K);
    else if (L.kind == LK_Q6K) LAUNCH_GQ_M(GQ_Q6K); else if (L.kind == LK_Q40) LAUNCH_GQ_M(GQ_Q40); else if (L.kind == LK_Q41) LAUNCH_GQ_M(GQ_Q41);
    else if (L.kind == LK_Q50) LAUNCH_GQ_M(GQ_Q50); else LAUNCH_GQ_M(GQ_Q51);
#undef LAUNCH_GQ_M
#undef LAUNCH_GQ_F
#undef LAUNCH_GQ
    BZ_HIP(hipGetLastError());
    return BZ_OK;
  }
  BZ_FAIL(BZ_E_UNSUPPORTED, "gemv: linear kind %d not implemented", L.kind);
}

__device__ __forceinline__ unsigned awq_nib(const uint32_t* qw, int N, int k, int n) {
  const unsigned sh = ((n & 1) << 4) | ((n & 7) >> 1 << 2);
  return (qw[(size_t)k * (N >> 3) + (n >> 3)] >> sh) & 15u;
}

__global__ void k_repack_awq(const uint32_t* qw, const float* sc, const float* zf, int N, int K, int gs, uint32_t* wout, __half* sout,
                             unsigned char* zout) {
  const size_t total = (size_t)N * (K >> 3);
  const int G = K / gs;
  for (size_t idx = (size_t)blockIdx.x * blockDim.x + threadIdx.x; idx < total; idx += (size_t)gridDim.x * blockDim.x) {
    const int j = idx & 3;
    const int lane = (idx >> 2) & 63;
    const size_t t = idx >> 8;
    const int kc = (int)(t % (size_t)(K >> 5));
    const int nt = (int)(t / (size_t)(K >> 5));
    const int n = nt * 64 + lane;
    unsigned word = 0;
#pragma unroll
    for (int bb = 0; bb < 4; bb++) {
      const int k1 = kc * 32 + j * 8 + bb;
      const unsigned q1 = awq_nib(qw, N, k1, n), q2 = awq_nib(qw, N, k1 + 4, n);
      word |= ((q1 ^ 8u) | ((q2 ^ 8u) << 4)) << (8 * bb);
    }
    wout[idx] = word;
  }
// ... 1167 lines not shown
#define LAUNCH_SP_P(DT) do { if (a.kv.paged) LAUNCH_SP_R(DT, 1); else LAUNCH_SP_R(DT, 0); } while (0)
  if (a.kv.dtype == BZ_F16) LAUNCH_SP_P(BZ_F16); else LAUNCH_SP_P(BZ_BF16);
#undef LAUNCH_SP_P
#undef LAUNCH_SP_R
#undef LAUNCH_SP
  BZ_HIP(hipGetLastError());
  return BZ_OK;
}
int bzk_attn_merge(hipStream_t s, const AttnArgs& a, const float* ws, int nsplit) {
  BZ_LAUNCH("attn_merge", 0.0, k_attn_merge, dim3(a.nq), dim3(512), 0, s, a, ws, nsplit);
  BZ_HIP(hipGetLastError());
  return BZ_OK;
}
int bzk_attn_merge_oproj_ok(const AttnArgs& a, const LinearDev& L) { int nw; return attn_oproj_plan(a, L, nw) > 0 && nw == 8; }
int bzk_attn_merge_oproj(hipStream_t s, const AttnArgs& a, const float* ws, int nsplit, const LinearDev& L, long long* acc) {
  int NW;
  const int CS = attn_oproj_plan(a, L, NW);
  if (CS <= 0 || NW != 8) BZ_FAIL(BZ_E_INVALID, "attn merge + o_proj fusion does not apply to this shape");
  const int TPW = (L.N / 64) / (CS * 8);
#define LAUNCH_MO(T) BZ_LAUNCH("attn_merge+o_proj", L.algo_bytes, (k_attn_merge_oproj<T>), dim3(a.nq * CS), dim3(512), 0, s, a, ws, nsplit, \
    (const uint4*)L.w, (const __half*)L.scales, (const unsigned char*)L.zeros, L.bias, CS, acc)
  if (TPW == 1) LAUNCH_MO(1); else LAUNCH_MO(2);
#undef LAUNCH_MO
  BZ_HIP(hipGetLastError());
  return BZ_OK;
}

int bzk_attn_decode(hipStream_t s, const AttnArgs& a) {
  const size_t smem = (size_t)(3 * a.hd + 8 + 256 * (a.hd + 4)) * 4;
#define LAUNCH_ATT(HD, DT) BZ_LAUNCH("attn_decode", 0.0, (k_attn_decode<HD, DT>), dim3(a.nq), dim3(256), smem, s, a)
#define LAUNCH_ATT_DT(HD) do { if (a.kv.dtype == BZ_F16) LAUNCH_ATT(HD, BZ_F16); else if (a.kv.dtype == BZ_BF16) LAUNCH_ATT(HD, BZ_BF16); \
                               else LAUNCH_ATT(HD, BZ_F32); } while (0)
  static const bool no_a64 = getenv("BZ_NO_ATTN2_HD64") != nullptr;
  if ((a.hd == 128 || (a.hd == 64 && a.rope_cur != nullptr && !no_a64)) && a.kv.dtype != BZ_F32) {
#define LAUNCH_A2(DT, PG, HDV) BZ_LAUNCH("attn_decode", 0.0, (k_attn2<DT, 0, 1, 8, PG, HDV>), dim3(a.nq), dim3(512), attn2_smem(8), s, a, (const uint4*)nullptr, \
    (const __half*)nullptr, (const unsigned char*)nullptr, (const float*)nullptr, 1, (long long*)nullptr)
#define LAUNCH_A2_P(DT, HDV) do { if (a.kv.paged) LAUNCH_A2(DT, 1, HDV); else LAUNCH_A2(DT, 0, HDV); } while (0)
#define LAUNCH_A2_H(DT) do { if (a.hd == 128) LAUNCH_A2_P(DT, 128); else LAUNCH_A2_P(DT, 64); } while (0)
    if (a.kv.dtype == BZ_F16) LAUNCH_A2_H(BZ_F16); else LAUNCH_A2_H(BZ_BF16);
#undef LAUNCH_A2_H
#undef LAUNCH_A2_P
#undef LAUNCH_A2
  }
  else if (a.hd == 128 && a.kv.dtype == BZ_F32 && a.rope_cur != nullptr && getenv("BZ_NO_ATTN_F32") == nullptr) {
    if (a.kv.paged) BZ_LAUNCH("attn_decode", 0.0, (k_attn2f<1, 0>), dim3(a.nq), dim3(512), 0, s, a, (const uint4*)nullptr, (const uint4*)nullptr, (const float*)nullptr, 1, (long long*)nullptr);
    else BZ_LAUNCH("attn_decode", 0.0, (k_attn2f<0, 0>), dim3(a.nq), dim3(512), 0, s, a, (const uint4*)nullptr, (const uint4*)nullptr, (const float*)nullptr, 1, (long long*)nullptr);
  }
  else if (a.hd == 64) LAUNCH_ATT_DT(64);
  else if (a.hd == 128) LAUNCH_ATT_DT(128);
  else BZ_FAIL(BZ_E_UNSUPPORTED, "head_dim %d unsupported (64 and 128 are built)", a.hd);
#undef LAUNCH_ATT_DT
#undef LAUNCH_ATT
  BZ_HIP(hipGetLastError());
  return BZ_OK;
}

__global__ void k_kv_insert(KvView kv, int layer, const float* k, const float* v, const int* pos, int nkv, int hd) {
  const int p = pos[0];
  for (int i = blockIdx.x * blockDim.x + threadIdx.x; i < nkv * hd; i += gridDim.x * blockDim.x) {
    const int h = i / hd, d = i % hd;
    const size_t off = kv.paged ? kv_slot_off(kv, layer, h, kv.slot ? kv.slot[0] : (kv.block_table[p / kv.bs] * kv.bs + p % kv.bs))
                                : kv_row_off(kv, layer, h, p);
    kv_st(kv.k, off + d, kv.dtype, k[i]);
    kv_st(kv.v, off + d, kv.dtype, v[i]);
  }
}
int bzk_kv_insert(hipStream_t s, const KvView& kv, int layer, const float* k, const float* v, const int* pos, int nkv, int hd) {
  hipLaunchKernelGGL(k_kv_insert, dim3((nkv * hd + 255) / 256), dim3(256), 0, s, kv, layer, k, v, pos, nkv, hd);
  BZ_HIP(hipGetLastError());
  return BZ_OK;
}
__global__ void k_kv_read(KvView kv, int layer, int kvh, int which, int len, float* out) {
  for (int i = blockIdx.x * blockDim.x + threadIdx.x; i < len * kv.hd; i += gridDim.x * blockDim.x) {
    const int p = i / kv.hd, d = i % kv.hd;
    out[i] = kv_ld(which ? kv.v : kv.k, kv_row_off(kv, layer, kvh, p) + d, kv.dtype);
  }
}
int bzk_kv_read(hipStream_t s, const KvView& kv, int layer, int kvh, int which, int len, float* out) {
  hipLaunchKernelGGL(k_kv_read, dim3((len * kv.hd + 255) / 256), dim3(256), 0, s, kv, layer, kvh, which, len, out);
  BZ_HIP(hipGetLastError());
  return BZ_OK;
}

__device__ __forceinline__ bool better(float v, int i, float bv, int bi) { return v > bv || (v == bv && i < bi); }

__global__ __launch_bounds__(256) void k_argmax_final(FinalArgs a) {
  __shared__ float sv[256];
  __shared__ int si[256];
  float bv = -INFINITY; int bi = 0x7fffffff;
  for (int i = threadIdx.x; i < a.nparts; i += 256) {
    const float v = a.pval[i]; const int ix = a.pidx[i];
    if (better(v, ix, bv, bi)) { bv = v; bi = ix; }
  }
  sv[threadIdx.x] = bv; si[threadIdx.x] = bi;
  __syncthreads();
  for (int s = 128; s > 0; s >>= 1) {
    if (threadIdx.x < s && better(sv[threadIdx.x + s], si[threadIdx.x + s], sv[threadIdx.x], si[threadIdx.x])) {
      sv[threadIdx.x] = sv[threadIdx.x + s]; si[threadIdx.x] = si[threadIdx.x + s];
    }
    __syncthreads();
  }
  if (threadIdx.x == 0) {
    const long long tok = si[0];
    a.tok_out[0] = tok;
    if (a.tok_log) { const int st = a.step[0]; a.tok_log[st % a.logcap] = tok; a.step[0] = st + 1; }
    if (a.pos) a.pos[0] = a.pos[0] + 1;
  }
  if (a.zero_buf) for (int i = threadIdx.x; i < a.zero_n; i += 256) a.zero_buf[i] = 0;
}
__global__ void k_batch_advance(long long* tok, const long long* next, int* pos, int* slot, const int* table, int stride, int bs, int N) {
  const int i = blockIdx.x * blockDim.x + threadIdx.x;
  if (i >= N) return;
  tok[i] = next[i];
  const int p = pos[i] + 1;
  pos[i] = p;
  slot[i] = table[(size_t)i * stride + p / bs] * bs + p % bs;
}
__global__ __launch_bounds__(256) void k_batch_argmax(const float* __restrict__ logits, int V, long long* next, long long* log, int* step, int logcap, int N) {
  __shared__ float sv[4]; __shared__ int si[4];
  const int row = blockIdx.x, tid = threadIdx.x, wave = tid >> 6, lane = tid & 63;
  const float* lg = logits + (size_t)row * V;
  float bv = -INFINITY; int bi = 0x7fffffff;
  for (int i = tid; i < V; i += 256) { const float v = lg[i]; if (v > bv) { bv = v; bi = i; } }
  for (int off = 32; off >= 1; off >>= 1) {
    const float ov = __shfl_xor(bv, off); const int oi = __shfl_xor(bi, off);
    if (ov > bv || (ov == bv && oi < bi)) { bv = ov; bi = oi; }
  }
  if (lane == 0) { sv[wave] = bv; si[wave] = bi; }
  __syncthreads();
  if (tid == 0) {
    for (int w = 1; w < 4; w++) if (sv[w] > bv || (sv[w] == bv && si[w] < bi)) { bv = sv[w]; bi = si[w]; }
    next[row] = bi;
    const int st = *step;
    log[(size_t)(st % logcap) * N + row] = bi;
  }
}
__global__ void k_batch_step_inc(int* step) { *step = *step + 1; }
int bzk_batch_advance(hipStream_t s, long long* tok, const long long* next, int* pos, int* slot, const int* table, int stride, int bs, int N) {
  hipLaunchKernelGGL(k_batch_advance, dim3((N + 63) / 64), dim3(64), 0, s, tok, next, pos, slot, table, stride, bs, N);
  BZ_HIP(hipGetLastError());
  return BZ_OK;
}
int bzk_batch_argmax(hipStream_t s, const float* logits, int V, long long* next, long long* log, int* step, int logcap, int N) {
  hipLaunchKernelGGL(k_batch_argmax, dim3(N), dim3(256), 0, s, logits, V, next, log, step, logcap, N);
  hipLaunchKernelGGL(k_batch_step_inc, dim3(1), dim3(1), 0, s, step);
  BZ_HIP(hipGetLastError());
  return BZ_OK;
}

int bzk_argmax_final(hipStream_t s, const FinalArgs& a) {
  BZ_LAUNCH("argmax_final", 0.0, k_argmax_final, dim3(1), dim3(256), 0, s, a);
  BZ_HIP(hipGetLastError());
  return BZ_OK;
}

__global__ __launch_bounds__(256) void k_penalised_argmax(const float* logits, long long V, const long long* ids, const int* cnts, int n,
                                                          float rp, float fp, float pp, float* pval, int* pidx) {
  __shared__ float sv[256];
  __shared__ int si[256];
  float bv = -INFINITY; int bi = 0x7fffffff;
  for (long long i = (long long)blockIdx.x * 256 + threadIdx.x; i < V; i += (long long)gridDim.x * 256) {
    float x = logits[i];
    for (int j = 0; j < n; j++) {
      if (ids[j] == i) {
        if (rp != 1.0f) x = (x > 0.f) ? x / rp : x * rp;
        x -= fp * (float)cnts[j] + pp;
      }
    }
// ... 1403 lines not shown
```

Baseline: 673.6 tokens/s.

## Fuse final argmax and next-token embed/RoPE staging into lm_head GEMV tail

The lm_head rows GEMV gains a last-block-done ticket. The final workgroup reduces the argmax partials, writes the token and position, and stages the next step's embedding row and RoPE cos/sin row into graph-owned buffers. This removes the separate argmax_final launch and the embed kernel at the start of each decode step inside the hipGraph. The cost is an atomic ticket plus serialized tail work in one block, and added complexity in memory ordering between blocks.

Result: no change. 673.4 tokens/s, median of 2 (-0.0%).

```diff
diff --git a/blazr_amd/csrc/bz_host.hip b/blazr_amd/csrc/bz_host.hip
--- a/blazr_amd/csrc/bz_host.hip
+++ b/blazr_amd/csrc/bz_host.hip
@@ -285,6 +285,7 @@
   std::vector<void*> owned;
   float* cos_t = nullptr; float* sin_t = nullptr;
   float* rope_cur = nullptr;
+  unsigned* tail_ticket = nullptr;
   float* att_ws = nullptr;
   float* hbuf[2] = {nullptr, nullptr};
   int pf_rows = 0; float* pf_h = nullptr; float* pf_t = nullptr; float* pf_qkv = nullptr; float* pf_gu = nullptr; void* pf_x16 = nullptr;
@@ -874,6 +875,7 @@
   m->nparts = m->lm_head.fix_out ? 64 : bzk_gemv_rows_blocks(m->lm_head.parts[0]);
   BZ_TRY(dev_alloc(m, &p, (size_t)m->nparts * 4)); m->pval = (float*)p;
   BZ_TRY(dev_alloc(m, &p, (size_t)m->nparts * 4)); m->pidx = (int*)p;
+  BZ_TRY(dev_alloc(m, &p, 64)); m->tail_ticket = (unsigned*)p; BZ_HIP(hipMemset(p, 0, 64));
   BZ_TRY(dev_alloc(m, &p, 4096)); m->scratch = (float*)p;
   BZ_TRY(dev_alloc(m, &p, 64)); m->tok_tmp = (long long*)p;
   BZ_TRY(dev_alloc(m, &p, 64)); m->pos_tmp = (int*)p;
@@ -1069,6 +1071,7 @@
   m->nparts = bzk_gemv_rows_blocks(m->lm_head.parts[0]);
   BZ_TRY(dev_alloc(m, &p, (size_t)m->nparts * 4)); m->pval = (float*)p;
   BZ_TRY(dev_alloc(m, &p, (size_t)m->nparts * 4)); m->pidx = (int*)p;
+  BZ_TRY(dev_alloc(m, &p, 64)); m->tail_ticket = (unsigned*)p; BZ_HIP(hipMemset(p, 0, 64));
   BZ_TRY(dev_alloc(m, &p, 4096)); m->scratch = (float*)p;
   BZ_TRY(dev_alloc(m, &p, 64)); m->tok_tmp = (long long*)p;
   BZ_TRY(dev_alloc(m, &p, 64)); m->pos_tmp = (int*)p;
@@ -1145,6 +1148,7 @@
   m->nparts = bzk_gemv_rows_blocks(m->lm_head.parts[0]);
   BZ_TRY(dev_alloc(m, &p, (size_t)m->nparts * 4)); m->pval = (float*)p;
   BZ_TRY(dev_alloc(m, &p, (size_t)m->nparts * 4)); m->pidx = (int*)p;
+  BZ_TRY(dev_alloc(m, &p, 64)); m->tail_ticket = (unsigned*)p; BZ_HIP(hipMemset(p, 0, 64));
   BZ_TRY(dev_alloc(m, &p, 64)); m->tok_tmp = (long long*)p;
   BZ_TRY(dev_alloc(m, &p, 64)); m->pos_tmp = (int*)p;
   const size_t act_b = bz_dtype_size(c.act_dtype);
@@ -1327,6 +1331,7 @@
   float* hidden_out = nullptr; float* prev_out = nullptr;
   FinalArgs* final_args = nullptr;
   bz_ssm_state* ssm = nullptr;
+  float* h_row = nullptr; float* rope_row = nullptr;
   int att_positions = 0;
 };
 
@@ -1364,6 +1369,42 @@
   return BZ_OK;
 }
 
+static bool step_tail_ok(const bz_model* m) {
+  return !m->lm_head.fix_out && m->lm_head.parts.size() == 1 && m->lm_head.parts[0].kind == LK_ROWS && m->lm_head.parts[0].sk <= 1 && m->tail_ticket != nullptr;
+}
+
+static int head_dense(bz_model* m, const StepIO& io, const Pro& ph, RingState& rs) {
+  const bz_model_config& c = m->cfg;
+  hipStream_t st = step_stream(m);
+  const int ra = (rs.ri + 2) % 3, rb = (rs.ri + 1) % 3;
+  GemvOut o{};
+  o.direct = m->logits; o.amax_val = m->pval; o.amax_idx = m->pidx;
+  o.zero_buf = rs.dirty[rb] > 0 ? m->ring[rb] : nullptr; o.zero_n = rs.dirty[rb];
+  StepTail tl{};
+  const bool fused = io.final_args && step_tail_ok(m);
+  if (fused) {
+    tl.fin = *io.final_args;
+    tl.fin.pval = m->pval; tl.fin.pidx = m->pidx; tl.fin.nparts = m->nparts;
+    tl.fin.zero_buf = rs.dirty[ra] > 0 ? m->ring[ra] : nullptr; tl.fin.zero_n = rs.dirty[ra];
+    tl.ticket = m->tail_ticket;
+    if (io.h_row) {
+      tl.table = m->embed; tl.tdt = m->embed_dt; tl.gg = m->embed_ggml; tl.H = c.hidden; tl.act = c.act_dtype; tl.vocab = c.vocab; tl.h_out = io.h_row;
+    }
+    if (io.rope_row) { tl.cos_t = m->cos_t; tl.sin_t = m->sin_t; tl.half = c.head_dim / 2; tl.rope_rows = c.max_seq_len; tl.rope_out = io.rope_row; }
+    o.tail = &tl;
+  }
+  BZ_TRY(bzk_gemv(st, m->lm_head.parts[0], ph, o, c.act_dtype));
+  rs.dirty[rb] = 0;
+  if (io.final_args && !fused) {
+    FinalArgs fa = *io.final_args;
+    fa.pval = m->pval; fa.pidx = m->pidx; fa.nparts = m->nparts;
+    fa.zero_buf = rs.dirty[ra] > 0 ? m->ring[ra] : nullptr; fa.zero_n = rs.dirty[ra];
+    BZ_TRY(bzk_argmax_final(st, fa));
+  }
+  if (io.final_args) rs.dirty[ra] = 0;
+  return BZ_OK;
+}
+
 static int llama_step(bz_model* m, const StepIO& io) {
   const bz_model_config& c = m->cfg;
   hipStream_t st = step_stream(m);
@@ -1372,7 +1413,9 @@
   int cur = 0;
   RingState rs;
   VSrc prev{nullptr, 0};
-  if (io.do_embed) {
+  float* rope_cur = io.rope_row ? io.rope_row : m->rope_cur;
+  if (io.h_row) {
+  } else if (io.do_embed) {
     BZ_TRY(bzk_embed(st, m->embed, m->embed_dt, m->embed_ggml, io.d_tok, H, act, m->hbuf[cur], io.d_pos, m->cos_t, m->sin_t, c.head_dim / 2, m->rope_cur));
   } else {
     if (io.d_pos && lend > io.layer_start) BZ_TRY(bzk_rope_row(st, io.d_pos, m->cos_t, m->sin_t, c.head_dim / 2, m->rope_cur));
@@ -1381,14 +1424,14 @@
   }
   for (int l = io.layer_start; l < lend; l++) {
     const LayerDev& Ld = m->layers[l];
-    Pro pn{}; pn.mode = PRO_NORM; pn.src = prev; pn.h_in = m->hbuf[cur]; pn.h_out = m->hbuf[cur ^ 1]; pn.norm_w = Ld.attn_norm;
+    Pro pn{}; pn.mode = PRO_NORM; pn.src = prev; pn.h_in = (io.h_row && l == io.layer_start) ? io.h_row : m->hbuf[cur]; pn.h_out = m->hbuf[cur ^ 1]; pn.norm_w = Ld.attn_norm;
     pn.eps = c.rms_eps; pn.H = H; pn.act = act;
     VSrc qkv;
     BZ_TRY(run_fused(m, Ld.qkv, pn, rs, &qkv));
     cur ^= 1;
 
     AttnArgs aa{};
-    aa.qkv = qkv; aa.cos_t = m->cos_t; aa.sin_t = m->sin_t; aa.interleaved = c.rope_interleaved; aa.pos = io.d_pos; aa.rope_cur = m->rope_cur;
+    aa.qkv = qkv; aa.cos_t = m->cos_t; aa.sin_t = m->sin_t; aa.interleaved = c.rope_interleaved; aa.pos = io.d_pos; aa.rope_cur = rope_cur;
     aa.nq = c.n_heads; aa.nkv = c.n_kv_heads; aa.hd = c.head_dim; aa.act = act; aa.kv = io.kv; aa.layer = l; aa.out = m->attn_out;
     aa.zero_buf = nullptr; aa.zero_n = 0; aa.q_only = 0;
     VSrc ov;
@@ -1456,30 +1499,21 @@
       else BZ_HIP(hipMemcpyAsync(io.prev_out, prev.p, (size_t)H * 4, hipMemcpyDeviceToDevice, st));
     }
   }
-  const int ra = (rs.ri + 2) % 3, rb = (rs.ri + 1) % 3;
   if (io.do_head) {
     Pro ph{}; ph.mode = PRO_NORM; ph.src = prev; ph.h_in = m->hbuf[cur]; ph.h_out = nullptr; ph.norm_w = m->final_norm;
     ph.eps = c.rms_eps; ph.H = H; ph.act = act;
-    int rfin = ra;
     if (m->lm_head.fix_out) {
       VSrc lv;
       BZ_TRY(run_fused(m, m->lm_head, ph, rs, &lv));
       BZ_TRY(bzk_fix_to_f32(st, (const long long*)lv.p, c.vocab, act, m->logits));
       BZ_TRY(bzk_argmax_partials(st, m->logits, c.vocab, m->pval, m->pidx, m->nparts));
-      rfin = -1;
+      if (io.final_args) {
+        FinalArgs fa = *io.final_args;
+        fa.pval = m->pval; fa.pidx = m->pidx; fa.nparts = m->nparts;
+        BZ_TRY(bzk_argmax_final(st, fa));
+      }
     } else {
-      GemvOut o{};
-      o.direct = m->logits; o.amax_val = m->pval; o.amax_idx = m->pidx;
-      o.zero_buf = rs.dirty[rb] > 0 ? m->ring[rb] : nullptr; o.zero_n = rs.dirty[rb];
-      BZ_TRY(bzk_gemv(st, m->lm_head.parts[0], ph, o, act));
-      rs.dirty[rb] = 0;
-    }
-    if (io.final_args) {
-      FinalArgs fa = *io.final_args;
-      fa.pval = m->pval; fa.pidx = m->pidx; fa.nparts = m->nparts;
-      if (rfin >= 0) { fa.zero_buf = rs.dirty[rfin] > 0 ? m->ring[rfin] : nullptr; fa.zero_n = rs.dirty[rfin]; }
-      BZ_TRY(bzk_argmax_final(st, fa));
-      if (rfin >= 0) rs.dirty[rfin] = 0;
+      BZ_TRY(head_dense(m, io, ph, rs));
     }
   }
   for (int i = 0; i < 3; i++) if (rs.dirty[i] > 0) BZ_TRY(bzk_zero64(st, m->ring[i], rs.dirty[i]));
@@ -1496,10 +1530,10 @@
   int cur = 0;
   RingState rs;
   VSrc prev{nullptr, 0};
-  BZ_TRY(bzk_embed(st, m->embed, m->embed_dt, m->embed_ggml, io.d_tok, D, act, m->hbuf[cur]));
+  if (!io.h_row) BZ_TRY(bzk_embed(st, m->embed, m->embed_dt, m->embed_ggml, io.d_tok, D, act, m->hbuf[cur]));
   for (int l = 0; l < c.n_layers; l++) {
     const MambaLayerDev& L = m->mlayers[l];
-    Pro pn{}; pn.mode = PRO_NORM; pn.src = prev; pn.h_in = m->hbuf[cur]; pn.h_out = m->hbuf[cur ^ 1]; pn.norm_w = L.norm; pn.eps = c.rms_eps; pn.H = D; pn.act = act;
+    Pro pn{}; pn.mode = PRO_NORM; pn.src = prev; pn.h_in = (io.h_row && l == 0) ? io.h_row : m->hbuf[cur]; pn.h_out = m->hbuf[cur ^ 1]; pn.norm_w = L.norm; pn.eps = c.rms_eps; pn.H = D; pn.act = act;
     VSrc zx;
     BZ_TRY(run_fused(m, L.in_proj, pn, rs, &zx));
     cur ^= 1;
@@ -1515,21 +1549,9 @@
     BZ_TRY(run_fused(m, L.out_proj, pg, rs, &ov, &shf));
     prev = ov;
   }
-  const int ra = (rs.ri + 2) % 3, rb = (rs.ri + 1) % 3;
   if (io.do_head) {
     Pro ph{}; ph.mode = PRO_NORM; ph.src = prev; ph.h_in = m->hbuf[cur]; ph.h_out = nullptr; ph.norm_w = m->final_norm; ph.eps = c.rms_eps; ph.H = D; ph.act = act;
-    GemvOut o{};
-    o.direct = m->logits; o.amax_val = m->pval; o.amax_idx = m->pidx;
-    o.zero_buf = rs.dirty[rb] > 0 ? m->ring[rb] : nullptr; o.zero_n = rs.dirty[rb];
-    BZ_TRY(bzk_gemv(st, m->lm_head.parts[0], ph, o, act));
-    rs.dirty[rb] = 0;
-    if (io.final_args) {
-      FinalArgs fa = *io.final_args;
-      fa.pval = m->pval; fa.pidx = m->pidx; fa.nparts = m->nparts;
-      fa.zero_buf = rs.dirty[ra] > 0 ? m->ring[ra] : nullptr; fa.zero_n = rs.dirty[ra];
-      BZ_TRY(bzk_argmax_final(st, fa));
-      rs.dirty[ra] = 0;
-    }
+    BZ_TRY(head_dense(m, io, ph, rs));
   }
   for (int i = 0; i < 3; i++) if (rs.dirty[i] > 0) BZ_TRY(bzk_zero64(st, m->ring[i], rs.dirty[i]));
   return BZ_OK;
@@ -1543,10 +1565,10 @@
   int cur = 0;
   RingState rs;
   VSrc prev{nullptr, 0};
-  BZ_TRY(bzk_embed(st, m->embed, m->embed_dt, m->embed_ggml, io.d_tok, H, act, m->hbuf[cur]));
+  if (!io.h_row) BZ_TRY(bzk_embed(st, m->embed, m->embed_dt, m->embed_ggml, io.d_tok, H, act, m->hbuf[cur]));
   for (int l = 0; l < c.n_layers; l++) {
     const DsLayerDev& L = m->dlayers[l];
-    Pro pn{}; pn.mode = PRO_NORM; pn.src = prev; pn.h_in = m->hbuf[cur]; pn.h_out = m->hbuf[cur ^ 1]; pn.norm_w = L.attn_norm; pn.eps = c.rms_eps; pn.H = H; pn.act = act; pn.f32_sums = 0;
+    Pro pn{}; pn.mode = PRO_NORM; pn.src = prev; pn.h_in = (io.h_row && l == 0) ? io.h_row : m->hbuf[cur]; pn.h_out = m->hbuf[cur ^ 1]; pn.norm_w = L.attn_norm; pn.eps = c.rms_eps; pn.H = H; pn.act = act; pn.f32_sums = 0;
     VSrc qkva;
     BZ_TRY(run_fused(m, L.qkva, pn, rs, &qkva));
     cur ^= 1;
@@ -1620,21 +1642,9 @@
       prev = VSrc{m->moe_out, 0};
     }
   }
-  const int ra = (rs.ri + 2) % 3, rb = (rs.ri + 1) % 3;
   if (io.do_head) {
     Pro ph{}; ph.mode = PRO_NORM; ph.src = prev; ph.h_in = m->hbuf[cur]; ph.h_out = nullptr; ph.norm_w = m->final_norm; ph.eps = c.rms_eps; ph.H = H; ph.act = act;
-    GemvOut o{};
-    o.direct = m->logits; o.amax_val = m->pval; o.amax_idx = m->pidx;
-    o.zero_buf = rs.dirty[rb] > 0 ? m->ring[rb] : nullptr; o.zero_n = rs.dirty[rb];
-    BZ_TRY(bzk_gemv(st, m->lm_head.parts[0], ph, o, act));
-    rs.dirty[rb] = 0;
-    if (io.final_args) {
-      FinalArgs fa = *io.final_args;
-      fa.pval = m->pval; fa.pidx = m->pidx; fa.nparts = m->nparts;
-      fa.zero_buf = rs.dirty[ra] > 0 ? m->ring[ra] : nullptr; fa.zero_n = rs.dirty[ra];
-      BZ_TRY(bzk_argmax_final(st, fa));
-      rs.dirty[ra] = 0;
-    }
+    BZ_TRY(head_dense(m, io, ph, rs));
   }
   for (int i = 0; i < 3; i++) if (rs.dirty[i] > 0) BZ_TRY(bzk_zero64(st, m->ring[i], rs.dirty[i]));
   return BZ_OK;
@@ -2610,6 +2620,8 @@
   long long* tok_buf = nullptr;
   int* pos = nullptr;
   int* step = nullptr;
+  float* h_row = nullptr;
+  float* rope_row = nullptr;
   long long* tok_log = nullptr;
   int* block_table = nullptr; int max_blocks = 0;
   bz_kv* kv = nullptr; bz_paged_kv* pkv = nullptr; bz_ssm_state* ssm = nullptr;
@@ -2624,6 +2636,7 @@
   fa.tok_out = g->tok_buf; fa.tok_log = g->tok_log; fa.step = g->step; fa.logcap = bz_decode_graph::LOGCAP; fa.pos = g->pos;
   StepIO io{};
   io.kv = g->view; io.d_tok = g->tok_buf; io.d_pos = g->pos; io.final_args = &fa; io.ssm = g->ssm; io.att_positions = att_positions;
+  io.h_row = g->h_row; io.rope_row = g->rope_row;
   BZ_TRACE("graph: begin capture");
   hipStream_t cap = nullptr;
   BZ_HIP(hipStreamCreateWithFlags(&cap, hipStreamNonBlocking));
@@ -2644,9 +2657,22 @@
   return BZ_OK;
 }
 
+static int graph_stage_rows(bz_decode_graph* g) {
+  bz_model* m = g->m;
+  if (!g->h_row) return BZ_OK;
+  const bool rope = g->rope_row != nullptr;
+  return bzk_embed(m->dev->stream, m->embed, m->embed_dt, m->embed_ggml, g->tok_buf, m->cfg.hidden, m->cfg.act_dtype, g->h_row, rope ? g->pos : nullptr,
+                   rope ? m->cos_t : nullptr, rope ? m->sin_t : nullptr, rope ? m->cfg.head_dim / 2 : 0, g->rope_row);
+}
+
 static int graph_capture_common(bz_decode_graph* g, const KvView& view) {
   bz_model* m = g->m;
   hipStream_t st = m->dev->stream;
+  if (step_tail_ok(m)) {
+    BZ_HIP(hipMalloc(&g->h_row, (size_t)m->cfg.hidden * 4));
+    BZ_HIP(hipMemset(g->h_row, 0, (size_t)m->cfg.hidden * 4));
+    if (m->cfg.arch == BZ_ARCH_LLAMA) { BZ_HIP(hipMalloc(&g->rope_row, 256 * 4)); BZ_HIP(hipMemset(g->rope_row, 0, 256 * 4)); }
+  }
   BZ_HIP(hipMalloc(&g->tok_buf, 64));
   BZ_HIP(hipMalloc(&g->pos, 64));
   BZ_HIP(hipMalloc(&g->step, 64));
@@ -2656,6 +2682,8 @@
   BZ_HIP(hipDeviceSynchronize());
   g->view = view;
   BZ_TRY(graph_capture_variant(g, 0, &g->graph, &g->exec));
+  BZ_TRY(graph_stage_rows(g));
+  BZ_HIP(hipStreamSynchronize(st));
   for (int i = 0; i < 8; i++) { hipEvent_t ev; BZ_HIP(hipEventCreateWithFlags(&ev, hipEventDisableTiming)); g->evs.push_back(ev); }
   return BZ_OK;
 }
@@ -2868,6 +2896,7 @@
   BZ_HIP(hipMemcpyAsync(g->tok_buf, &t, 8, hipMemcpyHostToDevice, st));
   BZ_HIP(hipMemcpyAsync(g->pos, &p, 4, hipMemcpyHostToDevice, st));
   BZ_HIP(hipMemcpyAsync(g->step, &z, 4, hipMemcpyHostToDevice, st));
+  BZ_TRY(graph_stage_rows(g));
   BZ_HIP(hipStreamSynchronize(st));
   g->replays = 0; g->seed_pos = position;
   return BZ_OK;
@@ -2927,6 +2956,8 @@
   if (g->tok_buf) hipFree(g->tok_buf);
   if (g->pos) hipFree(g->pos);
   if (g->step) hipFree(g->step);
+  if (g->h_row) hipFree(g->h_row);
+  if (g->rope_row) hipFree(g->rope_row);
   if (g->block_table) hipFree(g->block_table);
   if (g->tok_log) hipHostFree(g->tok_log);
   bz_dev_release(g->dev);
diff --git a/blazr_amd/csrc/bz_internal.h b/blazr_amd/csrc/bz_internal.h
--- a/blazr_amd/csrc/bz_internal.h
+++ b/blazr_amd/csrc/bz_internal.h
@@ -156,6 +156,7 @@
   int zero_n;
   float* amax_val; int* amax_idx;
   ConvShift shift;
+  const struct StepTail* tail;
 };
 
 int bzk_gemv(hipStream_t s, const LinearDev& L, const Pro& pro, const GemvOut& out, int act);
@@ -231,6 +232,12 @@
   long long* zero_buf; int zero_n;
 };
 int bzk_argmax_final(hipStream_t s, const FinalArgs& a);
+struct StepTail {
+  FinalArgs fin;
+  unsigned* ticket;
+  const void* table; int tdt, gg, H, act, vocab; float* h_out;
+  const float* cos_t; const float* sin_t; int half, rope_rows; float* rope_out;
+};
 int bzk_logits_to_token(hipStream_t s, const float* logits, long long V, const long long* ids, const int* cnts, int n, float rp,
                         float fp, float pp, float temperature, int top_k, float top_p, float min_p, unsigned long long seed,
                         float* scratch , long long* tok_out);
diff --git a/blazr_amd/csrc/bz_kernels.hip b/blazr_amd/csrc/bz_kernels.hip
--- a/blazr_amd/csrc/bz_kernels.hip
+++ b/blazr_amd/csrc/bz_kernels.hip
@@ -1606,7 +1606,7 @@
   x[0] = (double)xa.x; x[1] = (double)xa.y; x[2] = (double)xa.z; x[3] = (double)xa.w; x[4] = (double)xb.x; x[5] = (double)xb.y; x[6] = (double)xb.z; x[7] = (double)xb.w;
 }
 
-template <int WDT, bool SPLIT>
+template <int WDT, bool SPLIT, bool PUB = false>
 __device__ __forceinline__ void rows_body(const void* __restrict__ W, const float* __restrict__ bias, int N, int K, int rows_per_wg, const Pro& pro,
                                           float* out, int act, float* pval, int* pidx, long long* zero_buf, int zero_n, int SK, long long* accbuf,
                                           const int bid) {
@@ -1642,12 +1642,12 @@
   const float4* xs4;
   if (!SPLIT || pro.mode == PRO_GATED) {
     for (int i = K + threadIdx.x; i < KP; i += 256) xs[xs_pos<true>(i)] = 0.f;
-    build_x_simple<true>(pro, 0, K, xs, red, bid == 0);
+    [[clang::always_inline]] build_x_simple<true>(pro, 0, K, xs, red, bid == 0);
     xs4 = (const float4*)(xs + kb);
   } else {
     const int KR = max(min(K - kb, KC * 512), 0);
     for (int i = KR + threadIdx.x; i < KC * 512; i += 256) xs[xs_pos<true>(i)] = 0.f;
-    build_x_simple<true>(pro, kb, KR, xs, red, bid == 0);
+    [[clang::always_inline]] build_x_simple<true>(pro, kb, KR, xs, red, bid == 0);
     xs4 = (const float4*)xs;
   }
   float bestv = -INFINITY; int besti = 0x7fffffff;
@@ -1699,7 +1699,10 @@
     if (threadIdx.x == 0) {
       float v = bv[0]; int ix = bi[0];
       for (int w2 = 1; w2 < 4; w2++) if (bv[w2] > v) { v = bv[w2]; ix = bi[w2]; }
-      pval[bid] = v; pidx[bid] = ix;
+      if constexpr (PUB) {
+        __hip_atomic_store(pval + bid, v, __ATOMIC_RELAXED, __HIP_MEMORY_SCOPE_AGENT);
+        __hip_atomic_store(pidx + bid, ix, __ATOMIC_RELAXED, __HIP_MEMORY_SCOPE_AGENT);
+      } else { pval[bid] = v; pidx[bid] = ix; }
     }
   }
 }
@@ -1709,6 +1712,89 @@
                                                    int rows_per_wg, Pro pro, float* out, int act, float* pval, int* pidx,
                                                    long long* zero_buf, int zero_n, int SK, long long* accbuf) {
   rows_body<WDT, SPLIT>(W, bias, N, K, rows_per_wg, pro, out, act, pval, pidx, zero_buf, zero_n, SK, accbuf, blockIdx.x);
+}
+
+__device__ __forceinline__ bool better(float v, int i, float bv, int bi) { return v > bv || (v == bv && i < bi); }
+
+template <typename LD>
+__device__ __forceinline__ void tail_embed_row(int H, int act, float* h, LD ld) {
+  for (int base = 0; base < H; base += 4096) {
+    float v[16];
+#pragma unroll
+    for (int j = 0; j < 16; j++) { const int i = base + j * 256 + (int)threadIdx.x; v[j] = i < H ? ld(i) : 0.f; }
+#pragma unroll
+    for (int j = 0; j < 16; j++) { const int i = base + j * 256 + (int)threadIdx.x; if (i < H) h[i] = round_act(v[j], act); }
+  }
+}
+
+__device__ __forceinline__ void step_tail(const float* pval, const int* pidx, const int nparts, long long* tok_out, long long* tok_log, int* step, const int logcap, int* pos,
+                                          long long* zero_buf, const int zero_n, unsigned* ticket, const void* table, const int tdt, const int gg, const int H,
+                                          const int act, const int vocab, float* h_out, const float* cos_t, const float* sin_t, const int half, const int rope_rows,
+                                          float* rope_out, float* sc) {
+  const int tid = threadIdx.x, wave = tid >> 6, lane = tid & 63;
+  unsigned* last = (unsigned*)(sc + 8);
+  if (tid == 0) {
+    asm volatile("s_waitcnt vmcnt(0)" ::: "memory");
+    last[0] = __hip_atomic_fetch_add(ticket, 1u, __ATOMIC_RELAXED, __HIP_MEMORY_SCOPE_AGENT) == gridDim.x - 1 ? 1u : 0u;
+  }
+  __syncthreads();
+  if (!last[0]) return;
+  float bv = -INFINITY; int bi = 0x7fffffff;
+  for (int i = tid; i < nparts; i += 256) {
+    const float v = __hip_atomic_load(pval + i, __ATOMIC_RELAXED, __HIP_MEMORY_SCOPE_AGENT);
+    const int ix = __hip_atomic_load(pidx + i, __ATOMIC_RELAXED, __HIP_MEMORY_SCOPE_AGENT);
+    if (better(v, ix, bv, bi)) { bv = v; bi = ix; }
+  }
+#pragma unroll
+  for (int off = 32; off >= 1; off >>= 1) {
+    const float ov = __shfl_xor(bv, off); const int oi = __shfl_xor(bi, off);
+    if (better(ov, oi, bv, bi)) { bv = ov; bi = oi; }
+  }
+  int* si = (int*)(sc + 4);
+  if (lane == 0) { sc[wave] = bv; si[wave] = bi; }
+  const int pn = pos ? pos[0] + 1 : 0;
+  __syncthreads();
+  bv = sc[0]; bi = si[0];
+#pragma unroll
+  for (int w = 1; w < 4; w++) if (better(sc[w], si[w], bv, bi)) { bv = sc[w]; bi = si[w]; }
+  const long long tok = bi;
+  if (tid == 0) {
+    tok_out[0] = tok;
+    if (tok_log) { const int st = step[0]; tok_log[st % logcap] = tok; step[0] = st + 1; }
+    if (pos) pos[0] = pn;
+    __hip_atomic_store(ticket, 0u, __ATOMIC_RELAXED, __HIP_MEMORY_SCOPE_AGENT);
+  }
+  if (rope_out != nullptr && tid < 2 * half && pn < rope_rows) {
+    const int i = tid % half;
+    rope_out[tid] = tid < half ? cos_t[(size_t)pn * half + i] : sin_t[(size_t)pn * half + i];
+  }
+  if (h_out != nullptr && tok >= 0 && tok < vocab) {
+    if (gg != 0) {
+      const unsigned char* row = (const unsigned char*)table + (size_t)tok * ggml_blk_row_bytes(gg, H);
+#pragma unroll 1
+      for (int i = tid; i < H; i += 256) h_out[i] = round_act(ggml_row_elem(gg, row, i), act);
+    } else if (tdt == BZ_F32) {
+      const float* row = (const float*)table + (size_t)tok * H;
+      tail_embed_row(H, act, h_out, [=](int i) { return row[i]; });
+    } else if (tdt == BZ_F16) {
+      const __half* row = (const __half*)table + (size_t)tok * H;
+      tail_embed_row(H, act, h_out, [=](int i) { return __half2float(row[i]); });
+    } else {
+      const unsigned short* row = (const unsigned short*)table + (size_t)tok * H;
+      tail_embed_row(H, act, h_out, [=](int i) { return __uint_as_float((unsigned)row[i] << 16); });
+    }
+  }
+  if (zero_buf) for (int i = tid; i < zero_n; i += 256) zero_buf[i] = 0;
+}
+
+template <int WDT>
+__global__ __launch_bounds__(256) void k_gemv_rows_tail(const void* __restrict__ W, const float* __restrict__ bias, int N, int K, int rows_per_wg, Pro pro, float* out,
+                                                        int act, float* pval, int* pidx, long long* zero_buf, int zero_n, StepTail tail) {
+  extern __shared__ __attribute__((aligned(16))) char smem[];
+  rows_body<WDT, false, true>(W, bias, N, K, rows_per_wg, pro, out, act, pval, pidx, zero_buf, zero_n, 1, nullptr, blockIdx.x);
+  step_tail(tail.fin.pval, tail.fin.pidx, tail.fin.nparts, tail.fin.tok_out, tail.fin.tok_log, tail.fin.step, tail.fin.logcap, tail.fin.pos, tail.fin.zero_buf, tail.fin.zero_n,
+            tail.ticket, tail.table, tail.tdt, tail.gg, tail.H, tail.act, tail.vocab, tail.h_out, tail.cos_t, tail.sin_t, tail.half, tail.rope_rows, tail.rope_out,
+            (float*)smem + ((K + 511) & ~511) + 4);
 }
 
 __device__ __forceinline__ float wave_sum4(float v0, float v1, float v2, float v3) {
@@ -2440,6 +2526,7 @@
 int bzk_argmax_partials(hipStream_t s, const float* v, long long n, float* pval, int* pidx, int nb);
 
 int bzk_gemv(hipStream_t s, const LinearDev& L, const Pro& pro, const GemvOut& out, int act) {
+  if (out.tail && (L.kind != LK_ROWS || L.sk > 1 || out.acc)) BZ_FAIL(BZ_E_INVALID, "gemv: the step tail needs the direct-output rows kernel");
   if (L.kind == LK_Q4G && act == BZ_F16 && bzk_gemv_slim_ok(L, pro)) {
     if (!out.acc) BZ_FAIL(BZ_E_INVALID, "int4 gemv needs a fixed-point accumulator");
     const int nks = L.K / 256, ntg = (L.N / 64 + 7) / 8;
@@ -2508,6 +2595,21 @@
     const int KP = (L.K + 511) & ~511;
     const size_t smem = (size_t)KP * 4 + 64;
     if (smem > 160 * 1024) BZ_FAIL(BZ_E_UNSUPPORTED, "K=%d too large for the rows GEMV", L.K);
+    if (out.tail) {
+      const StepTail& t = *out.tail;
+      if (SK != 1 || !out.amax_val || !out.amax_idx || !t.ticket || !t.fin.tok_out || t.fin.pval != out.amax_val || t.fin.pidx != out.amax_idx || t.fin.nparts != grid ||
+          (t.fin.tok_log && (!t.fin.step || t.fin.logcap <= 0)))
+        BZ_FAIL(BZ_E_INVALID, "rows gemv: bad step tail arguments");
+      if (t.h_out && (!t.table || t.H <= 0 || t.vocab <= 0 || (t.gg != 0 && (ggml_blk_row_bytes(t.gg, t.H) == 0 || t.H % ggml_blk_k(t.gg)))))
+        BZ_FAIL(BZ_E_INVALID, "rows gemv: bad embedding staging arguments");
+      if (t.rope_out && (2 * t.half > 256 || t.half <= 0 || !t.fin.pos || !t.cos_t || !t.sin_t || t.rope_rows <= 0)) BZ_FAIL(BZ_E_INVALID, "rows gemv: bad RoPE staging arguments");
+#define LAUNCH_ROWS_TAIL(DT) BZ_LAUNCH("gemv_rows<lm_head+argmax>", L.algo_bytes, (k_gemv_rows_tail<DT>), dim3(grid), dim3(256), smem, s, (const void*)L.w, L.bias, L.N, L.K, \
+    rpw, pro, out.direct, act, out.amax_val, out.amax_idx, out.zero_buf, out.zero_n, t)
+      if (L.wdt == BZ_F16) LAUNCH_ROWS_TAIL(BZ_F16); else if (L.wdt == BZ_BF16) LAUNCH_ROWS_TAIL(BZ_BF16); else LAUNCH_ROWS_TAIL(BZ_F32);
+#undef LAUNCH_ROWS_TAIL
+      BZ_HIP(hipGetLastError());
+      return BZ_OK;
+    }
     const char* lbl = out.amax_val ? "gemv_rows<lm_head+argmax>" : pro.mode == PRO_NORM ? "gemv_rows<norm>" : (pro.mode == PRO_GATED || pro.mode == PRO_GATED2) ? "gemv_rows<gated>"
                       : pro.mode == PRO_SILU ? "gemv_rows<silu>" : "gemv_rows";
 #define LAUNCH_ROWS1(DT, SP) BZ_LAUNCH(lbl, L.algo_bytes, (k_gemv_rows<DT, SP>), dim3(grid), \
@@ -3841,8 +3943,6 @@
   return BZ_OK;
 }
 
-__device__ __forceinline__ bool better(float v, int i, float bv, int bi) { return v > bv || (v == bv && i < bi); }
-
 __global__ __launch_bounds__(256) void k_argmax_final(FinalArgs a) {
   __shared__ float sv[256];
   __shared__ int si[256];
```
